# CompVis/stable-diffusion

Measured on AMD Instinct MI355X. Metric: 512x512 images/sec, SD-v1-4 50-step PLMS CFG=7.5, higher is better.
Workload: dtype f16

## Files before the change

### include/sdmi.h

```cpp
#ifndef SDMI_H_
#define SDMI_H_

#include <stdint.h>

#ifdef __cplusplus
extern "C" {
#endif

#define SDMI_ABI_VERSION 17

typedef struct sdmi_unet sdmi_unet;

typedef struct sdmi_unet_cfg {
  int32_t in_channels;
  int32_t out_channels;
  int32_t model_channels;
  int32_t num_res_blocks;
  int32_t n_levels;
  int32_t channel_mult[8];
  int32_t n_attention_resolutions;
  int32_t attention_resolutions[8];
  int32_t num_heads;
  int32_t transformer_depth;
  int32_t context_dim;
// ... 171 lines not shown
                        float* cs, float* d, void* stream);
int sdmi_k_attention(const void* q, const void* k, const void* vt, void* out, int BH, int heads, int nq, int nkv,
                     int nkv_pad, int d, float scale, void* stream);
int sdmi_k_attention_split16(const void* q, const void* q_lo, const void* k, const void* k_lo, const void* vt, const void* vt_lo, void* out,
                             void* out_lo, int BH, int heads, int nq, int nkv, int nkv_pad, int d, float scale, void* stream);
int sdmi_k_attention_causal(const void* q, const void* k, const void* vt, void* out, int BH, int heads, int n, int n_pad,
                            int d, float scale, void* stream);
int sdmi_k_groupnorm(const float* x0, const float* x1, int c0, int c1, int B, int HW, const float* gamma,
                     const float* beta, float eps, int silu, void* out_f16, float* out_f32, void* raw_f16, void* out_lo,
                     void* raw_lo, float* partial_ws, int64_t partial_floats, void* stream);
int64_t sdmi_k_groupnorm_ws_floats(int B, int HW);
int sdmi_k_groupnorm_film(const float* x0, const float* x1, int c0, int c1, int B, int HW, const float* gamma, const float* beta, float eps,
                          int silu, const float* film, int film_ld, void* out_f16, float* out_f32, void* raw_f16, void* out_lo, void* raw_lo,
                          float* partial_ws, int64_t partial_floats, void* stream);
int sdmi_k_layernorm(const float* x, const float* gamma, const float* beta, void* out_f16, int M, int C, float eps,
                     void* stream);
int sdmi_k_cast_f16(const float* x, void* out_f16, void* out_lo, int64_t n, void* stream);
int sdmi_k_split_heads(const float* src, int ld, int col0, void* dst, void* dst_lo, int kind, int B, int ntok, int ntok_pad, int heads, int dh,
                       void* stream);
int sdmi_k_geglu_split(const float* src, int M, int F, void* out, void* out_lo, void* stream);
int sdmi_k_layernorm_split(const float* x, const float* gamma, const float* beta, void* out, void* out_lo, int M, int C, float eps, void* stream);
int sdmi_k_timestep_embedding(const int64_t* t_i64, const float* t_f32, float* out, int B, int dim, void* stream);
int sdmi_k_small_linear(const float* in, int ld_in, const float* w, const float* bias, float* out, int ld_out, int B,
                        int N, int K, int silu_in, void* stream);
int sdmi_k_conv_in(const float* x_nchw, const float* w_oihw, const float* bias, float* out_nhwc, int B, int Cin, int H,
                   int W, int Cout, void* stream);
int sdmi_k_conv_out(const float* h_nhwc, const float* w_ohwi, const float* bias, float* out_nchw, int B, int H, int W,
                    int Cin, int Cout, void* stream);
int sdmi_k_pack_conv_weight(const float* w_oihw, void* dst_f16, int O, int I, int KH, int KW, void* stream);
int sdmi_k_pack_conv_weight_src(const float* w_oihw, void* dst_f16, int O, int I, int KH, int KW, int c0, int c1, int c2, void* stream);
int sdmi_k_pack_conv_out(const float* w_oihw, float* dst_ohwi, int O, int I, void* stream);
int sdmi_k_pack_split3(const float* w, void* dst_f16, int N, int K, void* stream);
int sdmi_k_pack_conv_split3(const float* w_oihw, void* dst_f16, int O, int I, int KH, int KW, void* stream);
int sdmi_k_pointwise_nchw(const float* x, const float* w, const float* bias, float* out, int B, int Cin, int Cout, int HW,
                          float in_scale, void* stream);
int sdmi_k_softmax_rows(const float* S, void* P_f16, int rows, int cols, float scale, void* stream);
int sdmi_k_vq_quantize(const float* z, float z_scale, const float* codebook, float* norms_ws, int n_embed, int D, float* zq, int32_t* idx,
                       int B, int HW, void* stream);
int sdmi_k_resample2(const float* x, float* out_f32, void* out_f16, void* out_lo, int B, int H, int W, int C, int dir, void* stream);
int sdmi_k_patch_unfold(const float* x, const float* c, float* out, int B, int Cx, int Cc, int H, int W, int kh, int kw, int sy, int sx,
                        int l0, int nl, void* stream);
int sdmi_k_patch_fold(const float* o, const float* w, float* out, int B, int C, int H, int W, int kh, int kw, int sy, int sx, int uf, int df,
                      int norm_only, void* stream);
int sdmi_k_gelu_erf(const float* x, void* out_f16, int64_t n, void* stream);
int sdmi_k_pack_geglu(const float* w, const float* bias, void* wdst_f16, float* bdst, int N, int K, void* stream);
int sdmi_image_to_uint8(const float* img_nchw, void* out_nhwc_u8, int B, int C, int H, int W, void* stream);
int sdmi_range_check(int enable);
int sdmi_range_report(char* json_buf, int json_buf_len);
int sdmi_tune_begin(void);
int sdmi_tune_round(int r);
int sdmi_tune_end(const char* path, int* n_keys);
int sdmi_tune_dump(char* buf, int buflen);
int sdmi_profile_begin(void);
int sdmi_profile_end(char* json_buf, int json_buf_len);
int sdmi_k_prefetch_lines(const void* ptr, int64_t bytes, void* stream);
const void* sdmi_zero_page(void);

#ifdef __cplusplus
}
#endif
#endif
```

### stable-diffusion_amd/_lib.py

```python
import ctypes as C
import os

_HERE = os.path.dirname(os.path.abspath(__file__))
LIB_PATH = os.environ.get('SDMI_LIB_PATH') or os.path.join(_HERE, 'libsdmi.so')

c_f32p = C.c_void_p
c_ptr = C.c_void_p


class UNetCfg(C.Structure):
    _fields_ = [('in_channels', C.c_int32), ('out_channels', C.c_int32), ('model_channels', C.c_int32),
                ('num_res_blocks', C.c_int32), ('n_levels', C.c_int32), ('channel_mult', C.c_int32 * 8),
                ('n_attention_resolutions', C.c_int32), ('attention_resolutions', C.c_int32 * 8),
                ('num_heads', C.c_int32), ('transformer_depth', C.c_int32), ('context_dim', C.c_int32)]


class VaeCfg(C.Structure):
    _fields_ = [('ch', C.c_int32), ('out_ch', C.c_int32), ('n_levels', C.c_int32), ('ch_mult', C.c_int32 * 8),
                ('num_res_blocks', C.c_int32), ('in_channels', C.c_int32), ('z_channels', C.c_int32),
                ('embed_dim', C.c_int32)]


class UNetExt(C.Structure):
    _fields_ = [('attention_block', C.c_int32), ('resblock_updown', C.c_int32)]
# ... 109 lines not shown
                                C.c_int, c_ptr]),
    'sdmi_k_st_head': (C.c_int, [c_ptr, c_ptr, C.c_int64, c_ptr, c_ptr, C.c_float, c_ptr, c_ptr, c_ptr, c_ptr, C.c_float, c_ptr, c_ptr, c_ptr,
                                 c_ptr, c_ptr, c_ptr, C.c_int, C.c_int, C.c_int, C.c_int, C.c_int, C.c_int, c_ptr]),
    'sdmi_k_attention_split16': (C.c_int, [c_ptr, c_ptr, c_ptr, c_ptr, c_ptr, c_ptr, c_ptr, c_ptr, C.c_int, C.c_int, C.c_int, C.c_int,
                                           C.c_int, C.c_int, C.c_float, c_ptr]),
    'sdmi_k_attention_causal': (C.c_int, [c_ptr, c_ptr, c_ptr, c_ptr, C.c_int, C.c_int, C.c_int, C.c_int, C.c_int, C.c_float,
                                          c_ptr]),
    'sdmi_k_pointwise_nchw': (C.c_int, [c_ptr, c_ptr, c_ptr, c_ptr, C.c_int, C.c_int, C.c_int, C.c_int, C.c_float, c_ptr]),
    'sdmi_k_softmax_rows': (C.c_int, [c_ptr, c_ptr, C.c_int, C.c_int, C.c_float, c_ptr]),
    'sdmi_k_gelu_erf': (C.c_int, [c_ptr, c_ptr, C.c_int64, c_ptr]),
    'sdmi_k_attention': (C.c_int, [c_ptr, c_ptr, c_ptr, c_ptr, C.c_int, C.c_int, C.c_int, C.c_int, C.c_int, C.c_int,
                                   C.c_float, c_ptr]),
    'sdmi_k_groupnorm': (C.c_int, [c_ptr, c_ptr, C.c_int, C.c_int, C.c_int, C.c_int, c_ptr, c_ptr, C.c_float, C.c_int,
                                   c_ptr, c_ptr, c_ptr, c_ptr, c_ptr, c_ptr, C.c_int64, c_ptr]),
    'sdmi_k_groupnorm_ws_floats': (C.c_int64, [C.c_int, C.c_int]),
    'sdmi_k_groupnorm_film': (C.c_int, [c_ptr, c_ptr, C.c_int, C.c_int, C.c_int, C.c_int, c_ptr, c_ptr, C.c_float, C.c_int, c_ptr, C.c_int,
                                        c_ptr, c_ptr, c_ptr, c_ptr, c_ptr, c_ptr, C.c_int64, c_ptr]),
    'sdmi_k_layernorm': (C.c_int, [c_ptr, c_ptr, c_ptr, c_ptr, C.c_int, C.c_int, C.c_float, c_ptr]),
    'sdmi_k_cast_f16': (C.c_int, [c_ptr, c_ptr, c_ptr, C.c_int64, c_ptr]),
    'sdmi_k_split_heads': (C.c_int, [c_ptr, C.c_int, C.c_int, c_ptr, c_ptr, C.c_int, C.c_int, C.c_int, C.c_int, C.c_int, C.c_int,
                                     c_ptr]),
    'sdmi_k_geglu_split': (C.c_int, [c_ptr, C.c_int, C.c_int, c_ptr, c_ptr, c_ptr]),
    'sdmi_k_layernorm_split': (C.c_int, [c_ptr, c_ptr, c_ptr, c_ptr, c_ptr, C.c_int, C.c_int, C.c_float, c_ptr]),
    'sdmi_k_timestep_embedding': (C.c_int, [c_ptr, c_ptr, c_ptr, C.c_int, C.c_int, c_ptr]),
    'sdmi_k_small_linear': (C.c_int, [c_ptr, C.c_int, c_ptr, c_ptr, c_ptr, C.c_int, C.c_int, C.c_int, C.c_int,
                                      C.c_int, c_ptr]),
    'sdmi_k_conv_in': (C.c_int, [c_ptr, c_ptr, c_ptr, c_ptr, C.c_int, C.c_int, C.c_int, C.c_int, C.c_int, c_ptr]),
    'sdmi_k_conv_out': (C.c_int, [c_ptr, c_ptr, c_ptr, c_ptr, C.c_int, C.c_int, C.c_int, C.c_int, C.c_int, c_ptr]),
    'sdmi_k_pack_conv_weight': (C.c_int, [c_ptr, c_ptr, C.c_int, C.c_int, C.c_int, C.c_int, c_ptr]),
    'sdmi_k_pack_conv_weight_src': (C.c_int, [c_ptr, c_ptr, C.c_int, C.c_int, C.c_int, C.c_int, C.c_int, C.c_int, C.c_int, c_ptr]),
    'sdmi_k_pack_conv_out': (C.c_int, [c_ptr, c_ptr, C.c_int, C.c_int, c_ptr]),
    'sdmi_k_pack_split3': (C.c_int, [c_ptr, c_ptr, C.c_int, C.c_int, c_ptr]),
    'sdmi_k_pack_conv_split3': (C.c_int, [c_ptr, c_ptr, C.c_int, C.c_int, C.c_int, C.c_int, c_ptr]),
    'sdmi_k_pack_geglu': (C.c_int, [c_ptr, c_ptr, c_ptr, c_ptr, C.c_int, C.c_int, c_ptr]),
    'sdmi_k_ln_fold_prep': (C.c_int, [c_ptr, C.c_int, C.c_int, C.c_int, c_ptr, c_ptr, c_ptr, c_ptr, c_ptr, c_ptr]),
    'sdmi_image_to_uint8': (C.c_int, [c_ptr, c_ptr, C.c_int, C.c_int, C.c_int, C.c_int, c_ptr]),
    'sdmi_range_check': (C.c_int, [C.c_int]),
    'sdmi_range_report': (C.c_int, [C.c_char_p, C.c_int]),
    'sdmi_tune_begin': (C.c_int, []),
    'sdmi_tune_round': (C.c_int, [C.c_int]),
    'sdmi_tune_end': (C.c_int, [C.c_char_p, C.POINTER(C.c_int)]),
    'sdmi_tune_dump': (C.c_int, [C.c_char_p, C.c_int]),
    'sdmi_profile_begin': (C.c_int, []),
    'sdmi_profile_end': (C.c_int, [C.c_char_p, C.c_int]),
    'sdmi_k_prefetch_lines': (C.c_int, [c_ptr, C.c_int64, c_ptr]),
    'sdmi_zero_page': (c_ptr, []),
}

_lib = None


class SdmiError(RuntimeError):
    pass


def load():
    global _lib
    if _lib is None:
        if not os.path.exists(LIB_PATH):
            raise SdmiError(f'{LIB_PATH} not found: build it with `python stable-diffusion_amd/build.py` '
                            '(the MI355X path has no fallback implementation)')
        lib = C.CDLL(LIB_PATH)
        for name, (res, args) in _SIGS.items():
            fn = getattr(lib, name)
            fn.restype = res
            fn.argtypes = args
# ... 23 lines not shown
```

### stable-diffusion_amd/csrc/api.cpp

```cpp
#include <string.h>

#include <new>

#include "prof.h"
#include "split16.h"
#include "unet.h"
#include "vae.h"
#include "clip.h"

namespace sdmi {
static thread_local std::string g_err;
void set_error(const std::string& msg) { g_err = msg; }
int fail(const std::string& msg) { g_err = msg; return -1; }
}

struct sdmi_unet { sdmi::UNet impl; };
struct sdmi_vae { sdmi::Vae impl; };
struct sdmi_clip { sdmi::ClipText impl; };
struct sdmi_bert { sdmi::BertText impl; };

using namespace sdmi;

static int weight_info(const WeightStore& w, int idx, char* key_buf, int key_buf_len, int64_t* shape4, int* ndim) {
  SDMI_CHECK(key_buf && shape4 && ndim, "null argument");
// ... 272 lines not shown
int sdmi_k_vq_quantize(const float* z, float z_scale, const float* codebook, float* norms_ws, int n_embed, int D, float* zq, int32_t* idx,
                       int B, int HW, void* stream) {
  if (launch_vq_norms(codebook, norms_ws, n_embed, D, (hipStream_t)stream)) return -1;
  return launch_vq_quantize(z, z_scale, codebook, norms_ws, n_embed, D, zq, (int*)idx, B, HW, (hipStream_t)stream);
}
int sdmi_k_resample2(const float* x, float* out_f32, void* out_f16, void* out_lo, int B, int H, int W, int C, int dir, void* stream) {
  return launch_resample2(x, out_f32, (f16*)out_f16, (f16*)out_lo, B, H, W, C, dir, (hipStream_t)stream);
}
int sdmi_k_patch_unfold(const float* x, const float* c, float* out, int B, int Cx, int Cc, int H, int W, int kh, int kw, int sy, int sx,
                        int l0, int nl, void* stream) {
  return launch_patch_unfold(x, c, out, B, Cx, Cc, H, W, kh, kw, sy, sx, l0, nl, (hipStream_t)stream);
}
int sdmi_k_patch_fold(const float* o, const float* w, float* out, int B, int C, int H, int W, int kh, int kw, int sy, int sx, int uf, int df,
                      int norm_only, void* stream) {
  return launch_patch_fold(o, w, out, B, C, H, W, kh, kw, sy, sx, uf, df, norm_only, (hipStream_t)stream);
}
int sdmi_k_gelu_erf(const float* x, void* out_f16, int64_t n, void* stream) {
  return launch_gelu_erf(x, (f16*)out_f16, n, (hipStream_t)stream);
}
int sdmi_k_attention_causal(const void* q, const void* k, const void* vt, void* out, int BH, int heads, int n, int n_pad,
                            int d, float scale, void* stream) {
  AttnParams a = AttnParams();
  a.q = (const f16*)q; a.k = (const f16*)k; a.vt = (const f16*)vt; a.out = (f16*)out;
  a.BH = BH; a.heads = heads; a.nq = n; a.nkv = n; a.nkv_pad = n_pad; a.d = d; a.scale = scale; a.causal = 1;
  return launch_attention(a, (hipStream_t)stream);
}

static int igemm_params_of(const sdmi_igemm_desc* d, IGemmParams& p) {
  p.a0 = (const f16*)d->a0; p.a1 = (const f16*)d->a1; p.a2 = (const f16*)d->a2;
  p.c0 = d->c0; p.c1 = d->c1; p.c2 = d->c2; p.lda0 = d->lda0; p.lda1 = d->lda1; p.lda2 = d->lda2;
  p.B = d->B; p.Hin = d->Hin; p.Win = d->Win; p.Hout = d->Hout; p.Wout = d->Wout;
  p.ksize = d->ksize; p.stride = d->stride; p.up = d->up; p.pad = d->asym_pad ? 0 : 1;
  p.w = (const f16*)d->w; p.M = d->B * d->Hout * d->Wout; p.N = d->N; p.K = d->ksize * d->ksize * (d->c0 + d->c1 + d->c2);
  p.mode = d->mode; p.bias = d->bias; p.rowvec = d->rowvec; p.ld_rowvec = d->ld_rowvec;
  p.residual = d->residual; p.ldr = d->ldr; p.out_f32 = d->out_f32; p.out_f16 = (f16*)d->out_f16; p.ldo = d->ldo;
  for (int i = 0; i < 3; ++i) { p.seg_dst[i] = (f16*)d->seg_dst[i]; p.seg_kind[i] = d->seg_kind[i]; }
  p.heads = d->heads; p.dh = d->dh; p.ntok = d->ntok; p.ntok_pad = d->ntok_pad; p.segC = d->segC;
  p.splitk = d->splitk; p.splitk_ws = d->splitk_ws; p.splitk_ws_floats = d->splitk_ws_floats;
  p.splitk_cnt = d->splitk_cnt; p.splitk_cnt_ints = d->splitk_cnt_ints;
  p.gn_n = d->gn_n;
  for (int i = 0; i < 2; ++i) { p.gn_acc[i] = (long long*)d->gn_acc[i]; p.gn_cpg[i] = d->gn_cpg[i]; p.gn_cbase[i] = d->gn_cbase[i]; }
  if (d->split16) {
    p.split16 = 1; p.c1 = 0; p.K = d->c0; p.ldw = 3 * d->c0;
  }
  p.f16_scale = d->f16_scale; p.lnp_out = d->lnp_out;
  p.lnf_part = d->lnf_part; p.lnf_npart = d->lnf_npart; p.lnf_eps = d->lnf_eps; p.lnf_cs = d->lnf_cs; p.lnf_d = d->lnf_d;
  p.pgn_gamma = d->pgn_gamma; p.pgn_beta = d->pgn_beta; p.pgn_eps = d->pgn_eps; p.pgn_silu = d->pgn_silu;
  p.pgn_out = (f16*)d->pgn_out; p.pgn_keep_f32 = d->pgn_keep_f32; p.pgn_applied = d->pgn_applied;
  p.out_lo = (f16*)d->out_lo;
  return zero_page(&p.zero_page);
}
int sdmi_k_igemm(const sdmi_igemm_desc* d, void* stream) {
  SDMI_CHECK(d, "null descriptor");
  IGemmParams p = IGemmParams();
  if (igemm_params_of(d, p)) return -1;
  IGemmTune t; t.tile = d->tile; t.dma = d->dma;
  return launch_igemm(p, t, (hipStream_t)stream);
}
int sdmi_k_ff_tail(const sdmi_igemm_desc* proj_out, const void* ln_f16, const float* lnp, float ln_eps, const float* csd,
                   const void* wgg_f16, const void* wff2_f16, const float* bff2, const float* t, void* stream) {
  SDMI_CHECK(proj_out, "null descriptor");
  FfTailParams q = FfTailParams();
  if (igemm_params_of(proj_out, q.epi)) return -1;
  SDMI_CHECK(proj_out->split16 && proj_out->ksize == 1, "ff_tail: the proj_out descriptor is a split-fp16 1x1 (w = sdmi_k_pack_split3)");
  q.ln = (const f16*)ln_f16; q.lnp = lnp; q.ln_eps = ln_eps; q.csd = csd; q.wgg = (const f16*)wgg_f16; q.wff2 = (const f16*)wff2_f16;
  q.bff2 = bff2; q.t = t; q.wpo = (const f16*)proj_out->w;
// ... 119 lines not shown
int sdmi_k_geglu_split(const float* src, int M, int F, void* out, void* out_lo, void* stream) {
  return launch_geglu_split(src, M, F, (f16*)out, (f16*)out_lo, (hipStream_t)stream);
}
int sdmi_k_layernorm_split(const float* x, const float* gamma, const float* beta, void* out, void* out_lo, int M, int C, float eps, void* stream) {
  return launch_layernorm_split(x, gamma, beta, (f16*)out, (f16*)out_lo, M, C, eps, (hipStream_t)stream);
}
int sdmi_k_timestep_embedding(const int64_t* t_i64, const float* t_f32, float* out, int B, int dim, void* stream) {
  return launch_timestep_embedding(t_i64, t_f32, out, B, dim, (hipStream_t)stream);
}
int sdmi_k_small_linear(const float* in, int ld_in, const float* w, const float* bias, float* out, int ld_out, int B,
                        int N, int K, int silu_in, void* stream) {
  return launch_small_linear(in, ld_in, w, bias, out, ld_out, B, N, K, silu_in, (hipStream_t)stream);
}
int sdmi_k_conv_in(const float* x, const float* w, const float* bias, float* out, int B, int Cin, int H, int W, int Cout,
                   void* stream) {
  return launch_conv_in(x, w, bias, out, B, Cin, H, W, Cout, (hipStream_t)stream);
}
int sdmi_k_conv_out(const float* h, const float* w, const float* bias, float* out, int B, int H, int W, int Cin, int Cout,
                    void* stream) {
  return launch_conv_out(h, w, bias, out, B, H, W, Cin, Cout, (hipStream_t)stream);
}
int sdmi_k_pack_conv_weight(const float* w, void* dst, int O, int I, int KH, int KW, void* stream) {
  return launch_pack_conv_weight(w, (f16*)dst, O, I, KH, KW, (hipStream_t)stream);
}
int sdmi_k_pack_conv_weight_src(const float* w, void* dst, int O, int I, int KH, int KW, int c0, int c1, int c2, void* stream) {
  return launch_pack_conv_weight_src(w, (f16*)dst, O, I, KH, KW, c0, c1, c2, (hipStream_t)stream);
}
int sdmi_k_pack_conv_out(const float* w, float* dst, int O, int I, void* stream) {
  return launch_pack_conv_out(w, dst, O, I, (hipStream_t)stream);
}
int sdmi_k_pack_split3(const float* w, void* dst, int N, int K, void* stream) {
  return launch_pack_split3(w, (f16*)dst, N, K, (hipStream_t)stream);
}
int sdmi_k_pack_conv_split3(const float* w, void* dst, int O, int I, int KH, int KW, void* stream) {
  return launch_pack_conv_split3(w, (f16*)dst, O, I, KH, KW, (hipStream_t)stream);
}
int sdmi_k_pack_geglu(const float* w, const float* bias, void* wdst, float* bdst, int N, int K, void* stream) {
  return launch_pack_geglu(w, bias, (f16*)wdst, bdst, N, K, (hipStream_t)stream);
}
int sdmi_image_to_uint8(const float* img_nchw, void* out_nhwc_u8, int B, int C, int H, int W, void* stream) {
  return launch_image_u8(img_nchw, (unsigned char*)out_nhwc_u8, B, C, H, W, (hipStream_t)stream);
}
int sdmi_range_check(int enable) { return range_check_set(enable); }
int sdmi_range_report(char* buf, int buflen) {
  SDMI_CHECK(buf && buflen > 1, "null buffer");
  std::string js;
  if (range_report(&js)) return -1;
  SDMI_CHECK((int)js.size() + 1 <= buflen, "range report buffer too small");
  memcpy(buf, js.c_str(), js.size() + 1);
  return 0;
}
int sdmi_tune_begin(void) { return tune_begin(); }
int sdmi_tune_round(int r) { return tune_round(r); }
int sdmi_tune_end(const char* path, int* n_keys) { return tune_end(path, n_keys); }
int sdmi_tune_dump(char* buf, int buflen) {
  SDMI_CHECK(buf && buflen > 1, "null buffer");
  std::string txt;
  if (tune_dump(&txt)) return -1;
  SDMI_CHECK((int)txt.size() + 1 <= buflen, "tune dump buffer too small");
  memcpy(buf, txt.c_str(), txt.size() + 1);
  return 0;
}
int sdmi_profile_begin(void) { return prof_begin(); }
int sdmi_profile_end(char* buf, int buflen) {
  SDMI_CHECK(buf && buflen > 2, "null buffer");
  std::string js;
// ... 17 lines not shown
```

### stable-diffusion_amd/csrc/common.h

```cpp
#pragma once
#include <hip/hip_runtime.h>
#include <stdint.h>
#include <algorithm>
#include <string>

#include "tape.h"

typedef _Float16 f16;
typedef _Float16 f16x2 __attribute__((ext_vector_type(2)));
typedef _Float16 f16x4 __attribute__((ext_vector_type(4)));
typedef _Float16 f16x8 __attribute__((ext_vector_type(8)));
typedef float f32x4 __attribute__((ext_vector_type(4)));
typedef float f32x16 __attribute__((ext_vector_type(16)));

#ifdef __HIPCC__
__device__ __forceinline__ float gn_apply_elem(float v, float mean, float rstd, float gamma, float beta, int silu) {
  float t = __builtin_fmaf((v - mean) * rstd, gamma, beta);
  if (silu) t = t * __builtin_amdgcn_rcpf(1.0f + __expf(-t));
  return t;
}
__device__ __forceinline__ float gn_apply_film_elem(float v, float mean, float rstd, float gamma, float beta, float scale, float shift,
                                                    int silu) {
  float t = __builtin_fmaf((v - mean) * rstd, gamma, beta);
  t = __builtin_fmaf(t, 1.0f + scale, shift);
// ... 291 lines not shown
  float* x_next = nullptr;
  int64_t n = 0;
};
int launch_dpm_step(const DpmStepParams& p, hipStream_t s);

int launch_embed_tokens(const int64_t* ids, const float* tok_emb, const float* pos_emb, float* out, int M, int L, int C,
                        int vocab, hipStream_t s);
int launch_quick_gelu(const float* x, f16* out, int64_t n, hipStream_t s);
int launch_gelu_erf(const float* x, f16* out, int64_t n, hipStream_t s);

int launch_pointwise_nchw(const float* x_nchw, const float* w, const float* bias, float* out_nchw, int B, int Cin, int Cout,
                          int HW, float in_scale, hipStream_t s);
int launch_softmax_rows(const float* S, f16* P, int rows, int cols, int lds, int ldp, float scale, hipStream_t s);

int launch_resample2(const float* x, float* o32, f16* hi, f16* lo, int B, int H, int W, int C, int dir, hipStream_t s);
int launch_vq_norms(const float* e, float* se, int n_embed, int D, hipStream_t s);
int launch_vq_quantize(const float* z, float z_scale, const float* e, const float* se, int n_embed, int D, float* zq, int* idx, int B,
                       int HW, hipStream_t s);

int launch_patch_unfold(const float* x, const float* c, float* out, int B, int Cx, int Cc, int H, int W, int kh, int kw, int sy, int sx,
                        int l0, int nl, hipStream_t s);
int launch_patch_fold(const float* o, const float* w, float* out, int B, int C, int H, int W, int kh, int kw, int sy, int sx, int uf, int df,
                      int norm_only, hipStream_t s);

int launch_prefetch_lines(const void* ptr, int64_t bytes, hipStream_t s);

int launch_pack_conv_weight(const float* w_oihw, f16* dst, int O, int I, int KH, int KW, hipStream_t s);
int launch_pack_rows(const float* w, f16* dst, int rows, int cols, int dst_row0, int dst_ld, hipStream_t s);
int launch_ln_fold_prep(const f16* w, int N, int K, int ldw, const float* gamma, const float* beta, const float* bias, float* cs,
                        float* d, hipStream_t s);
int launch_pack_split3(const float* w, f16* dst, int N, int K, hipStream_t s);
int launch_pack_conv_weight_src(const float* w_oihw, f16* dst, int O, int I, int KH, int KW, int c0, int c1, int c2, hipStream_t s);
int launch_pack_conv_split3(const float* w, f16* dst, int O, int I, int KH, int KW, hipStream_t s);
int launch_pack_geglu(const float* w, const float* bias, f16* wdst, float* bdst, int N, int K, hipStream_t s);
int launch_pack_conv_out(const float* w_oihw, float* dst, int O, int I, hipStream_t s);

struct SamplerStepParams {
  const float* eps_model = nullptr;
  int cfg = 0; float scale = 1.f;
  const float* x = nullptr;
  int mode = 0;
  const float* old0 = nullptr; const float* old1 = nullptr; const float* old2 = nullptr;
  float a_t = 1.f, a_prev = 1.f, sigma = 0.f, sqrt_1m_at = 0.f;
  const float* noise = nullptr;
  float* e_t_out = nullptr;
  float* x_prev = nullptr; float* pred_x0 = nullptr;
  int64_t n = 0;
};
int launch_sampler_step(const SamplerStepParams& p, hipStream_t s);
int launch_image_u8(const float* img_nchw, unsigned char* out_nhwc, int B, int C, int H, int W, hipStream_t s);

}
```

### stable-diffusion_amd/csrc/igemm.hip

```cpp
#include <dlfcn.h>

#include <map>
#include <mutex>
#include <tuple>
#include <vector>

#include "igemm_dev.h"

namespace sdmi {
namespace {

__global__ void __launch_bounds__(256) splitk_reduce_kernel(IGemmParams p, int nsplit, int rows_per_block) {
  __shared__ unsigned long long s_gn[2][32][GN_WORDS];
  const int tx = threadIdx.x & 7, ty = threadIdx.x >> 3;
  const int n = (blockIdx.x * 8 + tx) * 4;
  const int row0 = blockIdx.y * rows_per_block;
  const int HW = p.Hout * p.Wout;
  const bool gn = p.gn_n > 0;
  const bool ncol = n < p.N;
  if (gn) {
    for (int i = threadIdx.x; i < 2 * 32 * GN_WORDS; i += 256) (&s_gn[0][0][0])[i] = 0ull;
    __syncthreads();
  }
  const size_t slab_sz = (size_t)p.M * p.N;
  f32x4 biasv = {0.f, 0.f, 0.f, 0.f};
  if (ncol && p.bias) biasv = *(const f32x4*)(p.bias + n);
  float a1[2] = {0.f, 0.f}, a2[2] = {0.f, 0.f}, c1[2] = {0.f, 0.f}, c2[2] = {0.f, 0.f};
  int g0[2] = {0, 0}, g1[2] = {0, 0}, gsplit[2] = {4, 4};
  for (int t = 0; t < p.gn_n; ++t) {
    const int c = p.gn_cbase[t] + n;
    g0[t] = fast_div(c, p.gn_magic[t]); g1[t] = fast_div(c + 3, p.gn_magic[t]);
    gsplit[t] = (g0[t] + 1) * p.gn_cpg[t] - c;
  }
  for (int r = ty; r < rows_per_block; r += 32) {
    const int m = row0 + r;
    if (!ncol || m >= p.M) continue;
    const float* src = p.splitk_ws + (size_t)m * p.N + n;
    f32x4 rvv = {0.f, 0.f, 0.f, 0.f}, resv = {0.f, 0.f, 0.f, 0.f};
    if (p.rowvec) rvv = *(const f32x4*)(p.rowvec + (size_t)(m / HW) * p.ld_rowvec + n);
    if (p.residual) resv = *(const f32x4*)(p.residual + (size_t)m * p.ldr + n);
    f32x4 part[16];
#pragma unroll
    for (int s = 0; s < 16; ++s) part[s] = (s < nsplit) ? *(const f32x4*)(src + s * slab_sz) : f32x4{0, 0, 0, 0};
    f32x4 v = part[0];
#pragma unroll
    for (int s = 1; s < 16; ++s) v += part[s];
    v += biasv;
    if (p.rowvec) v += rvv;
    if (p.residual) v += resv;
    if (p.out_f32) SDMI_ST_F32X4(p.out_f32, (size_t)m * p.ldo + n, v);
    if (p.out_f16) SDMI_ST_F16X4(p.out_f16, (size_t)m * p.ldo + n, (f16x4{(f16)v[0], (f16)v[1], (f16)v[2], (f16)v[3]}));
    if (p.out_lo) {
      f16x4 lo;
#pragma unroll
      for (int j = 0; j < 4; ++j) lo[j] = (f16)(v[j] - (float)(f16)v[j]);
      *(f16x4*)(p.out_lo + (size_t)m * p.ldo + n) = lo;
    }
    if (gn) {
#pragma unroll
      for (int t = 0; t < 2; ++t) {
#pragma unroll
        for (int j = 0; j < 4; ++j) {
          if (j < gsplit[t]) { a1[t] += v[j]; a2[t] += v[j] * v[j]; } else { c1[t] += v[j]; c2[t] += v[j] * v[j]; }
        }
      }
    }
  }
  if (gn) {
    if (ncol) {
      for (int t = 0; t < p.gn_n; ++t) {
        gn_acc_add(&s_gn[t][g0[t]][0], a1[t]);
        gn_acc_add(&s_gn[t][g0[t]][2], a2[t]);
        if (g1[t] != g0[t]) { gn_acc_add(&s_gn[t][g1[t]][0], c1[t]); gn_acc_add(&s_gn[t][g1[t]][2], c2[t]); }
      }
    }
    __syncthreads();
    const int b = row0 / HW;
    const int slot = (blockIdx.x + blockIdx.y) & (GN_SLOTS - 1);
    for (int e = threadIdx.x; e < p.gn_n * 32 * GN_WORDS; e += 256) {
      const unsigned long long w = (&s_gn[0][0][0])[e];
      if (w == 0ull) continue;
      const int word = e % GN_WORDS, g = (e / GN_WORDS) % 32, t = e / (GN_WORDS * 32);
      atomicAdd((unsigned long long*)p.gn_acc[t] + ((size_t)(b * 32 + g) * GN_SLOTS + slot) * GN_STRIDE + word, w);
    }
  }
}

__global__ void __launch_bounds__(256) splitk_reduce_heads_kernel(IGemmParams p, int nsplit) {
  const int64_t idx = (int64_t)blockIdx.x * blockDim.x + threadIdx.x;
  const int nq = p.N / 4;
  if (idx >= (int64_t)p.M * nq) return;
  const int m = (int)(idx / nq);
  const int n = (int)(idx - (int64_t)m * nq) * 4;
  const size_t slab_sz = (size_t)p.M * p.N;
  const float* src = p.splitk_ws + (size_t)m * p.N + n;
  f32x4 part[16];
#pragma unroll
  for (int s = 0; s < 16; ++s) part[s] = (s < nsplit) ? *(const f32x4*)(src + s * slab_sz) : f32x4{0, 0, 0, 0};
  f32x4 v = part[0];
#pragma unroll
  for (int s = 1; s < 16; ++s) v += part[s];
  if (p.bias) v += *(const f32x4*)(p.bias + n);
  const int seg = n / p.segC;
  const int c = n - seg * p.segC;
  const int head = c / p.dh;
  const int dd = c - head * p.dh;
  const int b = m / p.ntok;
  const int tok = m - b * p.ntok;
  const size_t bh = (size_t)b * p.heads + head;
  f16* dst = p.seg_dst[seg];
  if (p.seg_kind[seg] == 0) {
    *(f16x4*)(dst + (bh * p.ntok + tok) * p.dh + dd) = f16x4{(f16)v[0], (f16)v[1], (f16)v[2], (f16)v[3]};
  } else {
#pragma unroll
    for (int j = 0; j < 4; ++j) dst[(bh * p.dh + dd + j) * p.ntok_pad + tok] = (f16)v[j];
  }
}

__device__ __forceinline__ float pick4(const f32x4 v, int idx) {
  return idx == 0 ? v[0] : (idx == 1 ? v[1] : (idx == 2 ? v[2] : v[3]));
}
template <int CTRL>
__device__ __forceinline__ float quad_dpp(float x) {
  return __builtin_bit_cast(float, __builtin_amdgcn_update_dpp(0, __builtin_bit_cast(int, x), CTRL, 0xF, 0xF, true));
}
__device__ __forceinline__ f32x4 quad_transpose(const f32x4 v, int sub) {
  const float r0 = pick4(v, sub);
  const float r1 = quad_dpp<0x93>(pick4(v, (sub + 1) & 3));
  const float r2 = quad_dpp<0x4E>(pick4(v, (sub + 2) & 3));
  const float r3 = quad_dpp<0x39>(pick4(v, (sub + 3) & 3));
  const f32x4 r = {r0, r1, r2, r3};
  return f32x4{pick4(r, sub & 3), pick4(r, (sub - 1) & 3), pick4(r, (sub - 2) & 3), pick4(r, (sub - 3) & 3)};
}
__device__ __forceinline__ void quad_partials_split(const f32x4 v, int gsplit, float* a1, float* a2, float* c1, float* c2) {
#pragma clang fp contract(off)
  float s1 = 0.f, s2 = 0.f, t1 = 0.f, t2 = 0.f;
#pragma unroll
  for (int j = 0; j < 4; ++j) {
    const float sq = v[j] * v[j];
    if (j < gsplit) { s1 += v[j]; s2 += sq; } else { t1 += v[j]; t2 += sq; }
  }
  *a1 = s1; *a2 = s2; *c1 = t1; *c2 = t2;
}
struct TiledQuad { size_t off; int m, n; bool valid; };
__device__ __forceinline__ TiledQuad tiled_quad(const IGemmParams& p, int q, int lane) {
  const int BM = p.slab_bm, BN = p.slab_bn;
  const int WTM = BM / p.slab_wm, WTN = BN >> p.slab_sh_wn;
  const int tiles_n = (p.N + BN - 1) / BN;
  const int tile = q >> p.slab_sh_qpt, rem = q - (tile << p.slab_sh_qpt);
  const int blk = rem >> p.slab_sh_nt, t_in = rem - (blk << p.slab_sh_nt);
  const int wave = t_in >> 6;
  const int ij = blk >> 2, r4 = blk & 3, i = ij >> p.slab_sh_tn, j = ij - (i << p.slab_sh_tn);
  const int wm = wave >> p.slab_sh_wn, wn = wave - (wm << p.slab_sh_wn);
  const int tile_m = tile / tiles_n, tile_n = tile - tile_m * tiles_n;
  const int l31 = lane & 31, lg = lane >> 5;
  TiledQuad t;
  t.off = (size_t)tile * (size_t)(BM * BN) + (size_t)rem * 4;
  t.m = tile_m * BM + wm * WTM + i * 32 + 8 * r4 + 4 * lg + (l31 & 3);
  t.n = tile_n * BN + wn * WTN + j * 32 + (l31 & ~3);
  t.valid = t.m < p.M && t.n < p.N;
  return t;
}
#ifndef SDMI_REDUCE_GN_XCD_DEFAULT
#define SDMI_REDUCE_GN_XCD_DEFAULT 0
#endif
constexpr int COOP_BAR_INTS = 18 * 32;
template <bool COOP>
__global__ void __launch_bounds__(COOP ? 1024 : 256) splitk_reduce_tiled_kernel(IGemmParams p, int nsplit) {
  constexpr int NWV = COOP ? 16 : 4;
  __shared__ unsigned long long s_gn[2][NWV][32][GN_WORDS];
  const int tid = threadIdx.x, lane = tid & 63, wv = tid >> 6, NTB = blockDim.x;
  const bool gn = p.gn_n > 0;
  if (gn) {
    for (int i = tid; i < 2 * NWV * 32 * GN_WORDS; i += NTB) (&s_gn[0][0][0][0])[i] = 0ull;
    __syncthreads();
  }
  const TiledQuad t = tiled_quad(p, blockIdx.x * NTB + tid, lane);
  const int ntiles = ((p.M + p.slab_bm - 1) / p.slab_bm) * ((p.N + p.slab_bn - 1) / p.slab_bn);
  const size_t split_stride = (size_t)ntiles * (size_t)(p.slab_bm * p.slab_bn);
  const float* src = p.splitk_ws + t.off;
  const int HW = p.Hout * p.Wout;
  const int m = min(t.m, p.M - 1), n = min(t.n, p.N - 4);
  f32x4 biasv = {0.f, 0.f, 0.f, 0.f}, rvv = {0.f, 0.f, 0.f, 0.f}, resv = {0.f, 0.f, 0.f, 0.f};
  if (p.bias) biasv = *(const f32x4*)(p.bias + n);
  if (p.rowvec) rvv = *(const f32x4*)(p.rowvec + (size_t)(m / HW) * p.ld_rowvec + n);
  if (p.residual) resv = *(const f32x4*)(p.residual + (size_t)m * p.ldr + n);
  f32x4 part[16];
#pragma unroll
  for (int s = 0; s < 16; ++s) part[s] = (s < nsplit) ? *(const f32x4*)(src + s * split_stride) : f32x4{0.f, 0.f, 0.f, 0.f};
  f32x4 a = part[0];
#pragma unroll
  for (int s = 1; s < 16; ++s) a += part[s];
  f32x4 v = quad_transpose(a, lane & 3);
  v += biasv;
  if (p.rowvec) v += rvv;
  if (p.residual) v += resv;
  if (t.valid) {
    if (p.out_f32 && (!COOP || p.pgn_keep_f32)) SDMI_ST_F32X4(p.out_f32, (size_t)m * p.ldo + n, v);
    if (p.out_f16) SDMI_ST_F16X4(p.out_f16, (size_t)m * p.ldo + n, (f16x4{(f16)v[0], (f16)v[1], (f16)v[2], (f16)v[3]}));
    if (p.out_lo) {
      f16x4 lo;
#pragma unroll
      for (int j = 0; j < 4; ++j) lo[j] = (f16)(v[j] - (float)(f16)v[j]);
      *(f16x4*)(p.out_lo + (size_t)m * p.ldo + n) = lo;
    }
  }
  if (gn) {
    if (t.valid) {
      for (int tg = 0; tg < p.gn_n; ++tg) {
        const int c = p.gn_cbase[tg] + n;
        const int g0 = fast_div(c, p.gn_magic[tg]), g1 = fast_div(c + 3, p.gn_magic[tg]);
        const int gsplit = (g0 + 1) * p.gn_cpg[tg] - c;
        float a1, a2, c1, c2;
        quad_partials_split(v, gsplit, &a1, &a2, &c1, &c2);
        gn_acc_add(&s_gn[tg][wv][g0][0], a1);
        gn_acc_add(&s_gn[tg][wv][g0][2], a2);
        if (g1 != g0) { gn_acc_add(&s_gn[tg][wv][g1][0], c1); gn_acc_add(&s_gn[tg][wv][g1][2], c2); }
      }
    }
    __syncthreads();
    const int slot = blockIdx.x & (GN_SLOTS - 1);
    for (int e = tid; e < p.gn_n * NWV * 32 * GN_WORDS; e += NTB) {
      const unsigned long long w = (&s_gn[0][0][0][0])[e];
      if (w == 0ull) continue;
      const int word = e % GN_WORDS, g = (e / GN_WORDS) % 32, w4 = (e / (GN_WORDS * 32)) % NWV, tg = e / (GN_WORDS * 32 * NWV);
      if (w4 * 64 >= NTB) continue;
      const TiledQuad t0 = tiled_quad(p, blockIdx.x * NTB + w4 * 64, 0);
      if (t0.m >= p.M) continue;
      const int b = t0.m / HW;
      atomicAdd((unsigned long long*)p.gn_acc[tg] + ((size_t)(b * 32 + g) * GN_SLOTS + slot) * GN_STRIDE + word, w);
    }
  }
  if constexpr (COOP) {
    __shared__ int s_ok;
    __shared__ float2 s_tab[NWV][4];
    asm volatile("s_waitcnt vmcnt(0)" ::: "memory");
    __syncthreads();
    int* const blk = p.splitk_cnt + p.splitk_cnt_ints - COOP_BAR_INTS;
    const int nblk = (int)gridDim.x, ngrp = min(nblk, 8);
    if (tid == 0) {
      const int g = (int)blockIdx.x & 7, pop = (nblk - g + 7) >> 3;
      const int ep = __hip_atomic_load(blk + 9 * 32, __ATOMIC_RELAXED, __HIP_MEMORY_SCOPE_AGENT) + 1;
      if (__hip_atomic_fetch_add(blk + g * 32, 1, __ATOMIC_RELAXED, __HIP_MEMORY_SCOPE_AGENT) == pop - 1) {
        if (__hip_atomic_fetch_add(blk + 8 * 32, 1, __ATOMIC_RELAXED, __HIP_MEMORY_SCOPE_AGENT) == ngrp - 1) {
          for (int j = 0; j <= 8; ++j) __hip_atomic_store(blk + j * 32, 0, __ATOMIC_RELAXED, __HIP_MEMORY_SCOPE_AGENT);
          __hip_atomic_store(blk + 9 * 32, ep, __ATOMIC_RELAXED, __HIP_MEMORY_SCOPE_AGENT);
          for (int j = 0; j < ngrp; ++j) __hip_atomic_store(blk + (10 + j) * 32, ep, __ATOMIC_RELAXED, __HIP_MEMORY_SCOPE_AGENT);
        }
      }
      int budget = 1 << 16, seen = 0;
      while ((seen = __hip_atomic_load(blk + (10 + g) * 32, __ATOMIC_RELAXED, __HIP_MEMORY_SCOPE_AGENT)) != ep && --budget > 0) __builtin_amdgcn_s_sleep(2);
      s_ok = seen == ep;
    }
    __syncthreads();
    const int cpg = p.N >> 5;
    const TiledQuad tw = tiled_quad(p, blockIdx.x * NTB + wv * 64, 0);
    const int bw = min(tw.m, p.M - 1) / HW;
    const int gfirst = fast_div(min(tw.n, p.N - 1), p.gn_magic[0]);
    if (lane < 32) {
      const int g = min(gfirst + (lane >> 3), 31), sub = lane & 7;
      const long long* srcw = (const long long*)p.gn_acc[0] + ((size_t)(bw * 32 + g) * GN_SLOTS + sub) * GN_STRIDE;
// ... 29 lines not shown
  const float* src = p.splitk_ws + t.off;
  f32x4 part[16];
#pragma unroll
  for (int s = 0; s < 16; ++s) part[s] = (s < nsplit) ? *(const f32x4*)(src + s * split_stride) : f32x4{0.f, 0.f, 0.f, 0.f};
  f32x4 a = part[0];
#pragma unroll
  for (int s = 1; s < 16; ++s) a += part[s];
  f32x4 v = quad_transpose(a, lane & 3);
  if (!t.valid) return;
  const int m = t.m, n = t.n;
  if (p.bias) v += *(const f32x4*)(p.bias + n);
  const int seg = n / p.segC;
  const int c = n - seg * p.segC;
  const int head = c / p.dh;
  const int dd = c - head * p.dh;
  const int b = m / p.ntok;
  const int tok = m - b * p.ntok;
  const size_t bh = (size_t)b * p.heads + head;
  f16* dst = p.seg_dst[seg];
  if (p.seg_kind[seg] == 0) {
    *(f16x4*)(dst + (bh * p.ntok + tok) * p.dh + dd) = f16x4{(f16)v[0], (f16)v[1], (f16)v[2], (f16)v[3]};
  } else {
#pragma unroll
    for (int j = 0; j < 4; ++j) dst[(bh * p.dh + dd + j) * p.ntok_pad + tok] = (f16)v[j];
  }
}


}

int launch_splitk_reduce(const IGemmParams& p, int nsplit, hipStream_t stream) {
  SDMI_CHECK(nsplit >= 1 && nsplit <= 16 && p.N % 4 == 0 && p.splitk_ws, "splitk_reduce: bad arguments");
  if (p.slab_tiled) {
    const int64_t quads = (int64_t)cdiv(p.M, p.slab_bm) * cdiv(p.N, p.slab_bn) * (p.slab_bm * p.slab_bn / 4);
    SDMI_CHECK(quads % 256 == 0 && quads / 256 < (1ll << 31) && p.slab_wm > 0 && p.slab_wn > 0, "tiled split-K slabs: bad geometry");
    const double mn = (double)p.M * p.N;
    if (p.mode == EPI_HEADS) {
      ProfScope psh("splitk_reduce", 0.0, mn * (4.0 * nsplit + 2.0), stream);
      SDMI_LAUNCH(splitk_reduce_tiled_heads_kernel, dim3((unsigned)(quads / 256)), dim3(256), 0, stream, p, nsplit);
      SDMI_HIP_OK(hipGetLastError());
      return 0;
    }
    if (p.gn_n > 0) SDMI_CHECK((p.Hout * p.Wout) % 32 == 0, "GroupNorm statistics need Hout*Wout % 32 == 0");
    const bool coop = env_int("SDMI_REDUCE_GN_XCD", SDMI_REDUCE_GN_XCD_DEFAULT) && p.pgn_out && p.pgn_gamma && p.pgn_beta && p.mode == EPI_PLAIN && p.gn_n == 1 &&
                      p.gn_cbase[0] == 0 && p.gn_cpg[0] == p.N / 32 && p.N % 128 == 0 && p.N / 32 >= 16 && p.M == p.B * p.Hout * p.Wout &&
                      (p.Hout * p.Wout) % 32 == 0 && !p.out_f16 && !p.out_lo && !p.ln_out && p.splitk_cnt && p.splitk_cnt_ints >= COOP_BAR_INTS &&
                      quads % 1024 == 0 && quads / 1024 <= 256 && (!p.pgn_keep_f32 || (p.out_f32 && p.ldo % 4 == 0));
    ProfScope pst(coop ? "splitk_reduce_gn" : "splitk_reduce", 0.0, coop ? mn * (4.0 * nsplit + 2.0 + (p.pgn_keep_f32 ? 4.0 : 0.0)) : mn * 4.0 * (nsplit + 1), stream);
    const int rb_env = env_int("SDMI_REDUCE_BLOCK", 256);
    const int rb = (rb_env == 128 || (rb_env == 0 && quads / 256 < 512)) ? 128 : 256;
    if (coop) {
      SDMI_LAUNCH(splitk_reduce_tiled_kernel<true>, dim3((unsigned)(quads / 1024)), dim3(1024), 0, stream, p, nsplit);
      SDMI_HIP_OK(hipGetLastError());
      pst.end();
      if (p.pgn_applied) *p.pgn_applied = 1;
      if (range_check_enabled() && range_scan("GroupNorm fp16 output (split-K reduction)", p.pgn_out, (int64_t)p.M * p.N, stream)) return -1;
      return 0;
    }
    SDMI_LAUNCH(splitk_reduce_tiled_kernel<false>, dim3((unsigned)(quads / rb)), dim3(rb), 0, stream, p, nsplit);
    SDMI_HIP_OK(hipGetLastError());
    pst.end();
    if (p.ln_out) return launch_layernorm(p.out_f32, p.ln_gamma, p.ln_beta, p.ln_out, p.M, p.N, p.ln_eps, stream);
    return 0;
  }
  if (p.mode == EPI_HEADS) {
    const int64_t total_h = (int64_t)p.M * (p.N / 4);
    ProfScope psh("splitk_reduce", 0.0, (double)p.M * p.N * (4.0 * nsplit + 2.0), stream);
    SDMI_LAUNCH(splitk_reduce_heads_kernel, dim3((unsigned)((total_h + 255) / 256)), dim3(256), 0, stream, p, nsplit);
    SDMI_HIP_OK(hipGetLastError());
    return 0;
  }
  const int hw = p.Hout * p.Wout;
  if (p.gn_n > 0) SDMI_CHECK(hw % 32 == 0, "GroupNorm statistics need Hout*Wout % 32 == 0");
  const int rpb = reduce_rows_per_block(p);
  ProfScope ps2("splitk_reduce", 0.0, (double)p.M * p.N * 4.0 * (nsplit + 1), stream);
  SDMI_LAUNCH(splitk_reduce_kernel, dim3((unsigned)cdiv(p.N / 4, 8), (unsigned)cdiv(p.M, rpb)), dim3(256), 0, stream, p, nsplit,
                     rpb);
  SDMI_HIP_OK(hipGetLastError());
  ps2.end();
  if (p.ln_out) return launch_layernorm(p.out_f32, p.ln_gamma, p.ln_beta, p.ln_out, p.M, p.N, p.ln_eps, stream);
  return 0;
}

struct TileCfg { int bm, bn, wm, wn, ns; };
static const TileCfg kTiles[SDMI_NUM_TILES] = {
    {128, 128, 2, 2, 2},
    {128, 64, 2, 2, 2},
    {64, 64, 2, 2, 2},
    {256, 128, 4, 2, 2},
    {128, 64, 2, 2, 3},
    {64, 64, 2, 2, 3},
    {256, 128, 4, 2, 3},
    {128, 128, 2, 2, 3},
    {64, 128, 2, 2, 3},
    {128, 128, 4, 2, 3},
    {64, 64, 2, 2, 4},
    {128, 256, 2, 4, 2},
    {64, 256, 1, 4, 3},
    {256, 64, 4, 1, 3},
    {256, 64, 4, 2, 5},
    {256, 128, 4, 2, 3},
    {128, 64, 2, 2, 8},
    {128, 128, 2, 2, 5},
    {64, 64, 2, 2, 8},
    {64, 128, 2, 2, 6},
// ... 41 lines not shown
  std::vector<TuneRec> recs;
  std::map<TuneKey, std::vector<std::pair<TuneChoice, std::vector<float>>>> stats;
  std::vector<hipEvent_t> pool;

  static std::string default_path() {
    if (const char* e = getenv("SDMI_TUNE_FILE")) return e;
    Dl_info info;
    if (dladdr((const void*)&Tuner::default_path, &info) && info.dli_fname) {
      std::string so = info.dli_fname;
      const size_t k = so.find_last_of('/');
      return (k == std::string::npos ? std::string(".") : so.substr(0, k)) + "/tune_gfx950.txt";
    }
    return "tune_gfx950.txt";
  }
  void load_file(const std::string& path) {
    FILE* f = fopen(path.c_str(), "r");
    if (!f) return;
    char line[256];
    while (fgets(line, sizeof line, f)) {
      if (line[0] == '#') continue;
      TuneKey k; TuneChoice c; c.us = 0;
      if (sscanf(line, "%d %d %d %d %d %d %d %d %d %d %lf", &k.M, &k.N, &k.K, &k.ksize, &k.stride, &k.up, &k.mode,
                 &k.splitk_req, &c.tile, &c.splitk, &c.us) >= 10 && c.tile >= 0 && c.tile < SDMI_NUM_TILES && c.splitk >= 1 &&
          c.splitk <= 16)
        table[k] = c;
    }
    fclose(f);
  }
  void ensure_loaded() {
    if (loaded) return;
    loaded = true;
    if (env_int("SDMI_TUNE_DISABLE", 0)) return;
    load_file(default_path());
  }
  hipEvent_t ev() {
    if (!pool.empty()) { hipEvent_t e = pool.back(); pool.pop_back(); return e; }
    hipEvent_t e = nullptr;
    (void)hipEventCreate(&e);
    return e;
  }
};
static Tuner g_tuner;

static std::vector<TuneChoice> tune_candidates(const IGemmParams& p, bool can_split) {
  std::vector<TuneChoice> out;
  const int nkt = igemm_nkt(p);
  static const int splits[] = {1, 2, 3, 4, 5, 6, 8, 10, 12, 16};
  for (int t = 0; t < SDMI_NUM_TILES; ++t) {
    const TileCfg& c = kTiles[t];
    if (tile_is_halo(t) && !halo_supported(p, c.bm)) continue;
    if (p.split16 && !split16_tile_supported(t)) continue;
    if (!p.split16 && ((c.ns == 2 && t != 11 && !tile_is_halo(t)) || t == 12 || t == 13)) continue;
    if (p.mode == EPI_GEGLU && !tile_tn_even(t)) continue;
    if (p.lnp_out && (p.M % c.bm || p.N % c.bn || (p.Hout * p.Wout) % c.bm)) continue;
    const long blocks = (long)cdiv(p.M, c.bm) * cdiv(p.N, c.bn);
    if ((long)c.bm > 2L * p.M && c.bm > 64) continue;
    if ((long)c.bn > 2L * p.N && c.bn > 64) continue;
    for (int sk : splits) {
      if ((sk == 5 || sk == 10) && !tile_is_halo(t)) continue;
      if (sk > 1) {
        if (p.splitk != 0 || !can_split) break;
        if (nkt / sk < 4) break;
        if (tile_is_halo(t) && (nkt / 9) % sk != 0) continue;
        if (blocks * (sk / 2 + 1) > 1536) break;
        if (splitk_ws_need(p, c.bm, c.bn, sk) > p.splitk_ws_floats) break;
      }
      if (blocks * sk < 48 && sk < 16 && nkt / (sk * 2) >= 4 && can_split && p.splitk == 0) continue;
      out.push_back({t, p.splitk > 1 ? p.splitk : sk, 0.0});
      if (p.splitk != 0) break;
    }
  }
  if (out.empty()) out.push_back({5, p.splitk > 0 ? p.splitk : 1, 0.0});
  return out;
}

int tune_begin() {
  std::lock_guard<std::mutex> lk(g_tuner.mu);
  g_tuner.ensure_loaded();
  g_tuner.collecting = true; g_tuner.round = 0;
  g_tuner.recs.clear(); g_tuner.stats.clear();
  return 0;
}
int tune_round(int r) {
  std::lock_guard<std::mutex> lk(g_tuner.mu);
  g_tuner.round = r;
  return 0;
}
static int tune_drain() {
  for (auto& r : g_tuner.recs) {
// ... 33 lines not shown
  const std::string out = (path && *path) ? std::string(path) : Tuner::default_path();
  FILE* f = fopen(out.c_str(), "w");
  if (!f) return fail("cannot write the tuning table to " + out);
  fprintf(f, "# libsdmi igemm tuning table (gfx950), measured in situ by tools/tune.py -- M N K ksize stride up mode splitk_req tile splitk us\n");
  for (auto& kv : g_tuner.table) {
    const TuneKey& k = kv.first;
    fprintf(f, "%d %d %d %d %d %d %d %d %d %d %.2f\n", k.M, k.N, k.K, k.ksize, k.stride, k.up, k.mode, k.splitk_req, kv.second.tile,
            kv.second.splitk, kv.second.us);
  }
  fclose(f);
  return 0;
}
int tune_dump(std::string* out) {
  std::lock_guard<std::mutex> lk(g_tuner.mu);
  char buf[256];
  for (auto& kv : g_tuner.stats) {
    const TuneKey& k = kv.first;
    for (auto& c : kv.second) {
      if (c.second.empty()) continue;
      std::vector<float> v = c.second;
      std::sort(v.begin(), v.end());
      snprintf(buf, sizeof buf, "%d %d %d %d %d %d %d %d | %d %d %.2f %.2f %d\n", k.M, k.N, k.K, k.ksize, k.stride, k.up, k.mode,
               k.splitk_req, c.first.tile, c.first.splitk, (double)v[v.size() / 2], (double)v[0], (int)v.size());
      *out += buf;
    }
  }
  return 0;
}

int launch_igemm(const IGemmParams& p, const IGemmTune& tune, hipStream_t stream) {
  SDMI_CHECK(p.M > 0 && p.N > 0 && p.K > 0, "empty GEMM");
  SDMI_CHECK(p.ksize == 1 || p.ksize == 3, "ksize must be 1 or 3");
  const int Cin = p.c0 + p.c1 + p.c2;
  SDMI_CHECK(p.K == p.ksize * p.ksize * Cin, "K != ksize^2 * (c0 + c1 + c2)");
  SDMI_CHECK(p.c0 % BKH == 0 && p.c1 % BKH == 0 && p.c2 % BKH == 0 && p.c0 > 0, "channel counts of every A source must be multiples of 32");
  SDMI_CHECK((p.c2 == 0 || p.c1 > 0), "third A source without a second");
  SDMI_CHECK(p.lda0 % 8 == 0 && (p.a1 == nullptr || p.lda1 % 8 == 0), "A row pitch must be a multiple of 8 halves");
  SDMI_CHECK(p.zero_page != nullptr, "zero page missing");
  SDMI_CHECK(p.M == p.B * p.Hout * p.Wout, "M != B * Hout * Wout");
  SDMI_CHECK(p.c1 == 0 || p.a1 != nullptr, "second A source missing");
  SDMI_CHECK(p.c2 == 0 || (p.a2 != nullptr && p.lda2 % 8 == 0), "third A source missing");
  SDMI_CHECK((p.c1 == 0 || p.lda1 == p.lda0) && (p.c2 == 0 || p.lda2 == p.lda0), "all A sources must share one row pitch");
  SDMI_CHECK(!p.up || (p.ksize == 3 && p.stride == 1), "upsample folding needs a 3x3 stride-1 conv");
  if (p.mode == EPI_GEGLU) SDMI_CHECK(p.N % 64 == 0 && p.out_f16 != nullptr, "GEGLU needs N % 64 == 0 and an fp16 output");
  if (p.ln_out)
    SDMI_CHECK(p.mode == EPI_PLAIN && p.out_f32 && p.ldo == p.N && p.N % 4 == 0 && p.N <= 2560 && p.ln_gamma && p.ln_beta,
               "LayerNorm post-op needs plain mode, an fp32 output with ldo == N <= 2560, gamma and beta");
  if (p.out_lo) SDMI_CHECK(p.mode == EPI_PLAIN && p.ldo % 4 == 0, "out_lo needs plain mode");
  if (p.lnp_out || p.f16_scale)
    SDMI_CHECK(p.mode == EPI_PLAIN && p.out_f32 && p.out_f16 && !p.out_lo && !p.ln_out && p.N % 64 == 0 && p.M % 64 == 0 &&
                   (p.Hout * p.Wout) % 64 == 0 && p.splitk == 1 && epi_vec_ok(p),
               "LayerNorm row statistics: plain mode, fp32 + fp16 outputs, no split-K, M / N / rows per sample multiples of 64, 16-byte aligned rows");
  if (p.lnf_part)
    SDMI_CHECK(p.ksize == 1 && p.c1 == 0 && p.c2 == 0 && !p.split16 && p.lnf_npart * 32 == p.K && p.lnf_cs && p.lnf_d && !p.bias &&
                   p.splitk == 1 && p.lnf_npart <= 40,
               "LayerNorm-folding GEMM: dense, one source, K = 32 * lnf_npart <= 1280, column sums + offsets, no bias, no split-K");
  if (p.gn_n) {
    SDMI_CHECK(p.mode == EPI_PLAIN && p.gn_n <= 2 && (p.Hout * p.Wout) % 32 == 0, "GroupNorm statistics need plain mode and Hout*Wout % 32 == 0");
    SDMI_CHECK(p.N % 4 == 0, "GroupNorm statistics: N % 4 == 0");
    for (int t = 0; t < p.gn_n; ++t)
      SDMI_CHECK(p.gn_acc[t] && p.gn_cpg[t] >= 2 && (p.gn_cbase[t] + p.N + p.gn_cpg[t] - 1) / p.gn_cpg[t] <= 32, "bad GroupNorm statistics target");
  }
  if (p.mode == EPI_HEADS) SDMI_CHECK(p.segC > 0 && p.dh > 0 && p.N % p.segC == 0 && p.N / p.segC <= 3, "bad head scatter");

  SDMI_CHECK((int64_t)p.B * p.Hin * p.Win * p.lda0 * 2 + (int64_t)(p.Win + 1) * p.lda0 * 2 < ((int64_t)1 << 31) - 65536 &&
                 (int64_t)p.N * p.K * 2 < ((int64_t)1 << 31) - 65536,
             "tensor too large for 31-bit byte offsets (buffer addressing)");
// ... 141 lines not shown
```

### stable-diffusion_amd/csrc/igemm_dev.h

```cpp
#pragma once
#include "common.h"
#include "prof.h"

namespace sdmi {
typedef unsigned u32x4 __attribute__((ext_vector_type(4)));

int launch_splitk_reduce(const IGemmParams& p, int nsplit, hipStream_t stream);
int launch_generic_tile_g0(int tile, const IGemmParams& p, bool dma, int splitk, hipStream_t stream);
int launch_generic_tile_g1(int tile, const IGemmParams& p, bool dma, int splitk, hipStream_t stream);
int launch_generic_tile_g2(int tile, const IGemmParams& p, bool dma, int splitk, hipStream_t stream);
int launch_generic_tile_h0(int tile, const IGemmParams& p, bool dma, int splitk, hipStream_t stream);
int launch_generic_tile_h1(int tile, const IGemmParams& p, bool dma, int splitk, hipStream_t stream);
int launch_generic_tile_h2(int tile, const IGemmParams& p, bool dma, int splitk, hipStream_t stream);

static int env_int(const char* name, int dflt) {
  const char* v = getenv(name);
  return v ? atoi(v) : dflt;
}

namespace {

constexpr int BK = 64;
constexpr int BKH = 32;
static inline int src_chunks(int c) { return (c + BK - 1) / BK; }
static inline bool igemm_has_half(const IGemmParams& p) { return p.split16 ? (p.K % BK != 0) : (p.c0 % BK || p.c1 % BK || p.c2 % BK); }
static inline int igemm_nkt(const IGemmParams& p) {
  if (p.split16) return src_chunks(p.K);
  return p.ksize * p.ksize * (src_chunks(p.c0) + src_chunks(p.c1) + src_chunks(p.c2));
}

#ifdef SDMI_IGEMM_TIMING
#define SDMI_STAMP(name) const long long name = p.dbg_times ? (long long)__builtin_readcyclecounter() : 0
#else
#define SDMI_STAMP(name)
#endif

__device__ __forceinline__ float gelu_erf(float x) {
  const float z = fabsf(x) * 0.70710678118654752440f;
  const float t = __builtin_amdgcn_rcpf(1.0f + 0.3275911f * z);
  const float poly = t * (0.254829592f + t * (-0.284496736f + t * (1.421413741f + t * (-1.453152027f + t * 1.061405429f))));
  const float erf_abs = 1.0f - poly * __expf(-z * z);
  const float erf_v = __builtin_copysignf(erf_abs, x);
  return 0.5f * x * (1.0f + erf_v);
}

__device__ __forceinline__ void wait_vmcnt_n(int n) {
  switch (n) {
#define SDMI_VMCNT_CASE(k) case k: asm volatile("s_waitcnt vmcnt(" #k ")" ::: "memory"); break
    SDMI_VMCNT_CASE(0); SDMI_VMCNT_CASE(1); SDMI_VMCNT_CASE(2); SDMI_VMCNT_CASE(3); SDMI_VMCNT_CASE(4);
    SDMI_VMCNT_CASE(5); SDMI_VMCNT_CASE(6); SDMI_VMCNT_CASE(7); SDMI_VMCNT_CASE(8); SDMI_VMCNT_CASE(9);
    SDMI_VMCNT_CASE(10); SDMI_VMCNT_CASE(11); SDMI_VMCNT_CASE(12); SDMI_VMCNT_CASE(13); SDMI_VMCNT_CASE(14);
    SDMI_VMCNT_CASE(15); SDMI_VMCNT_CASE(16); SDMI_VMCNT_CASE(17); SDMI_VMCNT_CASE(18); SDMI_VMCNT_CASE(19);
    SDMI_VMCNT_CASE(20); SDMI_VMCNT_CASE(21); SDMI_VMCNT_CASE(22); SDMI_VMCNT_CASE(23); SDMI_VMCNT_CASE(24);
    SDMI_VMCNT_CASE(25); SDMI_VMCNT_CASE(26); SDMI_VMCNT_CASE(27); SDMI_VMCNT_CASE(28); SDMI_VMCNT_CASE(29);
    SDMI_VMCNT_CASE(30); SDMI_VMCNT_CASE(31); SDMI_VMCNT_CASE(32); SDMI_VMCNT_CASE(33); SDMI_VMCNT_CASE(34);
    SDMI_VMCNT_CASE(35); SDMI_VMCNT_CASE(36); SDMI_VMCNT_CASE(37); SDMI_VMCNT_CASE(38); SDMI_VMCNT_CASE(39);
    SDMI_VMCNT_CASE(40); SDMI_VMCNT_CASE(41); SDMI_VMCNT_CASE(42); SDMI_VMCNT_CASE(43); SDMI_VMCNT_CASE(44);
    SDMI_VMCNT_CASE(45); SDMI_VMCNT_CASE(46); SDMI_VMCNT_CASE(47); SDMI_VMCNT_CASE(48);
#undef SDMI_VMCNT_CASE
    default: __builtin_trap();
  }
}
template <int N>
__device__ __forceinline__ void wait_vmcnt() {
  static_assert(N >= 0 && N <= 48, "add the literal");
  wait_vmcnt_n(N);
}

enum : int { KIND_1X1 = 0, KIND_3X3 = 1, KIND_3X3_UP = 2 };

__device__ __forceinline__ int fast_div(int m, unsigned long long magic) {
  return (int)(((unsigned long long)(unsigned)m * magic) >> 40);
}
__device__ __forceinline__ int fast_div_hw(int m, unsigned long long magic) {
  return (int)(((unsigned long long)(unsigned)m * magic) >> 48);
}

#if defined(__HIP_DEVICE_COMPILE__)
template <int WTN> constexpr int SLAB_LPR = WTN / 4;
template <int WTN> constexpr int SLAB_RPI = 64 / (WTN / 4);
template <int WTN> constexpr int SLAB_NPASS = 32 / (64 / (WTN / 4));
template <int NWAVES, int WTN, int LDS_BYTES>
constexpr int SLAB_LSTR = (NWAVES * 32 * (WTN + 4) * 4 <= LDS_BYTES) ? WTN + 4 : WTN;
template <int NWAVES, int WTN, int LDS_BYTES>
__device__ __forceinline__ float* slab_base(unsigned char* smem, int wave) {
  static_assert(WTN == 32 || WTN == 64, "lane mapping of the 16-byte epilogue");
  static_assert(NWAVES * 32 * SLAB_LSTR<NWAVES, WTN, LDS_BYTES> * 4 <= LDS_BYTES, "LDS too small for the epilogue slabs");
  return (float*)smem + wave * (32 * SLAB_LSTR<NWAVES, WTN, LDS_BYTES>);
}
template <int TN, int LSTR>
__device__ __forceinline__ void slab_put(float* wl, const f32x16 (&a)[TN], int l31, int lg) {
#pragma unroll
  for (int j = 0; j < TN; ++j)
#pragma unroll
    for (int r = 0; r < 16; ++r) wl[((r & 3) + 8 * (r >> 2) + 4 * lg) * LSTR + j * 32 + l31] = a[j][r];
  asm volatile("s_waitcnt lgkmcnt(0)" ::: "memory");
}
template <int TN, int LSTR>
__device__ __forceinline__ void slab_get(const float* wl, f32x16 (&a)[TN], int l31, int lg) {
  asm volatile("s_waitcnt lgkmcnt(0)" ::: "memory");
#pragma unroll
  for (int j = 0; j < TN; ++j)
// ... 3 lines not shown
}

constexpr int LNF_MAXP = 40;
__device__ __forceinline__ void lnf_request(const IGemmParams& p, int m, float2 (&pv)[LNF_MAXP]) {
  const float2* src = (const float2*)p.lnf_part + m;
#pragma unroll
  for (int j = 0; j < 20; ++j) pv[j] = src[(size_t)min(j, p.lnf_npart - 1) * p.M];
  if (p.lnf_npart > 20) {
#pragma unroll
    for (int j = 20; j < LNF_MAXP; ++j) pv[j] = src[(size_t)min(j, p.lnf_npart - 1) * p.M];
  } else {
#pragma unroll
    for (int j = 20; j < LNF_MAXP; ++j) pv[j] = float2{0.f, 0.f};
  }
}
__device__ __forceinline__ void lnf_finish(const IGemmParams& p, const float2 (&pv)[LNF_MAXP], float* mean, float* rstd) {
  float s = 0.f, q = 0.f;
#pragma unroll
  for (int j = 0; j < LNF_MAXP; ++j)
    if (j < p.lnf_npart) { s += pv[j].x; q += pv[j].y; }
  const float inv_c = 1.0f / (32.0f * (float)p.lnf_npart);
  const float mu = s * inv_c;
  const float var = fmaxf(q * inv_c - mu * mu, 0.f);
  *mean = mu;
  *rstd = 1.0f / sqrtf(var + p.lnf_eps);
}
__device__ __forceinline__ float sum8_dpp(float v) {
  v += __builtin_bit_cast(float, __builtin_amdgcn_update_dpp(0, __builtin_bit_cast(int, v), 0xB1, 0xF, 0xF, true));
  v += __builtin_bit_cast(float, __builtin_amdgcn_update_dpp(0, __builtin_bit_cast(int, v), 0x4E, 0xF, 0xF, true));
  v += __builtin_bit_cast(float, __builtin_amdgcn_update_dpp(0, __builtin_bit_cast(int, v), 0x141, 0xF, 0xF, true));
  return v;
}

template <int BM, int BN, int WARPS_M, int WARPS_N, int LDS_BYTES>
__device__ __forceinline__ void igemm_epilogue(const IGemmParams& p_arg, f32x16 (&acc)[BM / WARPS_M / 32][BN / WARPS_N / 32],
                                               const int m0, const int n0, const int split, const int tile_m,
                                               const int tile_n, unsigned char* smem, const float lnf_mean = 0.f,
                                               const float lnf_rstd = 1.f) {
#ifdef SDMI_IGEMM_TIMING
  IGemmParams p = p_arg;
  if (p.dbg_abl & 1) p.residual = nullptr;
  if (p.dbg_abl & 4) { p.out_f32 = nullptr; p.out_f16 = nullptr; p.out_lo = nullptr; }
#else
  const IGemmParams& p = p_arg;
#endif
  constexpr int NT = WARPS_M * WARPS_N * 64;
  constexpr int WTM = BM / WARPS_M, WTN = BN / WARPS_N;
  constexpr int TM = WTM / 32, TN = WTN / 32;
  constexpr int LSTR = SLAB_LSTR<WARPS_M * WARPS_N, WTN, LDS_BYTES>;
  const int tid = threadIdx.x;
  const int lane = tid & 63;
  const int wave = tid >> 6;
  const int wm = wave / WARPS_N, wn = wave - wm * WARPS_N;
  const int l31 = lane & 31, lg = lane >> 5;
  const int HWout = p.Hout * p.Wout;
  const int mw = m0 + wm * WTM, nw = n0 + wn * WTN;
  const bool full = (m0 + BM <= p.M) && (n0 + BN <= p.N);
  if (p.splitk > 1 && p.splitk_fused) {
    constexpr int SC1 = 16;
    const int tile_lin = tile_m * ((p.N + BN - 1) / BN) + tile_n;
    const __amdgpu_buffer_rsrc_t ws = __builtin_amdgcn_make_buffer_rsrc(
        (void*)(p.splitk_ws + (size_t)tile_lin * p.splitk * (BM * BN)), 0, p.splitk * (BM * BN) * 4, 0x00020000);
    const int my_off = (split * (BM * BN) + tid * 4) * 4;
#pragma unroll
    for (int i = 0; i < TM; ++i)
#pragma unroll
      for (int j = 0; j < TN; ++j)
#pragma unroll
        for (int r4 = 0; r4 < 4; ++r4) {
          const f32x4 v = {acc[i][j][4 * r4], acc[i][j][4 * r4 + 1], acc[i][j][4 * r4 + 2], acc[i][j][4 * r4 + 3]};
          __builtin_amdgcn_raw_buffer_store_b128(__builtin_bit_cast(u32x4, v), ws, my_off + ((i * TN + j) * 4 + r4) * (NT * 16), 0, SC1);
        }
    asm volatile("s_waitcnt vmcnt(0)" ::: "memory");
    __syncthreads();
    if (tid == 0) *(volatile int*)smem = __hip_atomic_fetch_add(p.splitk_cnt + tile_lin, 1, __ATOMIC_RELAXED, __HIP_MEMORY_SCOPE_AGENT);
    __syncthreads();
    const int ticket = *(volatile int*)smem;
    if (ticket != p.splitk - 1) return;
    if (tid == 0) __hip_atomic_store(p.splitk_cnt + tile_lin, 0, __ATOMIC_RELAXED, __HIP_MEMORY_SCOPE_AGENT);
#pragma unroll
    for (int i = 0; i < TM; ++i)
#pragma unroll
      for (int j = 0; j < TN; ++j)
#pragma unroll
        for (int r = 0; r < 16; ++r) acc[i][j][r] = 0.f;
    constexpr int QPS = TM * TN * 4;
    constexpr int SB = QPS >= 16 ? 1 : 16 / QPS;
    for (int s0 = 0; s0 < p.splitk; s0 += SB) {
      f32x4 v[SB][QPS];
#pragma unroll
      for (int ss = 0; ss < SB; ++ss) {
        const int off = (min(s0 + ss, p.splitk - 1) * (BM * BN) + tid * 4) * 4;
#pragma unroll
        for (int e = 0; e < QPS; ++e)
          v[ss][e] = __builtin_bit_cast(f32x4, __builtin_amdgcn_raw_buffer_load_b128(ws, off + e * (NT * 16), 0, SC1));
      }
#pragma unroll
      for (int ss = 0; ss < SB; ++ss) {
        if (s0 + ss < p.splitk) {
#pragma unroll
          for (int i = 0; i < TM; ++i)
#pragma unroll
            for (int j = 0; j < TN; ++j)
#pragma unroll
              for (int r4 = 0; r4 < 4; ++r4)
#pragma unroll
                for (int e = 0; e < 4; ++e) acc[i][j][4 * r4 + e] += v[ss][(i * TN + j) * 4 + r4][e];
        }
      }
    }
    __syncthreads();
  }
  if (p.splitk > 1 && !p.splitk_fused && p.slab_tiled) {
    constexpr int SC1 = 16;
    const int tiles_n_all = (p.N + BN - 1) / BN, ntiles = ((p.M + BM - 1) / BM) * tiles_n_all;
    const int tile_lin = tile_m * tiles_n_all + tile_n;
    const __amdgpu_buffer_rsrc_t ws = __builtin_amdgcn_make_buffer_rsrc(
        (void*)(p.splitk_ws + ((size_t)split * ntiles + tile_lin) * (size_t)(BM * BN)), 0, BM * BN * 4, 0x00020000);
#pragma unroll
    for (int i = 0; i < TM; ++i)
#pragma unroll
      for (int j = 0; j < TN; ++j)
#pragma unroll
        for (int r4 = 0; r4 < 4; ++r4) {
          const f32x4 v = {acc[i][j][4 * r4], acc[i][j][4 * r4 + 1], acc[i][j][4 * r4 + 2], acc[i][j][4 * r4 + 3]};
          __builtin_amdgcn_raw_buffer_store_b128(__builtin_bit_cast(u32x4, v), ws, (tid * 4 + ((i * TN + j) * 4 + r4) * (NT * 4)) * 4, 0, SC1);
        }
    return;
  }
  if (p.lnf_part) {
    __syncthreads();
    float2* const tab = (float2*)smem;
    if (tid < BM) tab[tid] = float2{lnf_mean, lnf_rstd};
    __syncthreads();
#pragma unroll
    for (int j = 0; j < TN; ++j) {
      const int n = min(nw + j * 32 + l31, p.N - 1);
      const float cs = p.lnf_cs[n], dn = p.lnf_d[n];
#pragma unroll
      for (int i = 0; i < TM; ++i)
#pragma unroll
        for (int r = 0; r < 16; ++r) {
          const float2 mr = tab[wm * WTM + i * 32 + (r & 3) + 8 * (r >> 2) + 4 * lg];
          acc[i][j][r] = fmaf(mr.y, acc[i][j][r] - mr.x * cs, dn);
        }
    }
    __syncthreads();
  }
  const bool unfused_split = p.splitk > 1 && !p.splitk_fused;
  if (p.mode == EPI_PLAIN) {
    const bool atomic = unfused_split;
    float* slab = atomic ? (p.splitk_ws + (size_t)split * p.M * p.N) : nullptr;
    const int b_first = m0 / HWout;
    const bool one_batch = ((m0 + BM - 1) / HWout == b_first);
    if (full && one_batch && p.epi_vec && !atomic) {
      __syncthreads();
      float* const wl = slab_base<WARPS_M * WARPS_N, WTN, LDS_BYTES>(smem, wave);
      const int rl = lane / SLAB_LPR<WTN>, c4 = (lane % SLAB_LPR<WTN>) * 4;
      f32x4 colv = {0.f, 0.f, 0.f, 0.f};
      if (p.bias) colv = *(const f32x4*)(p.bias + nw + c4);
      if (p.rowvec) colv += *(const f32x4*)(p.rowvec + (size_t)b_first * p.ld_rowvec + nw + c4);
      f32x4 g4 = {1.f, 1.f, 1.f, 1.f};
      if (p.f16_scale) g4 = *(const f32x4*)(p.f16_scale + nw + c4);
#pragma unroll
      for (int i = 0; i < TM; ++i) {
        slab_put<TN, LSTR>(wl, acc[i], l31, lg);
        constexpr int NP = SLAB_NPASS<WTN>, RPI = SLAB_RPI<WTN>;
        f32x4 resv[NP];
        if (p.residual) {
#pragma unroll
          for (int q = 0; q < NP; ++q)
            resv[q] = *(const f32x4*)(p.residual + (size_t)(mw + i * 32 + q * RPI + rl) * p.ldr + nw + c4);
        } else {
#pragma unroll
          for (int q = 0; q < NP; ++q) resv[q] = f32x4{0.f, 0.f, 0.f, 0.f};
        }
#pragma unroll
        for (int q = 0; q < NP; ++q) {
          const int row = q * RPI + rl;
          float* const lp = wl + row * LSTR + c4;
          const f32x4 v = *(const f32x4*)lp + colv + resv[q];
          const size_t ro = (size_t)(mw + i * 32 + row) * p.ldo + nw + c4;
          if (p.out_f32) SDMI_ST_F32X4(p.out_f32, ro, v);
          const f32x4 vs = v * g4;
          const f16x4 h = {(f16)vs[0], (f16)vs[1], (f16)vs[2], (f16)vs[3]};
          if (p.out_f16) SDMI_ST_F16X4(p.out_f16, ro, h);
          if (p.out_lo)
            *(f16x4*)(p.out_lo + ro) = f16x4{(f16)(v[0] - (float)h[0]), (f16)(v[1] - (float)h[1]), (f16)(v[2] - (float)h[2]),
                                            (f16)(v[3] - (float)h[3])};
          if (p.lnp_out) {
            float s1 = (v[0] + v[1]) + (v[2] + v[3]);
            float s2 = (v[0] * v[0] + v[1] * v[1]) + (v[2] * v[2] + v[3] * v[3]);
            s1 = sum8_dpp(s1); s2 = sum8_dpp(s2);
            if ((lane & 7) == 0)
              *(float2*)(p.lnp_out + 2 * ((size_t)((nw + c4) >> 5) * p.M + (size_t)(mw + i * 32 + row))) = float2{s1, s2};
          }
          if (p.gn_n > 0) *(f32x4*)lp = v;
        }
        if (p.gn_n > 0) slab_get<TN, LSTR>(wl, acc[i], l31, lg);
        else asm volatile("s_waitcnt lgkmcnt(0)" ::: "memory");
      }
    } else if (full && one_batch) {
      if (atomic) {
#pragma unroll
        for (int i = 0; i < TM; ++i)
#pragma unroll
          for (int r = 0; r < 16; ++r) {
            float* row = slab + (size_t)(mw + i * 32 + (r & 3) + 8 * (r >> 2) + 4 * lg) * p.N + nw + l31;
#pragma unroll
            for (int j = 0; j < TN; ++j) row[j * 32] = acc[i][j][r];
          }
      } else {
        float colv[TN];
#pragma unroll
        for (int j = 0; j < TN; ++j) {
          const int n = nw + j * 32 + l31;
          colv[j] = p.bias ? p.bias[n] : 0.f;
          if (p.rowvec) colv[j] += p.rowvec[(size_t)b_first * p.ld_rowvec + n];
        }
#pragma unroll
        for (int i = 0; i < TM; ++i) {
          float resv[16][TN];
          if (p.residual) {
#pragma unroll
            for (int r = 0; r < 16; ++r) {
              const float* row = p.residual + (size_t)(mw + i * 32 + (r & 3) + 8 * (r >> 2) + 4 * lg) * p.ldr + nw + l31;
#pragma unroll
              for (int j = 0; j < TN; ++j) resv[r][j] = row[j * 32];
            }
          } else {
#pragma unroll
            for (int r = 0; r < 16; ++r)
#pragma unroll
              for (int j = 0; j < TN; ++j) resv[r][j] = 0.f;
          }
#pragma unroll
          for (int r = 0; r < 16; ++r) {
            const size_t ro = (size_t)(mw + i * 32 + (r & 3) + 8 * (r >> 2) + 4 * lg) * p.ldo + nw + l31;
#pragma unroll
            for (int j = 0; j < TN; ++j) {
              const float v = acc[i][j][r] + colv[j] + resv[r][j];
              acc[i][j][r] = v;
              if (p.out_f32) p.out_f32[ro + j * 32] = v;
              if (p.out_f16) p.out_f16[ro + j * 32] = (f16)v;
              if (p.out_lo) p.out_lo[ro + j * 32] = (f16)(v - (float)(f16)v);
            }
          }
        }
      }
    } else {
      float bias_v[TN];
#pragma unroll
      for (int j = 0; j < TN; ++j) {
        const int n = nw + j * 32 + l31;
        bias_v[j] = (!atomic && p.bias && n < p.N) ? p.bias[n] : 0.f;
      }
#pragma unroll
      for (int i = 0; i < TM; ++i) {
#pragma unroll
        for (int r = 0; r < 16; ++r) {
          const int m = mw + i * 32 + (r & 3) + 8 * (r >> 2) + 4 * lg;
          if (m >= p.M) continue;
          const float* rv = (!atomic && p.rowvec) ? (p.rowvec + (size_t)(m / HWout) * p.ld_rowvec) : nullptr;
#pragma unroll
          for (int j = 0; j < TN; ++j) {
            const int n = nw + j * 32 + l31;
            if (n >= p.N) continue;
            float v = acc[i][j][r];
            if (atomic) {
              slab[(size_t)m * p.N + n] = v;
            } else {
              v += bias_v[j];
              if (rv) v += rv[n];
              if (p.residual) v += p.residual[(size_t)m * p.ldr + n];
              acc[i][j][r] = v;
              if (p.out_f32) p.out_f32[(size_t)m * p.ldo + n] = v;
              if (p.out_f16) p.out_f16[(size_t)m * p.ldo + n] = (f16)v;
              if (p.out_lo) p.out_lo[(size_t)m * p.ldo + n] = (f16)(v - (float)(f16)v);
            }
          }
        }
      }
    }
#ifdef SDMI_IGEMM_TIMING
    if (p.dbg_times && threadIdx.x == 0) p.dbg_times[6 * (size_t)blockIdx.x + 3] = (long long)__builtin_readcyclecounter();
    if (p.dbg_abl & 2) return;
#endif
    if (p.gn_n > 0 && !atomic) {
      constexpr int GNB = BM / 32;
      unsigned long long* lacc = (unsigned long long*)smem;
      static_assert(2 * GNB * 32 * GN_WORDS * 8 <= LDS_BYTES, "LDS too small for the statistics accumulators");
      __syncthreads();
      for (int e = tid; e < 2 * GNB * 32 * GN_WORDS; e += NT) lacc[e] = 0ull;
      __syncthreads();
      const int b_tile = m0 / HWout;
#pragma unroll
      for (int j = 0; j < TN; ++j) {
        const int n = nw + j * 32 + l31;
        const bool nvalid = n < p.N;
        auto flush = [&](int b, float s1, float s2) {
          if (!nvalid) { s1 = 0.f; s2 = 0.f; }
          s1 += __shfl_xor(s1, 32); s2 += __shfl_xor(s2, 32);
          for (int t = 0; t < p.gn_n; ++t) {
            const int gid = nvalid ? fast_div(p.gn_cbase[t] + n, p.gn_magic[t]) : -1;
            float a1 = s1, a2 = s2;
#pragma unroll
            for (int off = 1; off < 32; off <<= 1) {
              const float t1 = __shfl_down(a1, off, 32), t2 = __shfl_down(a2, off, 32);
              const int tg = __shfl_down(gid, off, 32);
              if (l31 + off < 32 && tg == gid) { a1 += t1; a2 += t2; }
            }
            const int gprev = __shfl_up(gid, 1, 32);
            if (lg == 0 && gid >= 0 && (l31 == 0 || gprev != gid)) {
              unsigned long long* dst = lacc + ((size_t)(t * GNB + (b - b_tile)) * 32 + gid) * GN_WORDS;
              gn_acc_add(dst, a1);
              gn_acc_add(dst + 2, a2);
            }
          }
        };
        float s1 = 0.f, s2 = 0.f;
        int bcur = -1;
#pragma unroll
        for (int i = 0; i < TM; ++i) {
          const int mt = mw + i * 32;
          if (mt < p.M) {
            const int bi = mt / HWout;
            if (bcur >= 0 && bi != bcur) { flush(bcur, s1, s2); s1 = 0.f; s2 = 0.f; }
            bcur = bi;
#pragma unroll
            for (int r = 0; r < 16; ++r) {
              const int m = mt + (r & 3) + 8 * (r >> 2) + 4 * lg;
              if (m < p.M) { const float v = acc[i][j][r]; s1 += v; s2 += v * v; }
            }
          }
        }
        if (bcur >= 0) flush(bcur, s1, s2);
      }
      __syncthreads();
      const int slot = (tile_m + tile_n) & (GN_SLOTS - 1);
      for (int e = tid; e < p.gn_n * GNB * 32 * GN_WORDS; e += NT) {
        const unsigned long long w = lacc[e];
        if (w == 0ull) continue;
        const int word = e % GN_WORDS, g = (e / GN_WORDS) % 32, bl = (e / (GN_WORDS * 32)) % GNB, t = e / (GN_WORDS * 32 * GNB);
        if (b_tile + bl >= p.B) continue;
        atomicAdd((unsigned long long*)p.gn_acc[t] + ((size_t)((b_tile + bl) * 32 + g) * GN_SLOTS + slot) * GN_STRIDE + word, w);
      }
    }
  } else if (p.mode == EPI_GEGLU) {
    if constexpr (TN % 2 == 0) {
#pragma unroll
      for (int j2 = 0; j2 < TN / 2; ++j2) {
        const int nv = nw + (2 * j2) * 32 + l31;
        if (nv >= p.N) continue;
        const float bv = p.bias ? p.bias[nv] : 0.f, bg = p.bias ? p.bias[nv + 32] : 0.f;
        const int oc = (nw >> 1) + j2 * 32 + l31;
        if (full) {
#pragma unroll
          for (int i = 0; i < TM; ++i)
#pragma unroll
            for (int r = 0; r < 16; ++r) {
              const int m = mw + i * 32 + (r & 3) + 8 * (r >> 2) + 4 * lg;
              const float val = acc[i][2 * j2][r] + bv;
              const float gate = acc[i][2 * j2 + 1][r] + bg;
              SDMI_ST(f16, p.out_f16 + (size_t)m * p.ldo + oc, (f16)(val * gelu_erf(gate)));
            }
// ... 105 lines not shown
              if (m >= p.M) continue;
              const int b2 = m / p.ntok;
              const int t2 = m - b2 * p.ntok;
              const size_t bh2 = (size_t)b2 * p.heads + head;
              const size_t off = kind == 0 ? ((bh2 * p.ntok + t2) * p.dh + dd) : ((bh2 * p.dh + dd) * p.ntok_pad + t2);
              dst[off] = (f16)acc[i][j][r4 * 4 + e];
            }
          }
        }
    }
  }
}

#endif

static unsigned long long div_magic(int d) {
  const unsigned long long one = 1ull << 40;
  return (one + (unsigned long long)d - 1) / (unsigned long long)d;
}
static unsigned long long div_magic_hw(int d) {
  const unsigned long long one = 1ull << 48;
  return (one + (unsigned long long)d - 1) / (unsigned long long)d;
}

static int tile_order_n_fastest(const IGemmParams& p) {
  static const int env_order = env_int("SDMI_TILE_ORDER", 0);
  if (env_order == 1) return 0;
  if (env_order == 2) return 1;
  return p.M > p.N ? 1 : 0;
}

static int reduce_rows_per_block(const IGemmParams& p) {
  int rpb = 32;
  const int hw = p.Hout * p.Wout;
  while (rpb < 256 && (int64_t)cdiv(p.N / 4, 8) * cdiv(p.M, rpb * 2) >= 1024 && (p.gn_n == 0 || hw % (rpb * 2) == 0)) rpb *= 2;
  return rpb;
}
static bool slab_tiled_ok(const IGemmParams& p, int bm, int bn, int nsplit) {
  const int on = env_int("SDMI_SLAB_TILED", 1);
  if (!on || nsplit <= 1 || p.mode == EPI_GEGLU || p.N % 4) return false;
  if ((bm & (bm - 1)) || (bn & (bn - 1))) return false;
  if (p.mode == EPI_PLAIN && p.gn_n > 0 && reduce_rows_per_block(p) != 32) return false;
  if (p.lnf_part || p.lnp_out || p.f16_scale) return false;
  if ((int64_t)nsplit * cdiv(p.M, bm) * bm * cdiv(p.N, bn) * bn > p.splitk_ws_floats) return false;
  return true;
}
static void slab_layout(IGemmParams& q, int bm, int bn, int wm, int wn, int nsplit) {
  q.slab_tiled = slab_tiled_ok(q, bm, bn, nsplit) ? 1 : 0;
  q.slab_bm = bm; q.slab_bn = bn; q.slab_wm = wm; q.slab_wn = wn;
  auto lg2 = [](int v) { int s = 0; while ((1 << s) < v) ++s; return s; };
  q.slab_sh_qpt = lg2(bm * bn / 4); q.slab_sh_nt = lg2(wm * wn * 64); q.slab_sh_tn = lg2(bn / wn / 32); q.slab_sh_wn = lg2(wn);
  if (q.slab_tiled && (((wm * wn) & (wm * wn - 1)) || (wn & (wn - 1)))) q.slab_tiled = 0;
}
static int64_t splitk_ws_need(const IGemmParams& p, int bm, int bn, int nsplit) {
  if (nsplit <= 1) return 0;
  if (slab_tiled_ok(p, bm, bn, nsplit)) return (int64_t)nsplit * cdiv(p.M, bm) * bm * cdiv(p.N, bn) * bn;
  return (int64_t)nsplit * p.M * p.N;
}

static int epi_vec_ok(const IGemmParams& p) {
  if (!env_int("SDMI_EPI_VEC", 1) || p.N % 4) return 0;
  auto al = [](const void* q, uintptr_t a) { return ((uintptr_t)q & (a - 1)) == 0; };
  if (p.mode == EPI_PLAIN)
    return p.ldo % 4 == 0 && al(p.out_f32, 16) && al(p.out_f16, 8) && al(p.out_lo, 8) && al(p.bias, 16) &&
           al(p.rowvec, 16) && p.ld_rowvec % 4 == 0 && al(p.residual, 16) && p.ldr % 4 == 0;
  if (p.mode == EPI_GEGLU) return 0;
  return p.segC % 32 == 0 && p.dh % 4 == 0 && al(p.bias, 16) && al(p.seg_dst[0], 8) && al(p.seg_dst[1], 8) && al(p.seg_dst[2], 8);
}

}

bool halo_supported(const IGemmParams& p, int bm);
int launch_halo_tile(int tile, const IGemmParams& p, int splitk, hipStream_t stream);
bool split16_tile_supported(int tile);

int launch_split16_tile(int tile, const IGemmParams& p, int splitk, hipStream_t stream);

}
```

### stable-diffusion_amd/csrc/igemm_kernel.h

```cpp
#pragma once
#include <string>

#include "igemm_dev.h"

namespace sdmi {
namespace {


template <int BM, int BN, int WARPS_M, int WARPS_N, bool DMA, int NS, int KIND, bool HALF = false>
__global__ void __launch_bounds__(WARPS_M* WARPS_N * 64) igemm_kernel(const IGemmParams p, const int tiles_m,
                                                                       const int tiles_n, const int kt_per_split) {
  static_assert(DMA || NS == 2, "the register-staged path is double buffered");
#if defined(__HIP_DEVICE_COMPILE__)
  constexpr bool UP = KIND == KIND_3X3_UP;
  constexpr bool K3 = KIND != KIND_1X1;
  constexpr int NT = WARPS_M * WARPS_N * 64;
  constexpr int RPP = NT / 8;
  constexpr int A_PASSES = BM / RPP;
  constexpr int B_PASSES = BN / RPP;
  constexpr int WTM = BM / WARPS_M, WTN = BN / WARPS_N;
  constexpr int TM = WTM / 32, TN = WTN / 32;
  constexpr int STAGE_BYTES = (BM + BN) * 128;
  static_assert(A_PASSES >= 1 && B_PASSES >= 1 && TM >= 1 && TN >= 1, "tile/wave shape");
  static_assert(RPP % 16 == 0, "swizzle assumes pass offset keeps row bits 1..3");

  __shared__ __attribute__((aligned(16))) unsigned char smem[NS * STAGE_BYTES];

  const int nblk = gridDim.x;
  const int bid = blockIdx.x;
  const int q8 = nblk >> 3, r8 = nblk & 7, xcd = bid & 7;
  const int wgid = (xcd < r8 ? xcd * (q8 + 1) : r8 * (q8 + 1) + (xcd - r8) * q8) + (bid >> 3);
  const int tiles_mn = tiles_m * tiles_n;
  const int split = wgid / tiles_mn;
  const int tmn = wgid - split * tiles_mn;
  int tile_m, tile_n;
  if (p.tile_n_fastest) { tile_m = tmn / tiles_n; tile_n = tmn - tile_m * tiles_n; }
  else { tile_n = tmn / tiles_m; tile_m = tmn - tile_n * tiles_m; }
  const int m0 = tile_m * BM, n0 = tile_n * BN;
  const int nkt = HALF ? p.nkt : p.K / BK;
  const int kt_begin = split * kt_per_split;
  const int kt_end = min(nkt, kt_begin + kt_per_split);
  if (kt_begin >= kt_end) return;

  const int tid = threadIdx.x;
  SDMI_STAMP(dbg_t0);
  float2 lnf_pv[LNF_MAXP];
  float lnf_mean = 0.f, lnf_rstd = 1.f;
  const bool lnf_mine = p.lnf_part != nullptr && tid < BM;
  if (lnf_mine) lnf_request(p, min(m0 + tid, p.M - 1), lnf_pv);
  const int lane = tid & 63;
  const int wave = tid >> 6;
  const int cpos = tid & 7;
  const int lrow = tid >> 3;
  const int gch = cpos ^ ((lrow >> 1) & 7);
  const int hi_oob = (HALF && gch >= 4) ? (int)0x80000000 : 0;

  const int HWout = p.Hout * p.Wout;
  const int pad = K3 ? p.pad : 0;
  constexpr int ntap = K3 ? 9 : 1;
  const int ld = p.lda0;
  int a_off[A_PASSES];
  unsigned a_mask[K3 ? A_PASSES : 1];
  int a_ro[UP ? A_PASSES : 1][3], a_co[UP ? A_PASSES : 1][3];
#pragma unroll
  for (int i = 0; i < A_PASSES; ++i) {
    const int m = min(m0 + i * RPP + lrow, p.M - 1);
    const int b = fast_div_hw(m, p.magic_hw);
    const int rem = m - b * HWout;
    const int oy = fast_div(rem, p.magic_w), ox = rem - oy * p.Wout;
    const int pb = b * p.Hin * p.Win;
    if constexpr (UP) {
      const int Hv = 2 * p.Hin, Wv = 2 * p.Win;
      unsigned mk = 0;
#pragma unroll
      for (int d = 0; d < 3; ++d) {
        const int iy = oy + d - 1, ix = ox + d - 1;
        a_ro[i][d] = (pb + (max(iy, 0) >> 1) * p.Win) * ld * 2;
        a_co[i][d] = ((max(ix, 0) >> 1) * ld + gch * 8) * 2;
      }
#pragma unroll
      for (int t = 0; t < 9; ++t) {
        const int iy = oy + t / 3 - 1, ix = ox + t % 3 - 1;
        if (iy >= 0 && iy < Hv && ix >= 0 && ix < Wv) mk |= 1u << t;
      }
      a_mask[i] = mk | ((HALF && gch < 4) ? mk << 9 : 0u);
      a_off[i] = 0;
    } else {
      const int cy = oy * p.stride, cx = ox * p.stride;
      a_off[i] = ((pb + cy * p.Win + cx) * ld + gch * 8) * 2;
      if constexpr (K3) {
        unsigned mk = 0;
#pragma unroll
        for (int t = 0; t < 9; ++t) {
          const int iy = cy + t / 3 - pad, ix = cx + t % 3 - pad;
          if (iy >= 0 && iy < p.Hin && ix >= 0 && ix < p.Win) mk |= 1u << t;
        }
        a_mask[i] = mk | ((HALF && gch < 4) ? mk << 9 : 0u);
      }
    }
  }
  int b_off[B_PASSES];
#pragma unroll
  for (int i = 0; i < B_PASSES; ++i) {
    const int n = min(n0 + i * RPP + lrow, p.N - 1);
    b_off[i] = (n * p.K + gch * 8) * 2;
  }

  f16x8 regA[DMA ? 1 : A_PASSES], regB[DMA ? 1 : B_PASSES];
  const int wave_u = __builtin_amdgcn_readfirstlane(wave);

  int ld_kt = kt_begin;
  int ld_tap = K3 ? kt_begin % ntap : 0;
  int ld_cin0 = (kt_begin / ntap) * BK;
  int ld_ky = K3 ? ld_tap / 3 : 0, ld_kx = K3 ? ld_tap - 3 * (ld_tap / 3) : 0;
  const int pc0 = p.c0, pc1 = p.c1, pc2 = p.c2;
  const int pp0 = (pc0 + BK - 1) & ~(BK - 1), pp01 = pp0 + ((pc1 + BK - 1) & ~(BK - 1));
  int ld_boff = 0;
  if constexpr (HALF) {
    const int dense0 = ld_cin0 - (ld_cin0 >= pp0 ? pp0 - pc0 : 0) - (ld_cin0 >= pp01 ? pp01 - pp0 - pc1 : 0);
    const int left = ld_cin0 < pp0 ? pc0 - ld_cin0 : (ld_cin0 < pp01 ? pc1 - (ld_cin0 - pp0) : pc2 - (ld_cin0 - pp01));
    ld_boff = (ntap * dense0 + ld_tap * min(left, BK)) * 2;
  }

  constexpr int OOB = (int)0x80000000;
  const long long a_shift = (K3 && !UP) ? (long long)(pad * p.Win + pad) * ld * 2 : 0;
  const char* const srcA0 = (const char*)p.a0 - a_shift; const char* const srcA1 = (const char*)p.a1 - a_shift;
  const char* const srcA2 = (const char*)p.a2 - a_shift;
  const __amdgpu_buffer_rsrc_t rsrc_w = __builtin_amdgcn_make_buffer_rsrc((void*)p.w, 0, OOB, 0x00020000);
  const int pWin = p.Win;

  struct TileCursor { __amdgpu_buffer_rsrc_t rsrc_a; int a_soff, b_soff; unsigned tapbit; int ky, kx; unsigned lds; int half; };
  auto next_tile = [&](int stage) {
    TileCursor c;
    const char* src; int coff, left;
    if (ld_cin0 < pp0) { src = srcA0; coff = ld_cin0; left = pc0 - coff; }
    else if (ld_cin0 < pp01) { src = srcA1; coff = ld_cin0 - pp0; left = pc1 - coff; }
    else { src = srcA2; coff = ld_cin0 - pp01; left = pc2 - coff; }
    const bool half = HALF && left < BK;
    c.rsrc_a = __builtin_amdgcn_make_buffer_rsrc((void*)src, 0, OOB, 0x00020000);
    c.a_soff = ((K3 && !UP) ? (ld_ky * pWin + ld_kx) * ld + coff : coff) * 2;
    c.b_soff = HALF ? ld_boff : ld_kt * (BK * 2);
    c.tapbit = 1u << (half ? ld_tap + 9 : ld_tap); c.ky = ld_ky; c.kx = ld_kx;
    c.half = half ? OOB : 0;
    c.lds = stage * STAGE_BYTES;
    if (ld_kt + 1 < kt_end) {
      ++ld_kt;
      if constexpr (HALF) ld_boff += half ? BKH * 2 : BK * 2;
      if constexpr (K3) {
        ++ld_tap;
        if (++ld_kx == 3) { ld_kx = 0; ++ld_ky; }
        if (ld_tap == ntap) { ld_tap = 0; ld_ky = 0; ld_kx = 0; ld_cin0 += BK; }
      } else {
        ld_cin0 += BK;
      }
    }
    return c;
  };
  auto a_voff = [&](const TileCursor& c, int i) -> int {
    int v;
    if constexpr (UP) v = a_ro[i][c.ky] + a_co[i][c.kx];
    else v = a_off[i];
    if constexpr (K3) v = (a_mask[i] & c.tapbit) ? v : OOB;
    else if constexpr (HALF) v |= hi_oob & c.half;
    return v;
  };
  auto b_voff = [&](const TileCursor& c, int i) -> int { return HALF ? (b_off[i] | (hi_oob & c.half)) : b_off[i]; };
  auto issue_piece = [&](const TileCursor& c, int q) {
    const unsigned row0 = (q < A_PASSES ? q * RPP : BM + (q - A_PASSES) * RPP) + wave_u * 8;
    auto dst = (__attribute__((address_space(3))) void*)(smem + c.lds + row0 * 128);
    if (q < A_PASSES) __builtin_amdgcn_raw_ptr_buffer_load_lds(c.rsrc_a, dst, 16, a_voff(c, q), c.a_soff, 0, 0);
    else __builtin_amdgcn_raw_ptr_buffer_load_lds(rsrc_w, dst, 16, b_voff(c, q - A_PASSES), c.b_soff, 0, SDMI_W_AUX);
  };
  auto issue_loads = [&](int stage) {
    const TileCursor c = next_tile(stage);
#pragma unroll
    for (int q = 0; q < A_PASSES + B_PASSES; ++q) {
      if constexpr (DMA) {
        issue_piece(c, q);
      } else {
        typedef int i32x4 __attribute__((ext_vector_type(4)));
        i32x4 v;
        if (q < A_PASSES) v = __builtin_amdgcn_raw_buffer_load_b128(c.rsrc_a, a_voff(c, q), c.a_soff, 0);
        else v = __builtin_amdgcn_raw_buffer_load_b128(rsrc_w, b_voff(c, q - A_PASSES), c.b_soff, 0);
// ... 75 lines not shown
        }
#pragma unroll
        for (int g = 0; g < G; ++g) mfma_step(fa[u & 1][g], fb[u & 1][g]);
        __builtin_amdgcn_sched_group_barrier(0x100, G * (TM + TN), 0);
#pragma unroll
        for (int e = 0; e < MPU; ++e) {
          __builtin_amdgcn_sched_group_barrier(0x008, 1, 0);
          if (u + 1 < U && e < PPU && u * PPU + e < LPT) __builtin_amdgcn_sched_group_barrier(0x010, 1, 0);
        }
      }
      cur = cur1;
      nxt = (nxt + 1 == NS) ? 0 : nxt + 1;
    }
    wait_vmcnt<0>();
  } else {
    issue_loads(0);
    commit_regs(0);
    for (int kt = kt_begin; kt < kt_end; ++kt) {
      const int cur = (kt - kt_begin) & 1;
      __syncthreads();
      const bool more = (kt + 1 < kt_end);
      if (more) issue_loads(cur ^ 1);
#pragma unroll
      for (int ks = 0; ks < BK / 16; ++ks) {
        f16x8 a[TM], b[TN];
        read_frags(cur, ks, a, b);
        mfma_step(a, b);
      }
      if (more) commit_regs(cur ^ 1);
    }
  }

  SDMI_STAMP(dbg_t2);
  igemm_epilogue<BM, BN, WARPS_M, WARPS_N, NS * STAGE_BYTES>(p, acc, m0, n0, split, tile_m, tile_n, smem, lnf_mean, lnf_rstd);
#ifdef SDMI_IGEMM_TIMING
  if (p.dbg_times && tid == 0) {
    long long* d = p.dbg_times + 6 * (size_t)blockIdx.x;
    d[0] = dbg_t0; d[1] = dbg_t1; d[2] = dbg_t2; d[4] = (long long)__builtin_readcyclecounter();
  }
#endif
#endif
}

template <int BM, int BN, int WARPS_M, int WARPS_N, int NS, bool HALF = false>
int launch_cfg(const IGemmParams& p, bool dma, int splitk, hipStream_t stream) {
  SDMI_CHECK(HALF || (p.c0 % BK == 0 && p.c1 % BK == 0 && p.c2 % BK == 0), "internal: a half k-tile launch on the whole-chunk kernel");
  const int tiles_m = cdiv(p.M, BM), tiles_n = cdiv(p.N, BN);
  const int nkt = igemm_nkt(p);
  const int kt_per_split = cdiv(nkt, splitk);
  const int nsplit = cdiv(nkt, kt_per_split);
  IGemmParams q = p;
  q.nkt = nkt;
  q.splitk = nsplit;
  q.tile_n_fastest = tile_order_n_fastest(p);
  q.splitk_fused = 0;
  slab_layout(q, BM, BN, WARPS_M, WARPS_N, nsplit);
  q.epi_vec = epi_vec_ok(p);
  SDMI_CHECK(splitk_ws_need(p, BM, BN, nsplit) <= p.splitk_ws_floats, "split-K workspace too small");
  SDMI_CHECK((int64_t)p.M < (int64_t)65536 * p.Hout * p.Wout, "fast_div_hw: at most 65535 samples per launch");
  q.magic_hw = div_magic_hw(p.Hout * p.Wout);
  q.magic_w = div_magic(p.Wout);
  for (int t = 0; t < p.gn_n; ++t) q.gn_magic[t] = div_magic(p.gn_cpg[t]);
  dim3 grid(tiles_m * tiles_n * nsplit), block(WARPS_M * WARPS_N * 64);
  static const int by_shape = env_int("SDMI_PROF_SHAPES", 0);
  std::string pname = std::string("igemm_") + std::to_string(BM) + "x" + std::to_string(BN) + "w" +
                      std::to_string(WARPS_M * WARPS_N) + "s" + std::to_string(NS) + (HALF ? "h" : "");
  if (by_shape && prof_enabled())
    pname += "_M" + std::to_string(p.M) + "_N" + std::to_string(p.N) + "_K" + std::to_string(p.K) + "_k" +
             std::to_string(p.ksize) + "_m" + std::to_string(p.mode) + "_s" + std::to_string(nsplit);
  const double src_pix = (double)p.B * p.Hin * p.Win;
  const double out_b = (p.out_f32 ? 4.0 : 0.0) + ((p.out_f16 || p.mode != EPI_PLAIN) ? 2.0 : 0.0);
  const double n_out = p.mode == EPI_GEGLU ? p.N / 2.0 : (double)p.N;
  const int k_alg = p.k_alg > 0 ? p.k_alg : p.K;
  const double cin_alg = p.k_alg > 0 ? (double)p.k_alg : (double)(p.c0 + p.c1 + p.c2);
  ProfScope ps(pname.c_str(), 2.0 * p.M * (double)p.N * k_alg,
               src_pix * cin_alg * 2.0 + (double)p.N * k_alg * 2.0 + (double)p.M * n_out * out_b +
                   (p.residual ? (double)p.M * p.N * 4.0 : 0.0),
               stream, 2.0 * p.M * (double)p.N * p.K);
  const int kind = p.ksize == 1 ? KIND_1X1 : (p.up ? KIND_3X3_UP : KIND_3X3);
#define SDMI_LAUNCH_KIND(K_)                                                                                        \
  do {                                                                                                              \
    if (dma) SDMI_LAUNCH((igemm_kernel<BM, BN, WARPS_M, WARPS_N, true, NS, K_, HALF>), grid, block, 0, stream, q,   \
                                tiles_m, tiles_n, kt_per_split);                                                    \
    else SDMI_LAUNCH((igemm_kernel<BM, BN, WARPS_M, WARPS_N, false, 2, K_, HALF>), grid, block, 0, stream, q,       \
                            tiles_m, tiles_n, kt_per_split);                                                        \
  } while (0)
  if (kind == KIND_1X1) SDMI_LAUNCH_KIND(KIND_1X1);
  else if (kind == KIND_3X3) SDMI_LAUNCH_KIND(KIND_3X3);
  else SDMI_LAUNCH_KIND(KIND_3X3_UP);
#undef SDMI_LAUNCH_KIND
  SDMI_HIP_OK(hipGetLastError());
  ps.end();
  if (nsplit > 1) return launch_splitk_reduce(q, nsplit, stream);
  if (q.ln_out) return launch_layernorm(q.out_f32, q.ln_gamma, q.ln_beta, q.ln_out, q.M, q.N, q.ln_eps, stream);
  return 0;
}

}
}
```

### stable-diffusion_amd/csrc/small.hip

```cpp
#include "common.h"
#include "igemm_dev.h"
#include "prof.h"
#include <math.h>
#include <vector>

namespace sdmi {
namespace {

__global__ void temb_kernel(const int64_t* t_i64, const float* t_f32, const float* freqs, float* out, int B, int dim) {
  const int half = dim / 2;
  const int idx = blockIdx.x * blockDim.x + threadIdx.x;
  if (idx >= B * half) return;
  const int b = idx / half, i = idx - b * half;
  const float t = t_i64 ? (float)t_i64[b] : t_f32[b];
  const float arg = t * freqs[i];
  out[(size_t)b * dim + i] = cosf(arg);
  out[(size_t)b * dim + half + i] = sinf(arg);
  if ((dim & 1) && i == 0) out[(size_t)b * dim + dim - 1] = 0.f;
}

constexpr int SL_MAXB = 8;
__global__ void __launch_bounds__(256) small_linear_kernel(const float* in, int ld_in, const float* w, const float* bias,
                                                           float* out, int ld_out, int B, int N, int K, int silu_in) {
  const int lane = threadIdx.x & 63;
// ... 280 lines not shown
  const int I3 = 3 * I;
  const int64_t K = (int64_t)I3 * KH * KW;
  if (idx >= (int64_t)O * K) return;
  const int o = (int)(idx / K);
  const int64_t k = idx - (int64_t)o * K;
  const int chunk = (int)(k / (64 * KH * KW));
  const int rem = (int)(k - (int64_t)chunk * 64 * KH * KW);
  const int tap = rem / 64;
  const int i3 = chunk * 64 + rem % 64, ky = tap / KW, kx = tap % KW;
  const int part = i3 / I, i = i3 - part * I;
  const float v = w[(((int64_t)o * I + i) * KH + ky) * KW + kx];
  const f16 hi = (f16)v;
  dst[idx] = part < 2 ? hi : (f16)(v - (float)hi);
}
__global__ void pack_conv_src_kernel(const float* w, f16* dst, int O, int I, int KH, int KW, int c0, int c1, int c2, int split3) {
  const int64_t idx = (int64_t)blockIdx.x * blockDim.x + threadIdx.x;
  const int taps = KH * KW;
  const int64_t K = (int64_t)(c0 + c1 + c2) * taps;
  if (idx >= (int64_t)O * K) return;
  const int o = (int)(idx / K);
  const int k = (int)(idx - (int64_t)o * K);
  const int src = k < taps * c0 ? 0 : (k < taps * (c0 + c1) ? 1 : 2);
  const int cs = src == 0 ? c0 : (src == 1 ? c1 : c2), base = src == 0 ? 0 : (src == 1 ? c0 : c0 + c1);
  const int ks = k - taps * base;
  const int chunk = ks / (64 * taps);
  const int rem = ks - chunk * 64 * taps;
  const int wd = min(64, cs - chunk * 64);
  const int tap = rem / wd, ci = chunk * 64 + rem % wd, ky = tap / KW, kx = tap % KW;
  const int i = split3 ? ci : base + ci;
  const float v = w[(((int64_t)o * I + i) * KH + ky) * KW + kx];
  const f16 hi = (f16)v;
  dst[idx] = (!split3 || src < 2) ? hi : (f16)(v - (float)hi);
}
__global__ void pack_conv_f32_kernel(const float* w, float* dst, int O, int I, int KH, int KW) {
  const int64_t idx = (int64_t)blockIdx.x * blockDim.x + threadIdx.x;
  const int64_t total = (int64_t)O * I * KH * KW;
  if (idx >= total) return;
  const int i = (int)(idx % I);
  int64_t r = idx / I;
  const int kx = (int)(r % KW); r /= KW;
  const int ky = (int)(r % KH);
  const int o = (int)(r / KH);
  dst[idx] = w[(((int64_t)o * I + i) * KH + ky) * KW + kx];
}
__global__ void pack_rows_kernel(const float* w, f16* dst, int rows, int cols, int dst_row0, int dst_ld) {
  const int64_t idx = (int64_t)blockIdx.x * blockDim.x + threadIdx.x;
  if (idx >= (int64_t)rows * cols) return;
  const int r = (int)(idx / cols), c = (int)(idx - (int64_t)r * cols);
  dst[(int64_t)(dst_row0 + r) * dst_ld + c] = (f16)w[idx];
}
__global__ void pack_split3_kernel(const float* w, f16* dst, int N, int K) {
  const int64_t idx = (int64_t)blockIdx.x * blockDim.x + threadIdx.x;
  if (idx >= (int64_t)N * K) return;
  const int n = (int)(idx / K), k = (int)(idx - (int64_t)n * K);
  const float v = w[idx];
  const f16 hi = (f16)v;
  const f16 lo = (f16)(v - (float)hi);
  f16* d = dst + (int64_t)n * 3 * K;
  d[k] = hi; d[K + k] = hi; d[2 * K + k] = lo;
}
__global__ void pack_geglu_kernel(const float* w, const float* bias, f16* wdst, float* bdst, int N, int K) {
  const int64_t idx = (int64_t)blockIdx.x * blockDim.x + threadIdx.x;
  if (idx >= (int64_t)N * K) return;
  const int r = (int)(idx / K), c = (int)(idx - (int64_t)r * K);
  const int q = r >> 6, j = r & 63;
  const int src = (j < 32) ? (32 * q + j) : (N / 2 + 32 * q + (j - 32));
// ... 243 lines not shown
int launch_pack_conv_weight(const float* w, f16* dst, int O, int I, int KH, int KW, hipStream_t s) {
  if (KH * KW > 1 && I % 64 != 0) return launch_pack_conv_weight_src(w, dst, O, I, KH, KW, I, 0, 0, s);
  const int64_t total = (int64_t)O * I * KH * KW;
  SDMI_LAUNCH(pack_conv_kernel, dim3((unsigned)((total + 255) / 256)), dim3(256), 0, s, w, dst, O, I, KH, KW);
  SDMI_HIP_OK(hipGetLastError());
  return 0;
}
__global__ void __launch_bounds__(256) prefetch_lines_kernel(const unsigned* p, long long nlines) {
  const long long i = (long long)blockIdx.x * 256 + threadIdx.x;
  if (i >= nlines) return;
  const unsigned v = __builtin_nontemporal_load(p + i * 32);
  asm volatile("" ::"v"(v));
}
int launch_prefetch_lines(const void* ptr, int64_t bytes, hipStream_t s) {
  const long long nlines = bytes / 128;
  if (nlines <= 0) return 0;
  SDMI_LAUNCH(prefetch_lines_kernel, dim3((unsigned)((nlines + 255) / 256)), dim3(256), 0, s, (const unsigned*)ptr, nlines);
  SDMI_HIP_OK(hipGetLastError());
  return 0;
}

int launch_pack_conv_split3(const float* w, f16* dst, int O, int I, int KH, int KW, hipStream_t s) {
  SDMI_CHECK(I % 32 == 0, "split-fp16 conv pack: input channels % 64 must be 0, or 32 (a half k-tile)");
  const int64_t total = (int64_t)O * 3 * I * KH * KW;
  if (I % 64 != 0) {
    SDMI_LAUNCH(pack_conv_src_kernel, dim3((unsigned)((total + 255) / 256)), dim3(256), 0, s, w, dst, O, I, KH, KW, I, I, I, 1);
    SDMI_HIP_OK(hipGetLastError());
    return 0;
  }
  SDMI_LAUNCH(pack_conv_split3_kernel, dim3((unsigned)((total + 255) / 256)), dim3(256), 0, s, w, dst, O, I, KH, KW);
  SDMI_HIP_OK(hipGetLastError());
  return 0;
}
int launch_pack_conv_out(const float* w, float* dst, int O, int I, hipStream_t s) {
  const int64_t total = (int64_t)O * I * 9;
  SDMI_LAUNCH(pack_conv_f32_kernel, dim3((unsigned)((total + 255) / 256)), dim3(256), 0, s, w, dst, O, I, 3, 3);
  SDMI_HIP_OK(hipGetLastError());
  return 0;
}
int launch_pack_rows(const float* w, f16* dst, int rows, int cols, int dst_row0, int dst_ld, hipStream_t s) {
  const int64_t total = (int64_t)rows * cols;
  SDMI_LAUNCH(pack_rows_kernel, dim3((unsigned)((total + 255) / 256)), dim3(256), 0, s, w, dst, rows, cols,
                     dst_row0, dst_ld);
  SDMI_HIP_OK(hipGetLastError());
  return 0;
}

__global__ void __launch_bounds__(256) ln_fold_prep_kernel(const f16* w, int N, int K, int ldw, const float* gamma, const float* beta,
                                                           const float* bias, float* cs, float* d) {
  const int lane = threadIdx.x & 63;
  const int n = blockIdx.x * 4 + (threadIdx.x >> 6);
  if (n >= N) return;
  const f16* row = w + (size_t)n * ldw;
  float a = 0.f, b = 0.f;
  for (int k = lane; k < K; k += 64) { const float wv = (float)row[k]; a = fmaf(gamma[k], wv, a); b = fmaf(beta[k], wv, b); }
#pragma unroll
  for (int o = 32; o >= 1; o >>= 1) { a += __shfl_xor(a, o); b += __shfl_xor(b, o); }
  if (lane == 0) { cs[n] = a; d[n] = b + (bias ? bias[n] : 0.f); }
}
int launch_ln_fold_prep(const f16* w, int N, int K, int ldw, const float* gamma, const float* beta, const float* bias, float* cs,
                        float* d, hipStream_t s) {
  SDMI_CHECK(w && gamma && beta && cs && d && N > 0 && K > 0 && ldw >= K, "ln_fold_prep: bad arguments");
  SDMI_LAUNCH(ln_fold_prep_kernel, dim3((unsigned)cdiv(N, 4)), dim3(256), 0, s, w, N, K, ldw, gamma, beta, bias, cs, d);
  SDMI_HIP_OK(hipGetLastError());
  return 0;
}
// ... 16 lines not shown
```

### stable-diffusion_amd/csrc/unet.cpp

```cpp
#include "unet.h"

extern "C" char** environ;
#include "prof.h"
#include "split16.h"

#include <math.h>
#include <stdio.h>
#include <string.h>

#include <algorithm>

namespace sdmi {

static bool in_list(const int* v, int n, int x) {
  for (int i = 0; i < n; ++i)
    if (v[i] == x) return true;
  return false;
}

thread_local Tape* g_tape_rec = nullptr;

namespace {
uint64_t sdmi_env_hash() {
  uint64_t h = 1469598103934665603ull;
// ... 185 lines not shown
          store_.expect(t + ".attn2.to_v.weight", {C, CD}, precise_kv_ ? W_SPLIT3_ROWS : W_ROWS16, &T.wkv2, (int)C, 2 * (int)C);
          store_.expect(t + ".attn2.to_out.0.weight", {C, C}, lin, &T.wo2);
          store_.expect(t + ".attn2.to_out.0.bias", {C}, W_F32, &T.bo2);
          store_.expect(t + ".ff.net.0.proj.weight", {8 * C, C}, full() ? W_SPLIT3 : W_GEGLU_W, &T.wgg);
          store_.expect(t + ".ff.net.0.proj.bias", {8 * C}, full() ? W_F32 : W_GEGLU_B, &T.bgg);
          store_.expect(t + ".ff.net.2.weight", {C, 4 * C}, lin, &T.wff2);
          store_.expect(t + ".ff.net.2.bias", {C}, W_F32, &T.bff2);
          store_.expect(t + ".norm1.weight", {C}, W_F32, &T.ln[0]);
          store_.expect(t + ".norm1.bias", {C}, W_F32, &T.ln[1]);
          store_.expect(t + ".norm2.weight", {C}, W_F32, &T.ln[2]);
          store_.expect(t + ".norm2.bias", {C}, W_F32, &T.ln[3]);
          store_.expect(t + ".norm3.weight", {C}, W_F32, &T.ln[4]);
          store_.expect(t + ".norm3.bias", {C}, W_F32, &T.ln[5]);
        }
        break;
      }
      case L_ATTN_LEGACY: {
        const int64_t C = ci;
        const bool pq = L.p1x1;
        store_.expect(p + ".norm.weight", {C}, W_F32, &L.f32[0]);
        store_.expect(p + ".norm.bias", {C}, W_F32, &L.f32[1]);
        WeightSlot& qkv = store_.expect(p + ".qkv.weight", {3 * C, C, 1}, W_QKV_LEGACY, &L.w16[0]);
        qkv.heads = L.heads; qkv.split = pq;
        store_.expect(p + ".qkv.bias", {3 * C}, W_QKV_LEGACY_B, &L.f32[2]).heads = L.heads;
        store_.expect(p + ".proj_out.weight", {C, C, 1}, full() ? W_SPLIT3 : W_ROWS16, &L.w16[1]);
        store_.expect(p + ".proj_out.bias", {C}, W_F32, &L.f32[3]);
        break;
      }
      case L_DOWN:
        store_.expect(p + ".op.weight", {co, ci, 3, 3}, full() ? W_CONV_SPLIT3 : W_CONV, &L.w16[0]);
        store_.expect(p + ".op.bias", {co}, W_F32, &L.f32[0]);
        break;
      case L_UP:
        store_.expect(p + ".conv.weight", {co, ci, 3, 3}, full() ? W_CONV_SPLIT3 : W_CONV, &L.w16[0]);
        store_.expect(p + ".conv.bias", {co}, W_F32, &L.f32[0]);
        break;
    }
    return 0;
  });
  store_.expect("out.0.weight", {mc}, W_F32, &out_gamma_);
  store_.expect("out.0.bias", {mc}, W_F32, &out_beta_);
  store_.expect("out.2.weight", {c.out_channels, mc, 3, 3}, W_CONV_OUT, &out_w_);
  store_.expect("out.2.bias", {c.out_channels}, W_F32, &out_b_);
  return 0;
}

UNet::~UNet() {
  if (emb_tab_) (void)hipFree(emb_tab_);
  if (emb_tab_tdev_) (void)hipFree(emb_tab_tdev_);
  for_each_layer([](Layer& L) -> int {
    for (auto& T : L.tb) {
      if (T.ck) (void)hipFree(T.ck);
      if (T.cvt) (void)hipFree(T.cvt);
      if (T.ck_lo) (void)hipFree(T.ck_lo);
      if (T.cvt_lo) (void)hipFree(T.cvt_lo);
    }
    return 0;
  });
}

int UNet::set_weight(const char* key, const float* ptr, const int64_t* shape, int ndim, hipStream_t stream) {
  if (int rc = store_.set(key, ptr, shape, ndim, stream)) return rc;
  ++weights_gen_;
  finalized_ = false;
  ctx_valid_ = false;
  drop_timestep_table();
  return 0;
// ... 79 lines not shown
  }
  SDMI_HIP_OK(hipStreamSynchronize(stream));
  return 0;
}

int UNet::import_packed(const void* host_buf, int64_t bytes, hipStream_t stream) {
  SDMI_CHECK(host_buf && bytes >= (int64_t)sizeof(PackedHeader), "packed blob truncated");
  PackedHeader h;
  memcpy(&h, host_buf, sizeof(h));
  SDMI_CHECK(memcmp(h.magic, "SDMIPK01", 8) == 0, "not a libsdmi packed-weight blob");
  SDMI_CHECK(h.abi == SDMI_ABI_VERSION, "packed blob was written by a different ABI version: repack it");
  SDMI_CHECK(memcmp(&h.cfg, &cfg_, sizeof(cfg_)) == 0, "packed blob was written for a different UNet configuration");
  SDMI_CHECK(((h.reserved & PK_FULL) != 0) == full(), std::string("packed blob was written by a ") +
             ((h.reserved & PK_FULL) ? "full" : "mixed") + "-precision UNet handle and cannot be imported into a " + (full() ? "full" : "mixed") +
             "-precision one: repack it with a handle of this precision");
  SDMI_CHECK((h.precise_1x1 != 0) == precise_1x1_, "packed blob was written with a different precision allocation (split-fp16 1x1 convs)");
  SDMI_CHECK((h.reserved & (7 << 4)) == ((ext_.attention_block << 4) | (ext_.resblock_updown << 5) | ((scale_shift_ ? 1 : 0) << 6)),
             "packed blob was written for a different UNet family (attention_block / resblock_updown / scale-shift norm)");
  SDMI_CHECK(((h.reserved & PK_NHC_MASK) >> PK_NHC_SHIFT) == num_head_channels_,
             "packed blob was written for num_head_channels " + std::to_string((h.reserved & PK_NHC_MASK) >> PK_NHC_SHIFT) + ", this handle has " +
             std::to_string(num_head_channels_) + ": repack it");
  SDMI_CHECK((h.reserved & ~PK_FULL & ~(7 << 4) & ~PK_NHC_MASK) == ((precise_kv_ ? 1 : 0) | (precise_last_res_ ? 2 : 0) | (precise_1x1_max_ds_ << 8)),
             "packed blob was written with a different precision allocation (context K / V, last ResBlock, 1x1 conv levels)");
  std::vector<std::pair<void**, size_t>> bufs;
  int64_t total = 0;
  packed_layout(&bufs, &total);
  SDMI_CHECK(h.n_buffers == (int32_t)bufs.size() && h.total_bytes == total && bytes >= total, "packed blob truncated or inconsistent");
  int64_t off = (int64_t)round_up((int64_t)sizeof(PackedHeader), PK_ALIGN);
  for (auto& b : bufs) {
    if (store_.alloc(b.first, b.second)) return -1;
    SDMI_HIP_OK(hipMemcpyAsync(*b.first, (const char*)host_buf + off, b.second, hipMemcpyHostToDevice, stream));
    off += (int64_t)round_up((int64_t)b.second, PK_ALIGN);
  }
  SDMI_HIP_OK(hipStreamSynchronize(stream));
  store_.mark_all_set();
  ctx_valid_ = false;
  drop_timestep_table();
  return finalize();
}

struct Fwd : FwdBase {
  UNet* u; int Lctx;
  bool ln_fold_on = false;
  bool ff_tail_on = false;
  bool st_head_on = false;
  bool st_mid_on = false;
  bool st_tail_on = false;
  bool st_mid_ctx_on = false;
  bool ctx1_on = false;
  bool gn_conv_on = false;
  float* emb_all = nullptr;
  int emb_ld = 0;
  bool emb_caller = false;
  const f16* ctx16 = nullptr;
  const f16* ctx16_lo = nullptr;

  Act res_block(Layer& L, const Act& x0, const Act* x1) {
    const int H = x0.H, W = x0.W, M = B * H * W;
    const int Cin = x0.C + (x1 ? x1->C : 0), Cout = L.cout;
    if (Cin != L.cin) { ok(fail("res block channel mismatch at " + L.prefix)); }
    if (Cin == Cout && x1) ok(fail("identity skip with a concatenated input at " + L.prefix));
    const size_t mark = scratch.off;
    f16* raw = (Cin != Cout) ? S<f16>((size_t)M * Cin) : nullptr;
    const bool p1 = L.p1x1;
    const bool p3 = L.precise3;
    f16* raw_lo = (Cin != Cout && p1) ? S<f16>((size_t)M * Cin) : nullptr;
// ... 309 lines not shown
  }

  Act resample(Layer& L, const Act& x, bool up) {
    const int Hin = x.H, Win = x.W, C = x.C;
    const int Hout = up ? 2 * Hin : (Hin - 1) / 2 + 1, Wout = up ? 2 * Win : (Win - 1) / 2 + 1;
    const size_t mark = scratch.off;
    if (u->full()) {
      const int64_t n = (int64_t)B * Hin * Win * C;
      f16* hi = S<f16>((size_t)n); f16* lo = S<f16>((size_t)n);
      if (!dry && !rc) ok(launch_cast_f16(x.p, hi, lo, n, s));
      Act out = make_act(P<float>((size_t)B * Hout * Wout * C), L.cout, Hout, Wout, true);
      IGemmParams p = conv3(hi, C, Hin, Win, Hout, Wout, up ? 1 : 2, up ? 1 : 0, L.w16[0], L.cout);
      split3(p, hi, lo, C);
      p.bias = L.f32[0]; p.out_f32 = out.p; p.ldo = L.cout;
      attach_gn_targets(p, out);
      gemm(p);
      scratch.off = mark;
      return out;
    }
    const f16* x16 = nullptr;
    if (dry) { if (!want_f16_copy(x)) (void)S<f16>((size_t)B * Hin * Win * C); }
    else {
      x16 = f16_copy(x);
      if (!x16) {
        f16* c = S<f16>((size_t)B * Hin * Win * C);
        if (!rc) ok(launch_cast_f16(x.p, c, nullptr, (int64_t)B * Hin * Win * C, s));
        x16 = c;
      }
    }
    Act out = make_act(P<float>((size_t)B * Hout * Wout * C), L.cout, Hout, Wout, true);
    IGemmParams p = conv3(x16, C, Hin, Win, Hout, Wout, up ? 1 : 2, up ? 1 : 0, L.w16[0], L.cout);
    p.bias = L.f32[0]; p.out_f32 = out.p; p.ldo = L.cout;
    attach_gn_targets(p, out);
    gemm(p);
    scratch.off = mark;
    return out;
  }

  Act res_block_updown(Layer& L, const Act& x) {
    const int dir = L.updown, H = x.H, W = x.W, C = L.cin;
    if (x.C != C || L.cout != C) ok(fail("resampling res block channel mismatch at " + L.prefix));
    if (dir > 0 && ((H | W) & 1)) ok(fail("resampling res block at " + L.prefix + ": the 2x2 average pool needs even H and W"));
    const int Ho = dir > 0 ? H / 2 : 2 * H, Wo = dir > 0 ? W / 2 : 2 * W, M = B * Ho * Wo;
    const bool p3 = L.precise3;
    const bool ss = u->scale_shift_;
    const float* const film = ss ? emb_all + L.emb_off : nullptr;
    const size_t mark = scratch.off;
    float* g = S<float>((size_t)B * H * W * C);
    groupnorm(x, nullptr, L.f32[0], L.f32[1], 1e-5f, 1, nullptr, g, nullptr);
    f16* a = S<f16>((size_t)M * C);
    f16* a_lo = p3 ? S<f16>((size_t)M * C) : nullptr;
    float* xs = S<float>((size_t)M * C);
    if (!dry && !rc) ok(launch_resample2(g, nullptr, a, a_lo, B, H, W, C, dir, s));
    if (!dry && !rc) ok(launch_resample2(x.p, xs, nullptr, nullptr, B, H, W, C, dir, s));
    float* h = S<float>((size_t)M * C);
    Act out = make_act(P<float>((size_t)M * C), C, Ho, Wo, true);
    Act hact = make_act(h, C, Ho, Wo, true);
    {
      IGemmParams p = conv3(a, C, Ho, Wo, Ho, Wo, 1, 0, L.w16[0], C);
      if (p3) split3(p, a, a_lo, C);
      p.bias = L.f32[2];
      if (!ss) { p.rowvec = emb_all + L.emb_off; p.ld_rowvec = emb_ld; }
      p.out_f32 = h; p.ldo = C;
      attach_gn_targets(p, hact);
      TapeCaller tc(Tape::R_EMB, emb_caller ? p.rowvec : nullptr);
      gemm(p);
// ... 220 lines not shown
    fresh.reset(new Tape());
    memcpy(fresh->caller, caller, sizeof(caller));
    rec = fresh.get();
  }

  Fwd f;
  f.u = this; f.s = stream; f.dry = dry; f.B = B; f.Lctx = Lctx; f.zero = store_.zero(); f.precise_1x1 = precise_1x1_;
  {
    const char* e_fold = getenv("SDMI_LN_FOLD"); const char* e_vec = getenv("SDMI_EPI_VEC");
    f.ln_fold_on = (e_fold ? atoi(e_fold) != 0 : ln_fold_) && !(e_vec && atoi(e_vec) == 0);
    const char* e_ff = getenv("SDMI_FF_TAIL");
    f.ff_tail_on = e_ff ? atoi(e_ff) != 0 : ff_tail_;
    const char* e_sh = getenv("SDMI_ST_HEAD");
    f.st_head_on = e_sh ? atoi(e_sh) != 0 : st_head_;
    const char* e_sm = getenv("SDMI_ST_MID");
    f.st_mid_on = e_sm ? atoi(e_sm) != 0 : st_head_;
    const char* e_st = getenv("SDMI_ST_TAIL");
    f.st_tail_on = e_st ? atoi(e_st) != 0 : ff_tail_;
    const char* e_mc = getenv("SDMI_ST_MID_CTX");
    f.st_mid_ctx_on = e_mc ? atoi(e_mc) != 0 : st_head_;
    const char* e_c1 = getenv("SDMI_CTX1");
    f.ctx1_on = !(e_c1 && atoi(e_c1) == 0);
    const char* e_gc = getenv("SDMI_GN_CONV");
    f.gn_conv_on = e_gc ? atoi(e_gc) != 0 : false;
    if (full()) {
      f.ln_fold_on = f.ff_tail_on = f.st_head_on = f.st_mid_on = f.st_tail_on = f.st_mid_ctx_on = f.gn_conv_on = false;
    }
  }
  int64_t persist_bytes = 0, scratch_bytes = 0;
  for (int pass = 0; pass < 2; ++pass) {
    const bool d = (pass == 0) ? true : false;
    if (pass == 1 && dry) break;
    f.dry = d; f.rc = 0;
    f.n_acts = 0;
    TapeRecGuard tape_guard(d ? nullptr : rec);
    f.plan = fuse_gn_stats_ ? &gn_plan_ : nullptr;
    if (d) gn_plan_.clear();
    f.persist = Arena(); f.scratch = Arena();
    f.persist.dry = f.scratch.dry = d;
    if (!d) {
      SDMI_CHECK(persist_bytes + scratch_bytes <= ws_bytes, "workspace too small: need " +
                 std::to_string(persist_bytes + scratch_bytes) + " bytes, got " + std::to_string(ws_bytes));
      SDMI_CHECK(workspace != nullptr, "workspace is NULL");
      f.persist.base = (char*)workspace; f.persist.cap = (size_t)persist_bytes;
      f.scratch.base = (char*)workspace + persist_bytes; f.scratch.cap = (size_t)scratch_bytes;
      if (ensure_ctx_cache(B, Lctx, ctx_only)) return -1;
    }
    const int mc = cfg_.model_channels;
    if (f.begin_pass((int64_t)12 << 20)) return -1;
    f16* ctx16 = f.P<f16>((size_t)B * Lctx * cfg_.context_dim);
    f16* ctx16_lo = precise_kv_ ? f.P<f16>((size_t)B * Lctx * cfg_.context_dim) : nullptr;
    const bool have_ctx = has_ctx() && ((ctx != nullptr) || d);
    if (!has_ctx()) {
      f.ctx16 = nullptr; f.ctx16_lo = nullptr;
    } else if (have_ctx) {
      if (!d) {
        TapeCaller tc(Tape::R_CTX, ctx);
        int r = launch_cast_f16(ctx, ctx16, ctx16_lo, (int64_t)B * Lctx * cfg_.context_dim, stream);
        if (r) return r;
      }
      f.ctx16 = ctx16; f.ctx16_lo = ctx16_lo;
    } else {
      SDMI_CHECK(ctx_valid_, "ctx == NULL but no cached context for this (B, Lctx); call sdmi_unet_cache_context first");
      f.ctx16 = nullptr; f.ctx16_lo = nullptr;
    }
    if (ctx_only) {
      for_each_layer([&](Layer& L) -> int {
// ... 100 lines not shown
```

### stable-diffusion_amd/csrc/unet.h

```cpp
#pragma once
#include <stdlib.h>

#include <memory>
#include <string>
#include <utility>
#include <vector>

#include "../../include/sdmi.h"
#include "common.h"
#include "weights.h"

namespace sdmi {

struct Arena {
  char* base = nullptr; size_t cap = 0, off = 0, peak = 0; bool dry = false; bool overflow = false;
  void* alloc(size_t bytes) {
    const size_t a = (off + 255) & ~(size_t)255;
    off = a + bytes;
    peak = std::max(peak, off);
    if (dry) return (void*)(uintptr_t)(a + 4096);
    if (off > cap) { overflow = true; return base; }
    return base + a;
  }
};
// ... 70 lines not shown
  int begin_pass(int64_t splitk_floats, bool with_gn = true) {
    gn_calls = 0;
    gn_acc = nullptr;
    const size_t acc_words = with_gn ? (size_t)GN_MAX_CALLS * gn_acc_words(B) : 0;
    long long* blk = P<long long>(acc_words + SPLITK_CNT_INTS / 2);
    gn_acc = with_gn ? blk : nullptr;
    splitk_cnt = (int*)(blk + acc_words);
    if (!dry) SDMI_HIP_OK(memset_async(blk, 0, (acc_words + SPLITK_CNT_INTS / 2) * sizeof(long long), s));
    splitk_ws_floats = splitk_floats;
    splitk_ws = P<float>((size_t)splitk_floats);
    (void)P<float>((size_t)(splitk_floats / 2));
    return 0;
  }

  void gemm(IGemmParams& p) {
    p.zero_page = zero;
    p.splitk_ws = splitk_ws; p.splitk_ws_floats = splitk_ws_floats;
    p.splitk_cnt = splitk_cnt; p.splitk_cnt_ints = SPLITK_CNT_INTS;
    if (!dry && !rc) ok(launch_igemm(p, IGemmTune(), s));
  }
  IGemmParams dense(const f16* a, int M, int K, const f16* w, int N, int rows_per_batch) {
    IGemmParams p = IGemmParams();
    p.a0 = a; p.c0 = K; p.lda0 = K;
    p.B = M / rows_per_batch; p.Hin = p.Hout = rows_per_batch; p.Win = p.Wout = 1;
    p.ksize = 1; p.w = w; p.M = M; p.N = N; p.K = K; p.splitk = 0;
    return p;
  }
  IGemmParams conv3(const f16* a, int C, int Hin, int Win, int Hout, int Wout, int stride, int up, const f16* w, int N) {
    IGemmParams p = IGemmParams();
    p.a0 = a; p.c0 = C; p.lda0 = C;
    p.B = B; p.Hin = Hin; p.Win = Win; p.Hout = Hout; p.Wout = Wout;
    p.ksize = 3; p.stride = stride; p.up = up; p.w = w; p.M = B * Hout * Wout; p.N = N; p.K = 9 * C; p.splitk = 0;
    return p;
  }
  static void split3(IGemmParams& p, const f16* hi, const f16* lo, int C) {
    p.a0 = hi; p.c0 = C; p.lda0 = C; p.a1 = lo; p.c1 = C; p.lda1 = C; p.a2 = hi; p.c2 = C; p.lda2 = C;
    p.k_alg = p.ksize * p.ksize * C; p.K = 3 * p.k_alg;
  }
  IGemmParams dense1x1(const f16* hi, const f16* lo, int M, int K, const f16* w, int N, int rows_per_batch, bool precise) {
    IGemmParams p = dense(hi, M, K, w, N, rows_per_batch);
    if (precise) {
      static const bool family = !(getenv("SDMI_SPLIT16_KERNEL") && atoi(getenv("SDMI_SPLIT16_KERNEL")) == 0);
      if (family && K % 32 == 0) { p.a1 = lo; p.lda1 = K; p.split16 = 1; p.ldw = 3 * K; }
      else split3(p, hi, lo, K);
    }
    return p;
  }
  long long* groupnorm(const Act& x0, const Act* x1, const float* gamma, const float* beta, float eps, int silu, f16* o16,
                       float* o32, f16* raw, f16* o16_lo = nullptr, f16* raw_lo = nullptr, bool stats_only = false,
                       bool already_applied = false, const float* film = nullptr, int film_ld = 0) {
    GroupNormParams g = GroupNormParams();
    g.film = film; g.film_ld = film_ld;
    g.x0 = x0.p; g.c0 = x0.C;
    if (x1) { g.x1 = x1->p; g.c1 = x1->C; }
    g.B = B; g.HW = x0.H * x0.W; g.gamma = gamma; g.beta = beta; g.eps = eps; g.silu = silu;
    g.out_f16 = o16; g.out_f32 = o32; g.raw_f16 = raw; g.out_lo = o16_lo; g.raw_lo = raw_lo;
    g.stats_only = stats_only ? 1 : 0;
    const int idx = gn_calls;
    g.acc = next_gn_acc();
    if (plan) {
      const int cpg = (g.c0 + g.c1) / 32;
      if (dry) {
        const bool f = x0.stats && (!x1 || x1->stats) && x0.id >= 0 && (!x1 || x1->id >= 0);
        if ((int)plan->fused.size() <= idx) plan->fused.resize(idx + 1, 0);
        plan->fused[idx] = f ? 1 : 0;
        if (f) {
// ... 128 lines not shown
```

### stable-diffusion_amd/csrc/vae.cpp

```cpp
#include "vae.h"

#include "split16.h"

#include <math.h>

#include <algorithm>

namespace sdmi {

int Vae::build(const sdmi_vae_cfg& c, int parts, const sdmi_vae_ext* ext, int precision) {
  cfg_ = c; parts_ = parts; precision_ = precision;
  if (ext) ext_ = *ext;
  SDMI_CHECK((ext_.double_z == 0 || ext_.double_z == 1) && (ext_.mid_attn == 0 || ext_.mid_attn == 1) && ext_.n_embed >= 0,
             "first-stage extension: double_z and mid_attn are 0 or 1, n_embed >= 0");
  SDMI_CHECK(ext_.n_embed == 0 || (c.embed_dim == 1 || c.embed_dim == 2 || c.embed_dim == 3 || c.embed_dim == 4 || c.embed_dim == 8),
             "codebook quantizer: embed_dim must be 1, 2, 3, 4 or 8");
  SDMI_CHECK(parts >= 1 && parts <= 3, "parts: 1 decoder, 2 encoder, 3 both");
  SDMI_CHECK(c.n_levels >= 1 && c.n_levels <= 8 && c.num_res_blocks >= 1, "bad level / res block count");
  SDMI_CHECK(c.ch % 64 == 0, "ch must be a multiple of 64 on this path");
  SDMI_CHECK(c.in_channels >= 1 && c.in_channels <= 16 && c.z_channels >= 1 && c.z_channels <= 4 && c.embed_dim >= 1 &&
                 c.embed_dim <= 8 && c.out_ch >= 1 && c.out_ch <= 8,
             "in_channels <= 16, z_channels <= 4, embed_dim <= 8, out_ch <= 8 on this path");
  const int n = c.n_levels;
  if (full() && ext_.mid_attn) {
// ... 38 lines not shown
    enc_c_end_ = bi;
  }

  auto visit = [&](VLayer& L) {
    const std::string& p = L.prefix;
    const int64_t ci = L.cin, co = L.cout;
    switch (L.kind) {
      case V_RES:
        store_.expect(p + ".norm1.weight", {ci}, W_F32, &L.f32[0]);
        store_.expect(p + ".norm1.bias", {ci}, W_F32, &L.f32[1]);
        store_.expect(p + ".conv1.weight", {co, ci, 3, 3}, conv_kind, &L.w16[0]);
        store_.expect(p + ".conv1.bias", {co}, W_F32, &L.f32[2]);
        store_.expect(p + ".norm2.weight", {co}, W_F32, &L.f32[3]);
        store_.expect(p + ".norm2.bias", {co}, W_F32, &L.f32[4]);
        store_.expect(p + ".conv2.weight", {co, co, 3, 3}, conv_kind, &L.w16[1]);
        store_.expect(p + ".conv2.bias", {co}, W_F32, &L.f32[5]);
        if (ci != co) {
          store_.expect(p + ".nin_shortcut.weight", {co, ci, 1, 1}, (precise_1x1_ || full()) ? W_SPLIT3 : W_ROWS16, &L.w16[2]);
          store_.expect(p + ".nin_shortcut.bias", {co}, W_F32, &L.f32[6]);
        }
        break;
      case V_ATTN: {
        store_.expect(p + ".norm.weight", {ci}, W_F32, &L.f32[0]);
        store_.expect(p + ".norm.bias", {ci}, W_F32, &L.f32[1]);
        const char* names[4] = {"q", "k", "v", "proj_out"};
        for (int i = 0; i < 4; ++i) {
          store_.expect(p + "." + names[i] + ".weight", {ci, ci, 1, 1}, lin_kind, &L.w16[i]);
          store_.expect(p + "." + names[i] + ".bias", {ci}, W_F32, &L.f32[2 + i]);
        }
        break;
      }
      case V_UP:
      case V_DOWN:
        store_.expect(p + ".conv.weight", {co, ci, 3, 3}, conv_kind, &L.w16[0]);
        store_.expect(p + ".conv.bias", {co}, W_F32, &L.f32[0]);
        break;
    }
  };
  if (parts & 2) {
    store_.expect("encoder.conv_in.weight", {c.ch, c.in_channels, 3, 3}, W_F32, &eci_w_);
    store_.expect("encoder.conv_in.bias", {c.ch}, W_F32, &eci_b_);
    for (auto& L : enc_) visit(L);
    store_.expect("encoder.norm_out.weight", {enc_c_end_}, W_F32, &eno_g_);
    store_.expect("encoder.norm_out.bias", {enc_c_end_}, W_F32, &eno_b_);
    store_.expect("encoder.conv_out.weight", {enc_zc(), enc_c_end_, 3, 3}, W_CONV_OUT, &eco_w_);
    store_.expect("encoder.conv_out.bias", {enc_zc()}, W_F32, &eco_b_);
    store_.expect("quant_conv.weight", {enc_ed(), enc_zc(), 1, 1}, W_F32, &q_w_);
    store_.expect("quant_conv.bias", {enc_ed()}, W_F32, &q_b_);
  }
  if (parts & 1) {
    if (ext_.n_embed > 0) store_.expect("quantize.embedding.weight", {ext_.n_embed, c.embed_dim}, W_F32, &cb_);
    store_.expect("post_quant_conv.weight", {c.z_channels, c.embed_dim, 1, 1}, W_F32, &pq_w_);
    store_.expect("post_quant_conv.bias", {c.z_channels}, W_F32, &pq_b_);
    store_.expect("decoder.conv_in.weight", {c.ch * c.ch_mult[n - 1], c.z_channels, 3, 3}, W_F32, &dci_w_);
    store_.expect("decoder.conv_in.bias", {c.ch * c.ch_mult[n - 1]}, W_F32, &dci_b_);
    for (auto& L : dec_) visit(L);
    store_.expect("decoder.norm_out.weight", {dec_c_end_}, W_F32, &dno_g_);
    store_.expect("decoder.norm_out.bias", {dec_c_end_}, W_F32, &dno_b_);
    store_.expect("decoder.conv_out.weight", {c.out_ch, dec_c_end_, 3, 3}, W_CONV_OUT, &dco_w_);
    store_.expect("decoder.conv_out.bias", {c.out_ch}, W_F32, &dco_b_);
  }
  return 0;
}

int Vae::set_weight(const char* key, const float* ptr, const int64_t* shape, int ndim, hipStream_t stream) {
  if (int rc = store_.set(key, ptr, shape, ndim, stream)) return rc;
  finalized_ = false;
// ... 125 lines not shown
        }
        if (!dry && !rc) ok(launch_softmax_rows(Sm, Pm, rows, N, N, N, scale, s));
        {
          IGemmParams p = dense(Pm, rows, N, vt + (size_t)b * N * C, C, rows);
          p.bias = L.f32[4]; p.out_f16 = ao + ((size_t)b * N + r0) * C; p.ldo = C; p.splitk = 1;
          gemm(p);
        }
      }
    }
    Act out; out.p = P<float>((size_t)M * C); out.C = C; out.H = H; out.W = W;
    {
      IGemmParams p = dense(ao, M, C, L.w16[3], C, N);
      p.bias = L.f32[5]; p.residual = x.p; p.ldr = C; p.out_f32 = out.p; p.ldo = C;
      gemm(p);
    }
    scratch.off = mark;
    return out;
  }

  Act resample(VLayer& L, const Act& x, bool up) {
    const int Hin = x.H, Win = x.W, C = x.C;
    if (!up && ((Hin | Win) & 1)) ok(fail("first-stage Downsample needs even H and W"));
    const int Hout = up ? 2 * Hin : Hin / 2, Wout = up ? 2 * Win : Win / 2;
    const size_t mark = scratch.off;
    const int64_t n = (int64_t)B * Hin * Win * C;
    f16* x16 = S<f16>((size_t)n);
    f16* x16_lo = full ? S<f16>((size_t)n) : nullptr;
    if (!dry && !rc) ok(launch_cast_f16(x.p, x16, x16_lo, n, s));
    Act out; out.p = P<float>((size_t)B * Hout * Wout * C); out.C = C; out.H = Hout; out.W = Wout;
    IGemmParams p = conv3(x16, C, Hin, Win, Hout, Wout, up ? 1 : 2, up ? 1 : 0, L.w16[0], C);
    if (full) split3(p, x16, x16_lo, C);
    if (!up) p.pad = 0;
    p.bias = L.f32[0]; p.out_f32 = out.p; p.ldo = C;
    gemm(p);
    scratch.off = mark;
    return out;
  }

  Act run_layer(VLayer& L, const Act& x) {
    switch (L.kind) {
      case V_RES: return res_block(L, x);
      case V_ATTN: return full ? attn_block_full(L, x) : attn_block(L, x);
      case V_UP: return resample(L, x, true);
      case V_DOWN: return resample(L, x, false);
    }
    return x;
  }
};

template <class Body>
static int run_two_pass(VFwd& f, bool dry, void* workspace, int64_t ws_bytes, int64_t* bytes_needed, Body body) {
  int64_t persist_bytes = 0, scratch_bytes = 0;
  for (int pass = 0; pass < 2; ++pass) {
    const bool d = pass == 0;
    if (pass == 1 && dry) break;
    f.dry = d; f.rc = 0;
    f.persist = Arena(); f.scratch = Arena();
    f.persist.dry = f.scratch.dry = d;
    if (!d) {
      SDMI_CHECK(persist_bytes + scratch_bytes <= ws_bytes, "workspace too small: need " +
                 std::to_string(persist_bytes + scratch_bytes) + " bytes, got " + std::to_string(ws_bytes));
      SDMI_CHECK(workspace != nullptr, "workspace is NULL");
      f.persist.base = (char*)workspace; f.persist.cap = (size_t)persist_bytes;
      f.scratch.base = (char*)workspace + persist_bytes; f.scratch.cap = (size_t)scratch_bytes;
    }
    if (f.begin_pass((int64_t)8 << 20)) return -1;
// ... 72 lines not shown
```

### stable-diffusion_amd/csrc/weights.cpp

```cpp
#include "weights.h"

namespace sdmi {

int DevStage::acquire(const float* ptr, int64_t numel, hipStream_t stream) {
  dptr = ptr;
  hipPointerAttribute_t attr;
  hipError_t e = hipPointerGetAttributes(&attr, ptr);
  const bool on_device = (e == hipSuccess) && (attr.type == hipMemoryTypeDevice || attr.type == hipMemoryTypeManaged);
  if (e != hipSuccess) (void)hipGetLastError();
  if (!on_device) {
    SDMI_HIP_OK(hipMalloc((void**)&staged, numel * sizeof(float)));
    SDMI_HIP_OK(hipMemcpyAsync(staged, ptr, numel * sizeof(float), hipMemcpyHostToDevice, stream));
    dptr = staged;
  }
  return 0;
}
int DevStage::release(hipStream_t stream) {
  if (staged) {
    SDMI_HIP_OK(hipStreamSynchronize(stream));
    (void)hipFree(staged);
    staged = nullptr;
  }
  return 0;
}

WeightStore::~WeightStore() {
  for (void* p : owned_) (void)hipFree(p);
}

static size_t numel_of(const WeightSlot& s) {
  size_t n = 1;
  for (int64_t d : s.shape) n *= (size_t)d;
  return n;
}

WeightSlot& WeightStore::expect(const std::string& key, std::vector<int64_t> shape, WKind kind, void* dst, int row0, int buf_rows) {
  WeightSlot s;
  s.key = key; s.shape = std::move(shape); s.kind = kind; s.dst = (void**)dst; s.row0 = row0;
  s.ld = (int)(numel_of(s) / (size_t)s.shape[0]);
  s.buf_rows = buf_rows ? buf_rows : (int)s.shape[0];
  index_[key] = (int)slots_.size();
  slots_.push_back(std::move(s));
  return slots_.back();
}

size_t WeightStore::bytes(const WeightSlot& s) {
  const size_t numel = numel_of(s), rows = (size_t)s.buf_rows * s.ld;
  switch (s.kind) {
    case W_F32: case W_CONV_OUT: case W_GEGLU_B: case W_QKV_LEGACY_B: return numel * sizeof(float);
    case W_F32_ROWS: return rows * sizeof(float);
    case W_CONV: case W_GEGLU_W: return numel * sizeof(f16);
    case W_SPLIT3: case W_CONV_SPLIT3: return 3 * numel * sizeof(f16);
    case W_QKV_LEGACY: return numel * sizeof(f16) * (s.split ? 3 : 1);
    case W_ROWS16: return rows * sizeof(f16);
    case W_SPLIT3_ROWS: return 3 * rows * sizeof(f16);
    case W_DROP: return 0;
  }
  return 0;
}

int WeightStore::alloc(void** dst, size_t bytes) {
  if (*dst) return 0;
  SDMI_HIP_OK(hipMalloc(dst, bytes));
  owned_.push_back(*dst);
  return 0;
}

int WeightStore::zero_page() {
  if (zero_) return 0;
  if (alloc((void**)&zero_, 4096)) return -1;
  SDMI_HIP_OK(hipMemset(zero_, 0, 4096));
  return 0;
}

const WeightSlot* WeightStore::missing() const {
  for (const auto& s : slots_)
    if (!s.set && s.kind != W_DROP) return &s;
  return nullptr;
}

std::vector<std::pair<void**, size_t>> WeightStore::buffers() const {
  std::vector<std::pair<void**, size_t>> bufs;
  for (const auto& s : slots_) {
    if (s.kind == W_DROP) continue;
    bool seen = false;
    for (const auto& b : bufs) seen = seen || b.first == s.dst;
    if (!seen) bufs.push_back({s.dst, bytes(s)});
  }
  return bufs;
}

int WeightStore::set(const char* key, const float* ptr, const int64_t* shape, int ndim, hipStream_t stream) {
  auto it = index_.find(key);
  if (it == index_.end()) return fail(std::string("unexpected weight key: ") + key);
  WeightSlot& s = slots_[it->second];
  SDMI_CHECK((int)s.shape.size() == ndim, std::string("rank mismatch for ") + key);
  int64_t numel = 1;
  for (int i = 0; i < ndim; ++i) {
    SDMI_CHECK(shape[i] == s.shape[i], std::string("shape mismatch for ") + key);
    numel *= shape[i];
  }
  if (s.kind == W_DROP) {
    s.set = true;
    return 0;
  }
  DevStage st;
  if (st.acquire(ptr, numel, stream)) return -1;
  const float* dptr = st.dptr;
  int rc = alloc(s.dst, bytes(s));
  if (!rc) switch (s.kind) {
    case W_F32:
      SDMI_HIP_OK(hipMemcpyAsync(*s.dst, dptr, numel * sizeof(float), hipMemcpyDeviceToDevice, stream));
      break;
    case W_F32_ROWS:
      SDMI_HIP_OK(hipMemcpyAsync((float*)*s.dst + (size_t)s.row0 * s.ld, dptr, numel * sizeof(float), hipMemcpyDeviceToDevice, stream));
      break;
    case W_CONV:
      rc = launch_pack_conv_weight(dptr, (f16*)*s.dst, (int)shape[0], (int)shape[1], (int)shape[2], (int)shape[3], stream);
      break;
    case W_SPLIT3:
      rc = launch_pack_split3(dptr, (f16*)*s.dst, (int)shape[0], (int)shape[1], stream);
      break;
    case W_CONV_SPLIT3:
      rc = launch_pack_conv_split3(dptr, (f16*)*s.dst, (int)shape[0], (int)shape[1], (int)shape[2], (int)shape[3], stream);
      break;
    case W_SPLIT3_ROWS:
      rc = launch_pack_split3(dptr, (f16*)*s.dst + (size_t)s.row0 * 3 * s.ld, (int)shape[0], (int)shape[1], stream);
      break;
    case W_CONV_OUT:
      rc = launch_pack_conv_out(dptr, (float*)*s.dst, (int)shape[0], (int)shape[1], stream);
      break;
    case W_ROWS16:
      rc = launch_pack_rows(dptr, (f16*)*s.dst, (int)shape[0], (int)shape[1], s.row0, s.ld, stream);
      break;
    case W_QKV_LEGACY:
    case W_QKV_LEGACY_B: {
      const int R = (int)shape[0], K = s.ld, C = R / 3, d = C / s.heads;
      float* perm = nullptr;
      if (s.kind == W_QKV_LEGACY) SDMI_HIP_OK(hipMalloc((void**)&perm, (size_t)R * K * sizeof(float)));
      float* dst = s.kind == W_QKV_LEGACY ? perm : (float*)*s.dst;
      for (int h = 0; h < s.heads; ++h)
        for (int j = 0; j < 3; ++j)
          SDMI_HIP_OK(hipMemcpyAsync(dst + ((size_t)j * C + (size_t)h * d) * K, dptr + ((size_t)h * 3 * d + (size_t)j * d) * K,
                                     (size_t)d * K * sizeof(float), hipMemcpyDeviceToDevice, stream));
      if (s.kind == W_QKV_LEGACY)
        rc = s.split ? launch_pack_split3(perm, (f16*)*s.dst, R, K, stream) : launch_pack_rows(perm, (f16*)*s.dst, R, K, 0, K, stream);
      if (perm) {
        SDMI_HIP_OK(hipStreamSynchronize(stream));
        (void)hipFree(perm);
      }
      break;
    }
// ... 22 lines not shown
```

### stable-diffusion_amd/csrc/weights.h

```cpp
#pragma once
#include <map>
#include <string>
#include <utility>
#include <vector>

#include "common.h"

namespace sdmi {

struct DevStage {
  const float* dptr = nullptr; float* staged = nullptr;
  int acquire(const float* ptr, int64_t numel, hipStream_t stream);
  int release(hipStream_t stream);
};

enum WKind { W_F32, W_F32_ROWS, W_CONV, W_CONV_OUT, W_ROWS16, W_GEGLU_W, W_GEGLU_B, W_SPLIT3, W_SPLIT3_ROWS, W_CONV_SPLIT3, W_QKV_LEGACY,
             W_QKV_LEGACY_B, W_DROP };

struct WeightSlot {
  std::string key;
  std::vector<int64_t> shape;
  WKind kind = W_F32;
  void** dst = nullptr;
  int row0 = 0;
  int ld = 0;
  int buf_rows = 0;
  int heads = 0;
  bool split = false;
  bool set = false;
};

class WeightStore {
 public:
  WeightStore() = default;
  ~WeightStore();
  WeightStore(const WeightStore&) = delete;
  WeightStore& operator=(const WeightStore&) = delete;

  WeightSlot& expect(const std::string& key, std::vector<int64_t> shape, WKind kind, void* dst, int row0 = 0, int buf_rows = 0);
  int set(const char* key, const float* ptr, const int64_t* shape, int ndim, hipStream_t stream);
  static size_t bytes(const WeightSlot& s);
  const WeightSlot* missing() const;
  void mark_all_set() { for (auto& s : slots_) s.set = true; }
  int alloc(void** dst, size_t bytes);
  int zero_page();
  const f16* zero() const { return zero_; }
  std::vector<std::pair<void**, size_t>> buffers() const;
  const std::vector<WeightSlot>& slots() const { return slots_; }

 private:
  std::vector<WeightSlot> slots_;
  std::map<std::string, int> index_;
  std::vector<void*> owned_;
  f16* zero_ = nullptr;
};

}
```

Before: 3.817.

## Decompose nearest-upsample 3x3 convs into four 2x2 phase convs

Adds an up=2 implicit-GEMM mode that replaces the 3x3 conv over a nearest-upsampled image with four 2x2 sub-pixel phase convolutions over the source image. The phase weights are derived at load time by summing the taps that collapse onto each phase, so K falls from 9*C to 4*C per output pixel. The epilogue and split-K reduction scatter rows to the interleaved output positions. This targets the wasted MACs in the UNet and VAE upsample convs, at the cost of extra weight memory, strided output writes, a loss of the cooperative GroupNorm reduce path on these convs, and summing weights in fp16.

```diff
diff --git a/include/sdmi.h b/include/sdmi.h
--- a/include/sdmi.h
+++ b/include/sdmi.h
@@ -227,6 +227,7 @@
 int sdmi_k_pack_conv_out(const float* w_oihw, float* dst_ohwi, int O, int I, void* stream);
 int sdmi_k_pack_split3(const float* w, void* dst_f16, int N, int K, void* stream);
 int sdmi_k_pack_conv_split3(const float* w_oihw, void* dst_f16, int O, int I, int KH, int KW, void* stream);
+int sdmi_k_pack_conv_up_phase(const float* w_oihw, void* dst_f16, int O, int I, void* stream);
 int sdmi_k_pointwise_nchw(const float* x, const float* w, const float* bias, float* out, int B, int Cin, int Cout, int HW,
                           float in_scale, void* stream);
 int sdmi_k_softmax_rows(const float* S, void* P_f16, int rows, int cols, float scale, void* stream);
diff --git a/stable-diffusion_amd/_lib.py b/stable-diffusion_amd/_lib.py
--- a/stable-diffusion_amd/_lib.py
+++ b/stable-diffusion_amd/_lib.py
@@ -165,6 +165,7 @@
     'sdmi_k_pack_conv_out': (C.c_int, [c_ptr, c_ptr, C.c_int, C.c_int, c_ptr]),
     'sdmi_k_pack_split3': (C.c_int, [c_ptr, c_ptr, C.c_int, C.c_int, c_ptr]),
     'sdmi_k_pack_conv_split3': (C.c_int, [c_ptr, c_ptr, C.c_int, C.c_int, C.c_int, C.c_int, c_ptr]),
+    'sdmi_k_pack_conv_up_phase': (C.c_int, [c_ptr, c_ptr, C.c_int, C.c_int, c_ptr]),
     'sdmi_k_pack_geglu': (C.c_int, [c_ptr, c_ptr, c_ptr, c_ptr, C.c_int, C.c_int, c_ptr]),
     'sdmi_k_ln_fold_prep': (C.c_int, [c_ptr, C.c_int, C.c_int, C.c_int, c_ptr, c_ptr, c_ptr, c_ptr, c_ptr, c_ptr]),
     'sdmi_image_to_uint8': (C.c_int, [c_ptr, c_ptr, C.c_int, C.c_int, C.c_int, C.c_int, c_ptr]),
diff --git a/stable-diffusion_amd/csrc/api.cpp b/stable-diffusion_amd/csrc/api.cpp
--- a/stable-diffusion_amd/csrc/api.cpp
+++ b/stable-diffusion_amd/csrc/api.cpp
@@ -328,6 +328,7 @@
   p.B = d->B; p.Hin = d->Hin; p.Win = d->Win; p.Hout = d->Hout; p.Wout = d->Wout;
   p.ksize = d->ksize; p.stride = d->stride; p.up = d->up; p.pad = d->asym_pad ? 0 : 1;
   p.w = (const f16*)d->w; p.M = d->B * d->Hout * d->Wout; p.N = d->N; p.K = d->ksize * d->ksize * (d->c0 + d->c1 + d->c2);
+  if (d->up == 2) p.K = 4 * d->c0;
   p.mode = d->mode; p.bias = d->bias; p.rowvec = d->rowvec; p.ld_rowvec = d->ld_rowvec;
   p.residual = d->residual; p.ldr = d->ldr; p.out_f32 = d->out_f32; p.out_f16 = (f16*)d->out_f16; p.ldo = d->ldo;
   for (int i = 0; i < 3; ++i) { p.seg_dst[i] = (f16*)d->seg_dst[i]; p.seg_kind[i] = d->seg_kind[i]; }
@@ -513,6 +514,9 @@
 int sdmi_k_pack_split3(const float* w, void* dst, int N, int K, void* stream) {
   return launch_pack_split3(w, (f16*)dst, N, K, (hipStream_t)stream);
 }
+int sdmi_k_pack_conv_up_phase(const float* w, void* dst, int O, int I, void* stream) {
+  return launch_pack_conv_up_phase(w, nullptr, (f16*)dst, O, I, (hipStream_t)stream);
+}
 int sdmi_k_pack_conv_split3(const float* w, void* dst, int O, int I, int KH, int KW, void* stream) {
   return launch_pack_conv_split3(w, (f16*)dst, O, I, KH, KW, (hipStream_t)stream);
 }
diff --git a/stable-diffusion_amd/csrc/common.h b/stable-diffusion_amd/csrc/common.h
--- a/stable-diffusion_amd/csrc/common.h
+++ b/stable-diffusion_amd/csrc/common.h
@@ -347,6 +347,7 @@
 int launch_pack_split3(const float* w, f16* dst, int N, int K, hipStream_t s);
 int launch_pack_conv_weight_src(const float* w_oihw, f16* dst, int O, int I, int KH, int KW, int c0, int c1, int c2, hipStream_t s);
 int launch_pack_conv_split3(const float* w, f16* dst, int O, int I, int KH, int KW, hipStream_t s);
+int launch_pack_conv_up_phase(const float* w_oihw, const f16* w9, f16* dst, int O, int I, hipStream_t s);
 int launch_pack_geglu(const float* w, const float* bias, f16* wdst, float* bdst, int N, int K, hipStream_t s);
 int launch_pack_conv_out(const float* w_oihw, float* dst, int O, int I, hipStream_t s);
 
diff --git a/stable-diffusion_amd/csrc/igemm.hip b/stable-diffusion_amd/csrc/igemm.hip
--- a/stable-diffusion_amd/csrc/igemm.hip
+++ b/stable-diffusion_amd/csrc/igemm.hip
@@ -15,7 +15,9 @@
   const int tx = threadIdx.x & 7, ty = threadIdx.x >> 3;
   const int n = (blockIdx.x * 8 + tx) * 4;
   const int row0 = blockIdx.y * rows_per_block;
-  const int HW = p.Hout * p.Wout;
+  const bool up2 = p.up == 2;
+  const int Msrc = up2 ? p.M >> 2 : p.M;
+  const int HW = up2 ? p.Hin * p.Win : p.Hout * p.Wout;
   const bool gn = p.gn_n > 0;
   const bool ncol = n < p.N;
   if (gn) {
@@ -37,7 +39,9 @@
     if (!ncol || m >= p.M) continue;
     const float* src = p.splitk_ws + (size_t)m * p.N + n;
     f32x4 rvv = {0.f, 0.f, 0.f, 0.f}, resv = {0.f, 0.f, 0.f, 0.f};
-    if (p.rowvec) rvv = *(const f32x4*)(p.rowvec + (size_t)(m / HW) * p.ld_rowvec + n);
+    const int ph = up2 ? m / Msrc : 0, ms = m - ph * Msrc;
+    const size_t mo = up2 ? up2_out_row(p.Hin, p.Win, ms, ph) : (size_t)m;
+    if (p.rowvec) rvv = *(const f32x4*)(p.rowvec + (size_t)(ms / HW) * p.ld_rowvec + n);
     if (p.residual) resv = *(const f32x4*)(p.residual + (size_t)m * p.ldr + n);
     f32x4 part[16];
 #pragma unroll
@@ -48,13 +52,13 @@
     v += biasv;
     if (p.rowvec) v += rvv;
     if (p.residual) v += resv;
-    if (p.out_f32) SDMI_ST_F32X4(p.out_f32, (size_t)m * p.ldo + n, v);
-    if (p.out_f16) SDMI_ST_F16X4(p.out_f16, (size_t)m * p.ldo + n, (f16x4{(f16)v[0], (f16)v[1], (f16)v[2], (f16)v[3]}));
+    if (p.out_f32) SDMI_ST_F32X4(p.out_f32, mo * p.ldo + n, v);
+    if (p.out_f16) SDMI_ST_F16X4(p.out_f16, mo * p.ldo + n, (f16x4{(f16)v[0], (f16)v[1], (f16)v[2], (f16)v[3]}));
     if (p.out_lo) {
       f16x4 lo;
 #pragma unroll
       for (int j = 0; j < 4; ++j) lo[j] = (f16)(v[j] - (float)(f16)v[j]);
-      *(f16x4*)(p.out_lo + (size_t)m * p.ldo + n) = lo;
+      *(f16x4*)(p.out_lo + mo * p.ldo + n) = lo;
     }
     if (gn) {
 #pragma unroll
@@ -75,7 +79,7 @@
       }
     }
     __syncthreads();
-    const int b = row0 / HW;
+    const int b = (row0 % Msrc) / HW;
     const int slot = (blockIdx.x + blockIdx.y) & (GN_SLOTS - 1);
     for (int e = threadIdx.x; e < p.gn_n * 32 * GN_WORDS; e += 256) {
       const unsigned long long w = (&s_gn[0][0][0])[e];
@@ -142,7 +146,7 @@
   }
   *a1 = s1; *a2 = s2; *c1 = t1; *c2 = t2;
 }
-struct TiledQuad { size_t off; int m, n; bool valid; };
+struct TiledQuad { size_t off; size_t orow; int m, n; bool valid; };
 __device__ __forceinline__ TiledQuad tiled_quad(const IGemmParams& p, int q, int lane) {
   const int BM = p.slab_bm, BN = p.slab_bn;
   const int WTM = BM / p.slab_wm, WTN = BN >> p.slab_sh_wn;
@@ -156,9 +160,18 @@
   const int l31 = lane & 31, lg = lane >> 5;
   TiledQuad t;
   t.off = (size_t)tile * (size_t)(BM * BN) + (size_t)rem * 4;
-  t.m = tile_m * BM + wm * WTM + i * 32 + 8 * r4 + 4 * lg + (l31 & 3);
+  const int m_in = wm * WTM + i * 32 + 8 * r4 + 4 * lg + (l31 & 3);
   t.n = tile_n * BN + wn * WTN + j * 32 + (l31 & ~3);
-  t.valid = t.m < p.M && t.n < p.N;
+  if (p.up == 2) {
+    const int Msrc = p.M >> 2, tiles_ph = (Msrc + BM - 1) / BM, phase = tile_m / tiles_ph;
+    t.m = (tile_m - phase * tiles_ph) * BM + m_in;
+    t.valid = t.m < Msrc && t.n < p.N;
+    t.orow = up2_out_row(p.Hin, p.Win, min(t.m, Msrc - 1), phase);
+  } else {
+    t.m = tile_m * BM + m_in;
+    t.valid = t.m < p.M && t.n < p.N;
+    t.orow = (size_t)min(t.m, p.M - 1);
+  }
   return t;
 }
 #ifndef SDMI_REDUCE_GN_XCD_DEFAULT
@@ -176,11 +189,13 @@
     __syncthreads();
   }
   const TiledQuad t = tiled_quad(p, blockIdx.x * NTB + tid, lane);
-  const int ntiles = ((p.M + p.slab_bm - 1) / p.slab_bm) * ((p.N + p.slab_bn - 1) / p.slab_bn);
+  const int ntiles = igemm_tiles_m(p, p.slab_bm) * ((p.N + p.slab_bn - 1) / p.slab_bn);
   const size_t split_stride = (size_t)ntiles * (size_t)(p.slab_bm * p.slab_bn);
   const float* src = p.splitk_ws + t.off;
-  const int HW = p.Hout * p.Wout;
-  const int m = min(t.m, p.M - 1), n = min(t.n, p.N - 4);
+  const int HW = p.up == 2 ? p.Hin * p.Win : p.Hout * p.Wout;
+  const int Mrows = p.up == 2 ? p.M >> 2 : p.M;
+  const int m = min(t.m, Mrows - 1), n = min(t.n, p.N - 4);
+  const size_t mo = t.orow;
   f32x4 biasv = {0.f, 0.f, 0.f, 0.f}, rvv = {0.f, 0.f, 0.f, 0.f}, resv = {0.f, 0.f, 0.f, 0.f};
   if (p.bias) biasv = *(const f32x4*)(p.bias + n);
   if (p.rowvec) rvv = *(const f32x4*)(p.rowvec + (size_t)(m / HW) * p.ld_rowvec + n);
@@ -196,13 +211,13 @@
   if (p.rowvec) v += rvv;
   if (p.residual) v += resv;
   if (t.valid) {
-    if (p.out_f32 && (!COOP || p.pgn_keep_f32)) SDMI_ST_F32X4(p.out_f32, (size_t)m * p.ldo + n, v);
-    if (p.out_f16) SDMI_ST_F16X4(p.out_f16, (size_t)m * p.ldo + n, (f16x4{(f16)v[0], (f16)v[1], (f16)v[2], (f16)v[3]}));
+    if (p.out_f32 && (!COOP || p.pgn_keep_f32)) SDMI_ST_F32X4(p.out_f32, mo * p.ldo + n, v);
+    if (p.out_f16) SDMI_ST_F16X4(p.out_f16, mo * p.ldo + n, (f16x4{(f16)v[0], (f16)v[1], (f16)v[2], (f16)v[3]}));
     if (p.out_lo) {
       f16x4 lo;
 #pragma unroll
       for (int j = 0; j < 4; ++j) lo[j] = (f16)(v[j] - (float)(f16)v[j]);
-      *(f16x4*)(p.out_lo + (size_t)m * p.ldo + n) = lo;
+      *(f16x4*)(p.out_lo + mo * p.ldo + n) = lo;
     }
   }
   if (gn) {
@@ -226,7 +241,7 @@
       const int word = e % GN_WORDS, g = (e / GN_WORDS) % 32, w4 = (e / (GN_WORDS * 32)) % NWV, tg = e / (GN_WORDS * 32 * NWV);
       if (w4 * 64 >= NTB) continue;
       const TiledQuad t0 = tiled_quad(p, blockIdx.x * NTB + w4 * 64, 0);
-      if (t0.m >= p.M) continue;
+      if (t0.m >= Mrows) continue;
       const int b = t0.m / HW;
       atomicAdd((unsigned long long*)p.gn_acc[tg] + ((size_t)(b * 32 + g) * GN_SLOTS + slot) * GN_STRIDE + word, w);
     }
@@ -322,7 +337,7 @@
 int launch_splitk_reduce(const IGemmParams& p, int nsplit, hipStream_t stream) {
   SDMI_CHECK(nsplit >= 1 && nsplit <= 16 && p.N % 4 == 0 && p.splitk_ws, "splitk_reduce: bad arguments");
   if (p.slab_tiled) {
-    const int64_t quads = (int64_t)cdiv(p.M, p.slab_bm) * cdiv(p.N, p.slab_bn) * (p.slab_bm * p.slab_bn / 4);
+    const int64_t quads = (int64_t)igemm_tiles_m(p, p.slab_bm) * cdiv(p.N, p.slab_bn) * (p.slab_bm * p.slab_bn / 4);
     SDMI_CHECK(quads % 256 == 0 && quads / 256 < (1ll << 31) && p.slab_wm > 0 && p.slab_wn > 0, "tiled split-K slabs: bad geometry");
     const double mn = (double)p.M * p.N;
     if (p.mode == EPI_HEADS) {
@@ -331,8 +346,8 @@
       SDMI_HIP_OK(hipGetLastError());
       return 0;
     }
-    if (p.gn_n > 0) SDMI_CHECK((p.Hout * p.Wout) % 32 == 0, "GroupNorm statistics need Hout*Wout % 32 == 0");
-    const bool coop = env_int("SDMI_REDUCE_GN_XCD", SDMI_REDUCE_GN_XCD_DEFAULT) && p.pgn_out && p.pgn_gamma && p.pgn_beta && p.mode == EPI_PLAIN && p.gn_n == 1 &&
+    if (p.gn_n > 0) SDMI_CHECK((p.up == 2 ? p.Hin * p.Win : p.Hout * p.Wout) % 32 == 0, "GroupNorm statistics need Hout*Wout % 32 == 0");
+    const bool coop = env_int("SDMI_REDUCE_GN_XCD", SDMI_REDUCE_GN_XCD_DEFAULT) && p.up != 2 && p.pgn_out && p.pgn_gamma && p.pgn_beta && p.mode == EPI_PLAIN && p.gn_n == 1 &&
                       p.gn_cbase[0] == 0 && p.gn_cpg[0] == p.N / 32 && p.N % 128 == 0 && p.N / 32 >= 16 && p.M == p.B * p.Hout * p.Wout &&
                       (p.Hout * p.Wout) % 32 == 0 && !p.out_f16 && !p.out_lo && !p.ln_out && p.splitk_cnt && p.splitk_cnt_ints >= COOP_BAR_INTS &&
                       quads % 1024 == 0 && quads / 1024 <= 256 && (!p.pgn_keep_f32 || (p.out_f32 && p.ldo % 4 == 0));
@@ -360,7 +375,7 @@
     SDMI_HIP_OK(hipGetLastError());
     return 0;
   }
-  const int hw = p.Hout * p.Wout;
+  const int hw = p.up == 2 ? p.Hin * p.Win : p.Hout * p.Wout;
   if (p.gn_n > 0) SDMI_CHECK(hw % 32 == 0, "GroupNorm statistics need Hout*Wout % 32 == 0");
   const int rpb = reduce_rows_per_block(p);
   ProfScope ps2("splitk_reduce", 0.0, (double)p.M * p.N * 4.0 * (nsplit + 1), stream);
@@ -468,6 +483,11 @@
     loaded = true;
     if (env_int("SDMI_TUNE_DISABLE", 0)) return;
     load_file(default_path());
+    if (!getenv("SDMI_TUNE_FILE")) {
+      std::string p2 = default_path();
+      const size_t dot = p2.rfind(".txt");
+      if (dot != std::string::npos) load_file(p2.substr(0, dot) + "_up2.txt");
+    }
   }
   hipEvent_t ev() {
     if (!pool.empty()) { hipEvent_t e = pool.back(); pool.pop_back(); return e; }
@@ -489,8 +509,8 @@
     if (!p.split16 && ((c.ns == 2 && t != 11 && !tile_is_halo(t)) || t == 12 || t == 13)) continue;
     if (p.mode == EPI_GEGLU && !tile_tn_even(t)) continue;
     if (p.lnp_out && (p.M % c.bm || p.N % c.bn || (p.Hout * p.Wout) % c.bm)) continue;
-    const long blocks = (long)cdiv(p.M, c.bm) * cdiv(p.N, c.bn);
-    if ((long)c.bm > 2L * p.M && c.bm > 64) continue;
+    const long blocks = (long)igemm_tiles_m(p, c.bm) * cdiv(p.N, c.bn);
+    if ((long)c.bm > 2L * (p.up == 2 ? p.M / 4 : p.M) && c.bm > 64) continue;
     if ((long)c.bn > 2L * p.N && c.bn > 64) continue;
     for (int sk : splits) {
       if ((sk == 5 || sk == 10) && !tile_is_halo(t)) continue;
@@ -590,7 +610,18 @@
   SDMI_CHECK(p.M > 0 && p.N > 0 && p.K > 0, "empty GEMM");
   SDMI_CHECK(p.ksize == 1 || p.ksize == 3, "ksize must be 1 or 3");
   const int Cin = p.c0 + p.c1 + p.c2;
-  SDMI_CHECK(p.K == p.ksize * p.ksize * Cin, "K != ksize^2 * (c0 + c1 + c2)");
+  SDMI_CHECK(p.up == 0 || p.up == 1 || p.up == 2, "up must be 0, 1 (nine taps over the upsampled image) or 2 (four 2x2 phase convs)");
+  if (p.up == 2) {
+    SDMI_CHECK(p.K == 4 * p.c0 && p.c0 % BK == 0 && p.c1 == 0 && p.c2 == 0 && !p.split16, "up = 2: one source of whole 64-channel chunks, K = 4 * c0");
+    SDMI_CHECK(p.ksize == 3 && p.stride == 1 && p.pad == 1 && p.Hout == 2 * p.Hin && p.Wout == 2 * p.Win, "up = 2: a 3x3 stride-1 conv, output = 2 x input");
+    SDMI_CHECK(p.mode == EPI_PLAIN && !p.residual && !p.ln_out && !p.lnf_part && !p.lnp_out && !p.f16_scale && !p.pgn_out,
+               "up = 2: plain epilogue only (no GEGLU, head scatter, LayerNorm fold / post-op, residual, GroupNorm apply)");
+    SDMI_CHECK((int64_t)((int64_t)p.B * p.Hin * p.Win + 2 * p.Win + 2) * p.lda0 * 2 < ((int64_t)1 << 31) - 65536 && (int64_t)4 * p.N * p.K * 2 < ((int64_t)1 << 31) - 65536,
+               "up = 2: tensor too large for 31-bit byte offsets");
+    if (p.gn_n) SDMI_CHECK((p.Hin * p.Win) % 32 == 0, "up = 2: GroupNorm statistics need Hin*Win % 32 == 0");
+  } else {
+    SDMI_CHECK(p.K == p.ksize * p.ksize * Cin, "K != ksize^2 * (c0 + c1 + c2)");
+  }
   SDMI_CHECK(p.c0 % BKH == 0 && p.c1 % BKH == 0 && p.c2 % BKH == 0 && p.c0 > 0, "channel counts of every A source must be multiples of 32");
   SDMI_CHECK((p.c2 == 0 || p.c1 > 0), "third A source without a second");
   SDMI_CHECK(p.lda0 % 8 == 0 && (p.a1 == nullptr || p.lda1 % 8 == 0), "A row pitch must be a multiple of 8 halves");
diff --git a/stable-diffusion_amd/csrc/igemm_dev.h b/stable-diffusion_amd/csrc/igemm_dev.h
--- a/stable-diffusion_amd/csrc/igemm_dev.h
+++ b/stable-diffusion_amd/csrc/igemm_dev.h
@@ -26,7 +26,15 @@
 static inline bool igemm_has_half(const IGemmParams& p) { return p.split16 ? (p.K % BK != 0) : (p.c0 % BK || p.c1 % BK || p.c2 % BK); }
 static inline int igemm_nkt(const IGemmParams& p) {
   if (p.split16) return src_chunks(p.K);
+  if (p.up == 2) return 4 * src_chunks(p.c0);
   return p.ksize * p.ksize * (src_chunks(p.c0) + src_chunks(p.c1) + src_chunks(p.c2));
+}
+__host__ __device__ static inline int igemm_tiles_m(const IGemmParams& p, int bm) {
+  return p.up == 2 ? 4 * ((p.M / 4 + bm - 1) / bm) : (p.M + bm - 1) / bm;
+}
+__host__ __device__ static inline size_t up2_out_row(int Hin, int Win, int ms, int phase) {
+  const int b = ms / (Hin * Win), rem = ms - b * (Hin * Win), y = rem / Win, x = rem - y * Win;
+  return ((size_t)b * (2 * Hin) + (size_t)(2 * y + (phase >> 1))) * (size_t)(2 * Win) + (size_t)(2 * x + (phase & 1));
 }
 
 #ifdef SDMI_IGEMM_TIMING
@@ -67,7 +75,7 @@
   wait_vmcnt_n(N);
 }
 
-enum : int { KIND_1X1 = 0, KIND_3X3 = 1, KIND_3X3_UP = 2 };
+enum : int { KIND_1X1 = 0, KIND_3X3 = 1, KIND_3X3_UP = 2, KIND_2X2_UP = 3 };
 
 __device__ __forceinline__ int fast_div(int m, unsigned long long magic) {
   return (int)(((unsigned long long)(unsigned)m * magic) >> 40);
@@ -137,11 +145,11 @@
   return v;
 }
 
-template <int BM, int BN, int WARPS_M, int WARPS_N, int LDS_BYTES>
+template <int BM, int BN, int WARPS_M, int WARPS_N, int LDS_BYTES, bool UP2 = false>
 __device__ __forceinline__ void igemm_epilogue(const IGemmParams& p_arg, f32x16 (&acc)[BM / WARPS_M / 32][BN / WARPS_N / 32],
                                                const int m0, const int n0, const int split, const int tile_m,
                                                const int tile_n, unsigned char* smem, const float lnf_mean = 0.f,
-                                               const float lnf_rstd = 1.f) {
+                                               const float lnf_rstd = 1.f, const int phase = 0) {
 #ifdef SDMI_IGEMM_TIMING
   IGemmParams p = p_arg;
   if (p.dbg_abl & 1) p.residual = nullptr;
@@ -158,9 +166,19 @@
   const int wave = tid >> 6;
   const int wm = wave / WARPS_N, wn = wave - wm * WARPS_N;
   const int l31 = lane & 31, lg = lane >> 5;
-  const int HWout = p.Hout * p.Wout;
+  const int HWout = UP2 ? p.Hin * p.Win : p.Hout * p.Wout;
+  const int pM = UP2 ? p.M >> 2 : p.M;
+  auto out_row = [&](int m) -> size_t {
+    if constexpr (UP2) {
+      const int b = fast_div_hw(m, p.magic_hw), rem = m - b * HWout, y = fast_div(rem, p.magic_w), x = rem - y * p.Win;
+      return ((size_t)b * (2 * p.Hin) + (size_t)(2 * y + (phase >> 1))) * (size_t)(2 * p.Win) + (size_t)(2 * x + (phase & 1));
+    } else {
+      return (size_t)m;
+    }
+  };
+  const int slab_row0 = UP2 ? phase * pM : 0;
   const int mw = m0 + wm * WTM, nw = n0 + wn * WTN;
-  const bool full = (m0 + BM <= p.M) && (n0 + BN <= p.N);
+  const bool full = (m0 + BM <= pM) && (n0 + BN <= p.N);
   if (p.splitk > 1 && p.splitk_fused) {
     constexpr int SC1 = 16;
     const int tile_lin = tile_m * ((p.N + BN - 1) / BN) + tile_n;
@@ -218,7 +236,7 @@
   }
   if (p.splitk > 1 && !p.splitk_fused && p.slab_tiled) {
     constexpr int SC1 = 16;
-    const int tiles_n_all = (p.N + BN - 1) / BN, ntiles = ((p.M + BM - 1) / BM) * tiles_n_all;
+    const int tiles_n_all = (p.N + BN - 1) / BN, ntiles = (UP2 ? 4 : 1) * ((pM + BM - 1) / BM) * tiles_n_all;
     const int tile_lin = tile_m * tiles_n_all + tile_n;
     const __amdgpu_buffer_rsrc_t ws = __builtin_amdgcn_make_buffer_rsrc(
         (void*)(p.splitk_ws + ((size_t)split * ntiles + tile_lin) * (size_t)(BM * BN)), 0, BM * BN * 4, 0x00020000);
@@ -255,7 +273,7 @@
   const bool unfused_split = p.splitk > 1 && !p.splitk_fused;
   if (p.mode == EPI_PLAIN) {
     const bool atomic = unfused_split;
-    float* slab = atomic ? (p.splitk_ws + (size_t)split * p.M * p.N) : nullptr;
+    float* slab = atomic ? (p.splitk_ws + ((size_t)split * p.M + slab_row0) * p.N) : nullptr;
     const int b_first = m0 / HWout;
     const bool one_batch = ((m0 + BM - 1) / HWout == b_first);
     if (full && one_batch && p.epi_vec && !atomic) {
@@ -285,7 +303,7 @@
           const int row = q * RPI + rl;
           float* const lp = wl + row * LSTR + c4;
           const f32x4 v = *(const f32x4*)lp + colv + resv[q];
-          const size_t ro = (size_t)(mw + i * 32 + row) * p.ldo + nw + c4;
+          const size_t ro = out_row(mw + i * 32 + row) * p.ldo + nw + c4;
           if (p.out_f32) SDMI_ST_F32X4(p.out_f32, ro, v);
           const f32x4 vs = v * g4;
           const f16x4 h = {(f16)vs[0], (f16)vs[1], (f16)vs[2], (f16)vs[3]};
@@ -341,7 +359,7 @@
           }
 #pragma unroll
           for (int r = 0; r < 16; ++r) {
-            const size_t ro = (size_t)(mw + i * 32 + (r & 3) + 8 * (r >> 2) + 4 * lg) * p.ldo + nw + l31;
+            const size_t ro = out_row(mw + i * 32 + (r & 3) + 8 * (r >> 2) + 4 * lg) * p.ldo + nw + l31;
 #pragma unroll
             for (int j = 0; j < TN; ++j) {
               const float v = acc[i][j][r] + colv[j] + resv[r][j];
@@ -365,8 +383,9 @@
 #pragma unroll
         for (int r = 0; r < 16; ++r) {
           const int m = mw + i * 32 + (r & 3) + 8 * (r >> 2) + 4 * lg;
-          if (m >= p.M) continue;
+          if (m >= pM) continue;
           const float* rv = (!atomic && p.rowvec) ? (p.rowvec + (size_t)(m / HWout) * p.ld_rowvec) : nullptr;
+          const size_t mo = out_row(m);
 #pragma unroll
           for (int j = 0; j < TN; ++j) {
             const int n = nw + j * 32 + l31;
@@ -379,9 +398,9 @@
               if (rv) v += rv[n];
               if (p.residual) v += p.residual[(size_t)m * p.ldr + n];
               acc[i][j][r] = v;
-              if (p.out_f32) p.out_f32[(size_t)m * p.ldo + n] = v;
-              if (p.out_f16) p.out_f16[(size_t)m * p.ldo + n] = (f16)v;
-              if (p.out_lo) p.out_lo[(size_t)m * p.ldo + n] = (f16)(v - (float)(f16)v);
+              if (p.out_f32) p.out_f32[mo * p.ldo + n] = v;
+              if (p.out_f16) p.out_f16[mo * p.ldo + n] = (f16)v;
+              if (p.out_lo) p.out_lo[mo * p.ldo + n] = (f16)(v - (float)(f16)v);
             }
           }
         }
@@ -428,14 +447,14 @@
 #pragma unroll
         for (int i = 0; i < TM; ++i) {
           const int mt = mw + i * 32;
-          if (mt < p.M) {
+          if (mt < pM) {
             const int bi = mt / HWout;
             if (bcur >= 0 && bi != bcur) { flush(bcur, s1, s2); s1 = 0.f; s2 = 0.f; }
             bcur = bi;
 #pragma unroll
             for (int r = 0; r < 16; ++r) {
               const int m = mt + (r & 3) + 8 * (r >> 2) + 4 * lg;
-              if (m < p.M) { const float v = acc[i][j][r]; s1 += v; s2 += v * v; }
+              if (m < pM) { const float v = acc[i][j][r]; s1 += v; s2 += v * v; }
             }
           }
         }
@@ -607,7 +626,7 @@
 
 static int reduce_rows_per_block(const IGemmParams& p) {
   int rpb = 32;
-  const int hw = p.Hout * p.Wout;
+  const int hw = p.up == 2 ? p.Hin * p.Win : p.Hout * p.Wout;
   while (rpb < 256 && (int64_t)cdiv(p.N / 4, 8) * cdiv(p.M, rpb * 2) >= 1024 && (p.gn_n == 0 || hw % (rpb * 2) == 0)) rpb *= 2;
   return rpb;
 }
@@ -617,7 +636,7 @@
   if ((bm & (bm - 1)) || (bn & (bn - 1))) return false;
   if (p.mode == EPI_PLAIN && p.gn_n > 0 && reduce_rows_per_block(p) != 32) return false;
   if (p.lnf_part || p.lnp_out || p.f16_scale) return false;
-  if ((int64_t)nsplit * cdiv(p.M, bm) * bm * cdiv(p.N, bn) * bn > p.splitk_ws_floats) return false;
+  if ((int64_t)nsplit * igemm_tiles_m(p, bm) * bm * cdiv(p.N, bn) * bn > p.splitk_ws_floats) return false;
   return true;
 }
 static void slab_layout(IGemmParams& q, int bm, int bn, int wm, int wn, int nsplit) {
@@ -629,7 +648,7 @@
 }
 static int64_t splitk_ws_need(const IGemmParams& p, int bm, int bn, int nsplit) {
   if (nsplit <= 1) return 0;
-  if (slab_tiled_ok(p, bm, bn, nsplit)) return (int64_t)nsplit * cdiv(p.M, bm) * bm * cdiv(p.N, bn) * bn;
+  if (slab_tiled_ok(p, bm, bn, nsplit)) return (int64_t)nsplit * igemm_tiles_m(p, bm) * bm * cdiv(p.N, bn) * bn;
   return (int64_t)nsplit * p.M * p.N;
 }
 
diff --git a/stable-diffusion_amd/csrc/igemm_kernel.h b/stable-diffusion_amd/csrc/igemm_kernel.h
--- a/stable-diffusion_amd/csrc/igemm_kernel.h
+++ b/stable-diffusion_amd/csrc/igemm_kernel.h
@@ -13,7 +13,9 @@
   static_assert(DMA || NS == 2, "the register-staged path is double buffered");
 #if defined(__HIP_DEVICE_COMPILE__)
   constexpr bool UP = KIND == KIND_3X3_UP;
+  constexpr bool UP2 = KIND == KIND_2X2_UP;
   constexpr bool K3 = KIND != KIND_1X1;
+  static_assert(!(UP2 && HALF), "the phase form takes whole 64-channel chunks");
   constexpr int NT = WARPS_M * WARPS_N * 64;
   constexpr int RPP = NT / 8;
   constexpr int A_PASSES = BM / RPP;
@@ -36,7 +38,10 @@
   int tile_m, tile_n;
   if (p.tile_n_fastest) { tile_m = tmn / tiles_n; tile_n = tmn - tile_m * tiles_n; }
   else { tile_n = tmn / tiles_m; tile_m = tmn - tile_n * tiles_m; }
-  const int m0 = tile_m * BM, n0 = tile_n * BN;
+  const int tiles_ph = UP2 ? tiles_m >> 2 : tiles_m;
+  const int phase = UP2 ? tile_m / tiles_ph : 0;
+  const int m0 = (tile_m - phase * tiles_ph) * BM, n0 = tile_n * BN;
+  const int pM = UP2 ? p.M >> 2 : p.M;
   const int nkt = HALF ? p.nkt : p.K / BK;
   const int kt_begin = split * kt_per_split;
   const int kt_end = min(nkt, kt_begin + kt_per_split);
@@ -55,19 +60,21 @@
   const int gch = cpos ^ ((lrow >> 1) & 7);
   const int hi_oob = (HALF && gch >= 4) ? (int)0x80000000 : 0;
 
-  const int HWout = p.Hout * p.Wout;
+  const int HWout = UP2 ? p.Hin * p.Win : p.Hout * p.Wout;
+  const int Wrow = UP2 ? p.Win : p.Wout;
   const int pad = K3 ? p.pad : 0;
-  constexpr int ntap = K3 ? 9 : 1;
+  constexpr int ntap = K3 ? (UP2 ? 4 : 9) : 1;
+  constexpr int KW = UP2 ? 2 : 3;
   const int ld = p.lda0;
   int a_off[A_PASSES];
   unsigned a_mask[K3 ? A_PASSES : 1];
   int a_ro[UP ? A_PASSES : 1][3], a_co[UP ? A_PASSES : 1][3];
 #pragma unroll
   for (int i = 0; i < A_PASSES; ++i) {
-    const int m = min(m0 + i * RPP + lrow, p.M - 1);
+    const int m = min(m0 + i * RPP + lrow, pM - 1);
     const int b = fast_div_hw(m, p.magic_hw);
     const int rem = m - b * HWout;
-    const int oy = fast_div(rem, p.magic_w), ox = rem - oy * p.Wout;
+    const int oy = fast_div(rem, p.magic_w), ox = rem - oy * Wrow;
     const int pb = b * p.Hin * p.Win;
     if constexpr (UP) {
       const int Hv = 2 * p.Hin, Wv = 2 * p.Win;
@@ -85,6 +92,16 @@
       }
       a_mask[i] = mk | ((HALF && gch < 4) ? mk << 9 : 0u);
       a_off[i] = 0;
+    } else if constexpr (UP2) {
+      const int cy = oy + (phase >> 1), cx = ox + (phase & 1);
+      a_off[i] = ((pb + cy * p.Win + cx) * ld + gch * 8) * 2;
+      unsigned mk = 0;
+#pragma unroll
+      for (int t = 0; t < 4; ++t) {
+        const int iy = cy + t / 2 - 1, ix = cx + t % 2 - 1;
+        if (iy >= 0 && iy < p.Hin && ix >= 0 && ix < p.Win) mk |= 1u << t;
+      }
+      a_mask[i] = mk;
     } else {
       const int cy = oy * p.stride, cx = ox * p.stride;
       a_off[i] = ((pb + cy * p.Win + cx) * ld + gch * 8) * 2;
@@ -112,7 +129,7 @@
   int ld_kt = kt_begin;
   int ld_tap = K3 ? kt_begin % ntap : 0;
   int ld_cin0 = (kt_begin / ntap) * BK;
-  int ld_ky = K3 ? ld_tap / 3 : 0, ld_kx = K3 ? ld_tap - 3 * (ld_tap / 3) : 0;
+  int ld_ky = K3 ? ld_tap / KW : 0, ld_kx = K3 ? ld_tap - KW * (ld_tap / KW) : 0;
   const int pc0 = p.c0, pc1 = p.c1, pc2 = p.c2;
   const int pp0 = (pc0 + BK - 1) & ~(BK - 1), pp01 = pp0 + ((pc1 + BK - 1) & ~(BK - 1));
   int ld_boff = 0;
@@ -126,7 +143,7 @@
   const long long a_shift = (K3 && !UP) ? (long long)(pad * p.Win + pad) * ld * 2 : 0;
   const char* const srcA0 = (const char*)p.a0 - a_shift; const char* const srcA1 = (const char*)p.a1 - a_shift;
   const char* const srcA2 = (const char*)p.a2 - a_shift;
-  const __amdgpu_buffer_rsrc_t rsrc_w = __builtin_amdgcn_make_buffer_rsrc((void*)p.w, 0, OOB, 0x00020000);
+  const __amdgpu_buffer_rsrc_t rsrc_w = __builtin_amdgcn_make_buffer_rsrc((void*)(p.w + (UP2 ? (size_t)phase * p.N * p.K : 0)), 0, OOB, 0x00020000);
   const int pWin = p.Win;
 
   struct TileCursor { __amdgpu_buffer_rsrc_t rsrc_a; int a_soff, b_soff; unsigned tapbit; int ky, kx; unsigned lds; int half; };
@@ -148,7 +165,7 @@
       if constexpr (HALF) ld_boff += half ? BKH * 2 : BK * 2;
       if constexpr (K3) {
         ++ld_tap;
-        if (++ld_kx == 3) { ld_kx = 0; ++ld_ky; }
+        if (++ld_kx == KW) { ld_kx = 0; ++ld_ky; }
         if (ld_tap == ntap) { ld_tap = 0; ld_ky = 0; ld_kx = 0; ld_cin0 += BK; }
       } else {
         ld_cin0 += BK;
@@ -290,7 +307,7 @@
   }
 
   SDMI_STAMP(dbg_t2);
-  igemm_epilogue<BM, BN, WARPS_M, WARPS_N, NS * STAGE_BYTES>(p, acc, m0, n0, split, tile_m, tile_n, smem, lnf_mean, lnf_rstd);
+  igemm_epilogue<BM, BN, WARPS_M, WARPS_N, NS * STAGE_BYTES, UP2>(p, acc, m0, n0, split, tile_m, tile_n, smem, lnf_mean, lnf_rstd, phase);
 #ifdef SDMI_IGEMM_TIMING
   if (p.dbg_times && tid == 0) {
     long long* d = p.dbg_times + 6 * (size_t)blockIdx.x;
@@ -303,7 +320,8 @@
 template <int BM, int BN, int WARPS_M, int WARPS_N, int NS, bool HALF = false>
 int launch_cfg(const IGemmParams& p, bool dma, int splitk, hipStream_t stream) {
   SDMI_CHECK(HALF || (p.c0 % BK == 0 && p.c1 % BK == 0 && p.c2 % BK == 0), "internal: a half k-tile launch on the whole-chunk kernel");
-  const int tiles_m = cdiv(p.M, BM), tiles_n = cdiv(p.N, BN);
+  SDMI_CHECK(p.up != 2 || !HALF, "internal: the phase form of an Upsample conv on the half k-tile kernel");
+  const int tiles_m = igemm_tiles_m(p, BM), tiles_n = cdiv(p.N, BN);
   const int nkt = igemm_nkt(p);
   const int kt_per_split = cdiv(nkt, splitk);
   const int nsplit = cdiv(nkt, kt_per_split);
@@ -316,8 +334,8 @@
   q.epi_vec = epi_vec_ok(p);
   SDMI_CHECK(splitk_ws_need(p, BM, BN, nsplit) <= p.splitk_ws_floats, "split-K workspace too small");
   SDMI_CHECK((int64_t)p.M < (int64_t)65536 * p.Hout * p.Wout, "fast_div_hw: at most 65535 samples per launch");
-  q.magic_hw = div_magic_hw(p.Hout * p.Wout);
-  q.magic_w = div_magic(p.Wout);
+  q.magic_hw = div_magic_hw(p.up == 2 ? p.Hin * p.Win : p.Hout * p.Wout);
+  q.magic_w = div_magic(p.up == 2 ? p.Win : p.Wout);
   for (int t = 0; t < p.gn_n; ++t) q.gn_magic[t] = div_magic(p.gn_cpg[t]);
   dim3 grid(tiles_m * tiles_n * nsplit), block(WARPS_M * WARPS_N * 64);
   static const int by_shape = env_int("SDMI_PROF_SHAPES", 0);
@@ -335,7 +353,7 @@
                src_pix * cin_alg * 2.0 + (double)p.N * k_alg * 2.0 + (double)p.M * n_out * out_b +
                    (p.residual ? (double)p.M * p.N * 4.0 : 0.0),
                stream, 2.0 * p.M * (double)p.N * p.K);
-  const int kind = p.ksize == 1 ? KIND_1X1 : (p.up ? KIND_3X3_UP : KIND_3X3);
+  const int kind = p.ksize == 1 ? KIND_1X1 : (p.up == 2 ? KIND_2X2_UP : (p.up ? KIND_3X3_UP : KIND_3X3));
 #define SDMI_LAUNCH_KIND(K_)                                                                                        \
   do {                                                                                                              \
     if (dma) SDMI_LAUNCH((igemm_kernel<BM, BN, WARPS_M, WARPS_N, true, NS, K_, HALF>), grid, block, 0, stream, q,   \
@@ -345,7 +363,8 @@
   } while (0)
   if (kind == KIND_1X1) SDMI_LAUNCH_KIND(KIND_1X1);
   else if (kind == KIND_3X3) SDMI_LAUNCH_KIND(KIND_3X3);
-  else SDMI_LAUNCH_KIND(KIND_3X3_UP);
+  else if (kind == KIND_3X3_UP) SDMI_LAUNCH_KIND(KIND_3X3_UP);
+  else if constexpr (!HALF) SDMI_LAUNCH_KIND(KIND_2X2_UP);
 #undef SDMI_LAUNCH_KIND
   SDMI_HIP_OK(hipGetLastError());
   ps.end();
diff --git a/stable-diffusion_amd/csrc/small.hip b/stable-diffusion_amd/csrc/small.hip
--- a/stable-diffusion_amd/csrc/small.hip
+++ b/stable-diffusion_amd/csrc/small.hip
@@ -336,6 +336,29 @@
   const f16 hi = (f16)v;
   dst[idx] = (!split3 || src < 2) ? hi : (f16)(v - (float)hi);
 }
+__global__ void pack_conv_up_phase_kernel(const float* w, const f16* w9, f16* dst, int O, int I) {
+  const int64_t idx = (int64_t)blockIdx.x * blockDim.x + threadIdx.x;
+  const int64_t K = (int64_t)4 * I;
+  if (idx >= 4 * (int64_t)O * K) return;
+  const int phase = (int)(idx / ((int64_t)O * K));
+  const int64_t r = idx - (int64_t)phase * O * K;
+  const int o = (int)(r / K), k = (int)(r - (int64_t)o * K);
+  const int chunk = k / 256, rem = k - chunk * 256, t = rem / 64, ci = chunk * 64 + rem % 64;
+  const int a = phase >> 1, c = phase & 1, i = t >> 1, j = t & 1;
+  const int ky0 = (a == 0) ? (i == 0 ? 0 : 1) : (i == 0 ? 0 : 2), ky1 = (a == 0) ? (i == 0 ? 0 : 2) : (i == 0 ? 1 : 2);
+  const int kx0 = (c == 0) ? (j == 0 ? 0 : 1) : (j == 0 ? 0 : 2), kx1 = (c == 0) ? (j == 0 ? 0 : 2) : (j == 0 ? 1 : 2);
+  const float* src = w ? w + ((int64_t)o * I + ci) * 9 : nullptr;
+  const f16* src9 = w9 + (int64_t)o * 9 * I + (int64_t)chunk * 9 * 64 + (ci & 63);
+  float sum = 0.f;
+  bool first = true;
+  for (int ky = ky0; ky <= ky1; ++ky)
+    for (int kx = kx0; kx <= kx1; ++kx) {
+      const float v = src ? src[ky * 3 + kx] : (float)src9[(ky * 3 + kx) * 64];
+      sum = first ? v : sum + v;
+      first = false;
+    }
+  dst[idx] = (f16)sum;
+}
 __global__ void pack_conv_f32_kernel(const float* w, float* dst, int O, int I, int KH, int KW) {
   const int64_t idx = (int64_t)blockIdx.x * blockDim.x + threadIdx.x;
   const int64_t total = (int64_t)O * I * KH * KW;
@@ -645,6 +668,14 @@
   SDMI_HIP_OK(hipGetLastError());
   return 0;
 }
+int launch_pack_conv_up_phase(const float* w, const f16* w9, f16* dst, int O, int I, hipStream_t s) {
+  SDMI_CHECK(I > 0 && I % 64 == 0, "phase pack of an Upsample conv: input channels must be a multiple of 64");
+  SDMI_CHECK((w != nullptr) != (w9 != nullptr), "phase pack of an Upsample conv: one source, the fp32 weight or its nine-tap pack");
+  const int64_t total = (int64_t)16 * O * I;
+  SDMI_LAUNCH(pack_conv_up_phase_kernel, dim3((unsigned)((total + 255) / 256)), dim3(256), 0, s, w, w9, dst, O, I);
+  SDMI_HIP_OK(hipGetLastError());
+  return 0;
+}
 int launch_pack_conv_out(const float* w, float* dst, int O, int I, hipStream_t s) {
   const int64_t total = (int64_t)O * I * 9;
   SDMI_LAUNCH(pack_conv_f32_kernel, dim3((unsigned)((total + 255) / 256)), dim3(256), 0, s, w, dst, O, I, 3, 3);
diff --git a/stable-diffusion_amd/csrc/unet.cpp b/stable-diffusion_amd/csrc/unet.cpp
--- a/stable-diffusion_amd/csrc/unet.cpp
+++ b/stable-diffusion_amd/csrc/unet.cpp
@@ -241,7 +241,8 @@
         store_.expect(p + ".op.bias", {co}, W_F32, &L.f32[0]);
         break;
       case L_UP:
-        store_.expect(p + ".conv.weight", {co, ci, 3, 3}, full() ? W_CONV_SPLIT3 : W_CONV, &L.w16[0]);
+        if (full()) store_.expect(p + ".conv.weight", {co, ci, 3, 3}, W_CONV_SPLIT3, &L.w16[0]);
+        else store_.expect(p + ".conv.weight", {co, ci, 3, 3}, W_CONV_UP, &L.w16[0]).dst2 = (void**)&L.w16[1];
         store_.expect(p + ".conv.bias", {co}, W_F32, &L.f32[0]);
         break;
     }
@@ -387,6 +388,7 @@
     SDMI_HIP_OK(hipMemcpyAsync(*b.first, (const char*)host_buf + off, b.second, hipMemcpyHostToDevice, stream));
     off += (int64_t)round_up((int64_t)b.second, PK_ALIGN);
   }
+  if (store_.derive_up_phase(stream)) return -1;
   SDMI_HIP_OK(hipStreamSynchronize(stream));
   store_.mark_all_set();
   ctx_valid_ = false;
@@ -762,6 +764,7 @@
     IGemmParams p = conv3(x16, C, Hin, Win, Hout, Wout, up ? 1 : 2, up ? 1 : 0, L.w16[0], L.cout);
     p.bias = L.f32[0]; p.out_f32 = out.p; p.ldo = L.cout;
     attach_gn_targets(p, out);
+    if (up) up_phase(p, L.w16[1], up_sites++);
     gemm(p);
     scratch.off = mark;
     return out;
@@ -1048,7 +1051,7 @@
     const bool d = (pass == 0) ? true : false;
     if (pass == 1 && dry) break;
     f.dry = d; f.rc = 0;
-    f.n_acts = 0;
+    f.n_acts = 0; f.up_sites = 0;
     TapeRecGuard tape_guard(d ? nullptr : rec);
     f.plan = fuse_gn_stats_ ? &gn_plan_ : nullptr;
     if (d) gn_plan_.clear();
diff --git a/stable-diffusion_amd/csrc/unet.h b/stable-diffusion_amd/csrc/unet.h
--- a/stable-diffusion_amd/csrc/unet.h
+++ b/stable-diffusion_amd/csrc/unet.h
@@ -126,6 +126,18 @@
     p.B = B; p.Hin = Hin; p.Win = Win; p.Hout = Hout; p.Wout = Wout;
     p.ksize = 3; p.stride = stride; p.up = up; p.w = w; p.M = B * Hout * Wout; p.N = N; p.K = 9 * C; p.splitk = 0;
     return p;
+  }
+  static constexpr int UP_PHASE_SITE_FIRST_STAGE = 8;
+  static constexpr unsigned long UP_PHASE_SITES_DEFAULT = 0xfful;
+  int up_sites = 0;
+  static void up_phase(IGemmParams& p, const f16* w_phase, int site) {
+    if (!w_phase || p.c0 % 64 != 0 || p.c1 != 0) return;
+    if (const char* e = getenv("SDMI_UP_PHASE")) { if (atoi(e) == 0) return; }
+    const char* e_sites = getenv("SDMI_UP_PHASE_SITES");
+    const unsigned long sites = e_sites ? strtoul(e_sites, nullptr, 0) : UP_PHASE_SITES_DEFAULT;
+    if (site > 31 || !((sites >> site) & 1ul)) return;
+    if (p.gn_n > 0 && (p.Hin * p.Win) % 32 != 0) return;
+    p.up = 2; p.w = w_phase; p.K = 4 * p.c0;
   }
   static void split3(IGemmParams& p, const f16* hi, const f16* lo, int C) {
     p.a0 = hi; p.c0 = C; p.lda0 = C; p.a1 = lo; p.c1 = C; p.lda1 = C; p.a2 = hi; p.c2 = C; p.lda2 = C;
diff --git a/stable-diffusion_amd/csrc/vae.cpp b/stable-diffusion_amd/csrc/vae.cpp
--- a/stable-diffusion_amd/csrc/vae.cpp
+++ b/stable-diffusion_amd/csrc/vae.cpp
@@ -94,7 +94,8 @@
       }
       case V_UP:
       case V_DOWN:
-        store_.expect(p + ".conv.weight", {co, ci, 3, 3}, conv_kind, &L.w16[0]);
+        if (L.kind == V_UP && !full()) store_.expect(p + ".conv.weight", {co, ci, 3, 3}, W_CONV_UP, &L.w16[0]).dst2 = (void**)&L.w16[1];
+        else store_.expect(p + ".conv.weight", {co, ci, 3, 3}, conv_kind, &L.w16[0]);
         store_.expect(p + ".conv.bias", {co}, W_F32, &L.f32[0]);
         break;
     }
@@ -286,6 +287,7 @@
     if (full) split3(p, x16, x16_lo, C);
     if (!up) p.pad = 0;
     p.bias = L.f32[0]; p.out_f32 = out.p; p.ldo = C;
+    if (up && !full) up_phase(p, L.w16[1], UP_PHASE_SITE_FIRST_STAGE);
     gemm(p);
     scratch.off = mark;
     return out;
diff --git a/stable-diffusion_amd/csrc/weights.cpp b/stable-diffusion_amd/csrc/weights.cpp
--- a/stable-diffusion_amd/csrc/weights.cpp
+++ b/stable-diffusion_amd/csrc/weights.cpp
@@ -49,7 +49,7 @@
   switch (s.kind) {
     case W_F32: case W_CONV_OUT: case W_GEGLU_B: case W_QKV_LEGACY_B: return numel * sizeof(float);
     case W_F32_ROWS: return rows * sizeof(float);
-    case W_CONV: case W_GEGLU_W: return numel * sizeof(f16);
+    case W_CONV: case W_CONV_UP: case W_GEGLU_W: return numel * sizeof(f16);
     case W_SPLIT3: case W_CONV_SPLIT3: return 3 * numel * sizeof(f16);
     case W_QKV_LEGACY: return numel * sizeof(f16) * (s.split ? 3 : 1);
     case W_ROWS16: return rows * sizeof(f16);
@@ -63,6 +63,17 @@
   if (*dst) return 0;
   SDMI_HIP_OK(hipMalloc(dst, bytes));
   owned_.push_back(*dst);
+  return 0;
+}
+
+static int up_phase_of(WeightStore& st, const WeightSlot& s, hipStream_t stream) {
+  if (!s.dst2 || s.shape.size() != 4 || s.shape[1] % 64 != 0 || s.shape[2] != 3 || s.shape[3] != 3) return 0;
+  if (st.alloc(s.dst2, (size_t)16 * s.shape[0] * s.shape[1] * sizeof(f16))) return -1;
+  return launch_pack_conv_up_phase(nullptr, (const f16*)*s.dst, (f16*)*s.dst2, (int)s.shape[0], (int)s.shape[1], stream);
+}
+int WeightStore::derive_up_phase(hipStream_t stream) {
+  for (const auto& s : slots_)
+    if (s.kind == W_CONV_UP && *s.dst && up_phase_of(*this, s, stream)) return -1;
   return 0;
 }
 
@@ -118,6 +129,10 @@
     case W_CONV:
       rc = launch_pack_conv_weight(dptr, (f16*)*s.dst, (int)shape[0], (int)shape[1], (int)shape[2], (int)shape[3], stream);
       break;
+    case W_CONV_UP:
+      rc = launch_pack_conv_weight(dptr, (f16*)*s.dst, (int)shape[0], (int)shape[1], (int)shape[2], (int)shape[3], stream);
+      if (!rc) rc = up_phase_of(*this, s, stream);
+      break;
     case W_SPLIT3:
       rc = launch_pack_split3(dptr, (f16*)*s.dst, (int)shape[0], (int)shape[1], stream);
       break;
diff --git a/stable-diffusion_amd/csrc/weights.h b/stable-diffusion_amd/csrc/weights.h
--- a/stable-diffusion_amd/csrc/weights.h
+++ b/stable-diffusion_amd/csrc/weights.h
@@ -15,13 +15,14 @@
 };
 
 enum WKind { W_F32, W_F32_ROWS, W_CONV, W_CONV_OUT, W_ROWS16, W_GEGLU_W, W_GEGLU_B, W_SPLIT3, W_SPLIT3_ROWS, W_CONV_SPLIT3, W_QKV_LEGACY,
-             W_QKV_LEGACY_B, W_DROP };
+             W_QKV_LEGACY_B, W_DROP, W_CONV_UP };
 
 struct WeightSlot {
   std::string key;
   std::vector<int64_t> shape;
   WKind kind = W_F32;
   void** dst = nullptr;
+  void** dst2 = nullptr;
   int row0 = 0;
   int ld = 0;
   int buf_rows = 0;
@@ -43,6 +44,7 @@
   const WeightSlot* missing() const;
   void mark_all_set() { for (auto& s : slots_) s.set = true; }
   int alloc(void** dst, size_t bytes);
+  int derive_up_phase(hipStream_t stream);
   int zero_page();
   const f16* zero() const { return zero_; }
   std::vector<std::pair<void**, size_t>> buffers() const;
```

Result: no change. 3.834 (median of 6 runs) (+0.5%).
